# hupe1980/vecgo

Hardware: AMD Instinct MI355X
Metric: QPS at recall@10≥0.95, 1M×768 HNSW+PQ; PQ-ADC HBM GB/s vs peak (higher is better)
Workload: dtype f32; 1 GPU; flat_exact_l2_1Mx768_top10 (BASELINE configs[1]): MFMA GEMM nomination + exact re-score + proof; operating_point=flat_exact, rows=1000000, dim=768, k=10, parallelism=1 GPU

## Files before the change

### go/segment/resident.go

```go

package segment

import "C"

import (
	"fmt"
	"unsafe"

	"github.com/hupe1980/vecgo/distance"
	"github.com/hupe1980/vecgo/internal/hipctx"
)

type Stats struct {
	NodesVisited, DistanceComputations, DistanceShortCircuits, Pops int64
	DescentDistanceComputations                                    int64
}

const (
	ScanF32 = int32(C.VG_SCAN_F32)
	ScanPQ  = int32(C.VG_SCAN_PQ)
	ScanSQ8 = int32(C.VG_SCAN_SQ8)
)

const (
// ... 346 lines not shown
		return nil, nil, counts, false, nil
	}
	if mask != nil {
		need := (r.rows + 7) / 8
		if maskStride != 0 {
			if maskStride < need {
				return nil, nil, nil, false, fmt.Errorf("%s: maskStride %d is shorter than a mask (%d bytes)", name, maskStride, need)
			}
			need += (nq - 1) * maskStride
		}
		if len(mask) < need {
			return nil, nil, nil, false, fmt.Errorf("%s: mask holds %d bytes, %d needed", name, len(mask), need)
		}
	}
	ids, sc = r.out(nq, maxResults)
	return ids, sc, counts, true, nil
}

func (r *Resident) SearchProbedThreshold(queries []float32, nq int, thresholds []float32, maxResults, nprobes int, scan int32, rerank bool, mask []byte, maskStride int) ([]uint32, []float32, []int32, error) {
	ids, sc, counts, ok, err := r.thresholdOperands("SearchProbedThreshold", nq, thresholds, maxResults, mask, maskStride)
	if !ok {
		return nil, nil, counts, err
	}
	var mp *C.uint8_t
	if mask != nil {
		mp = bp(mask)
	}
	rr := 0
	if rerank {
		rr = 1
	}
	st := C.vg_search_flat_probed_threshold(r.h, fp(queries), C.int64_t(nq), fp(thresholds), C.int32_t(maxResults), C.int32_t(nprobes), C.int32_t(scan), C.int32_t(rr), mp, C.int64_t(maskStride), up(ids), fp(sc), ip(counts), nil)
	return ids, sc, counts, hipctx.Err(int32(st))
}

func (r *Resident) SearchSegmentThreshold(queries []float32, nq int, thresholds []float32, maxResults, nprobes int, rerank bool, mask []byte, maskStride int) ([]uint32, []float32, []int32, error) {
	ids, sc, counts, ok, err := r.thresholdOperands("SearchSegmentThreshold", nq, thresholds, maxResults, mask, maskStride)
	if !ok {
		return nil, nil, counts, err
	}
	var mp *C.uint8_t
	if mask != nil {
		mp = bp(mask)
	}
	rr := 0
	if rerank {
		rr = 1
	}
	st := C.vg_segment_search_threshold(r.seg, fp(queries), C.int64_t(nq), fp(thresholds), C.int32_t(maxResults), C.int32_t(nprobes), C.int32_t(rr), mp, C.int64_t(maskStride), up(ids), fp(sc), ip(counts), nil)
	return ids, sc, counts, hipctx.Err(int32(st))
}

func (r *Resident) SearchPQ(queries []float32, nq, k int) ([]uint32, []float32, error) {
	ids, sc := r.out(nq, k)
	st := C.vg_search_pq_adc(r.h, fp(queries), C.int64_t(nq), C.int32_t(k), up(ids), fp(sc), nil)
	return ids, sc, hipctx.Err(int32(st))
}

func (r *Resident) SearchSQ8(queries []float32, nq, k int) ([]uint32, []float32, error) {
	ids, sc := r.out(nq, k)
	st := C.vg_search_sq8(r.h, fp(queries), C.int64_t(nq), C.int32_t(k), up(ids), fp(sc), nil)
	return ids, sc, hipctx.Err(int32(st))
}

func (r *Resident) EnableSQ8Nomination(on bool) error {
	v := C.int32_t(0)
	if on {
		v = 1
	}
	return hipctx.Err(int32(C.vg_index_enable_sq8_nomination(r.h, v, nil)))
}

func (r *Resident) EnablePQNomination(on bool) error {
	v := C.int32_t(0)
	if on {
		v = 1
	}
	return hipctx.Err(int32(C.vg_index_enable_pq_nomination(r.h, v, nil)))
}

func (r *Resident) FlatRetried() (int64, error) {
	var n C.int64_t
	st := C.vg_index_flat_retried(r.h, &n, nil)
	return int64(n), hipctx.Err(int32(st))
}

func (r *Resident) SearchRaBitQ(queries []float32, nq, k int) ([]uint32, []float32, error) {
	ids, sc := r.out(nq, k)
	st := C.vg_search_rabitq(r.h, fp(queries), C.int64_t(nq), C.int32_t(k), up(ids), fp(sc), nil)
	return ids, sc, hipctx.Err(int32(st))
}

func (r *Resident) SearchProbed(queries []float32, nq, k, nprobes int, scan int32) ([]uint32, []float32, error) {
	ids, sc := r.out(nq, k)
	st := C.vg_search_flat_probed(r.h, fp(queries), C.int64_t(nq), C.int32_t(k), C.int32_t(nprobes), C.int32_t(scan), up(ids), fp(sc), nil)
	return ids, sc, hipctx.Err(int32(st))
}

func (r *Resident) SearchSegmentFiltered(queries []float32, nq, k, nprobes int, mask []byte, maskStride int) ([]uint32, []float32, error) {
	ids, sc := r.out(nq, k)
	need := (r.rows + 7) / 8
	if maskStride != 0 {
		if maskStride < need {
			return nil, nil, fmt.Errorf("SearchSegmentFiltered: maskStride %d is shorter than a mask (%d bytes)", maskStride, need)
		}
		need += (nq - 1) * maskStride
	}
	if len(mask) < need {
		return nil, nil, fmt.Errorf("SearchSegmentFiltered: mask holds %d bytes, %d needed", len(mask), need)
	}
	st := C.vg_segment_search_filtered(r.seg, fp(queries), C.int64_t(nq), C.int32_t(k), C.int32_t(nprobes), bp(mask), C.int64_t(maskStride), up(ids), fp(sc), nil)
	return ids, sc, hipctx.Err(int32(st))
}

func (r *Resident) SearchFiltered(queries []float32, nq, k, nprobes int, scan int32, mask []byte, maskStride int) ([]uint32, []float32, error) {
	ids, sc := r.out(nq, k)
	need := (r.rows + 7) / 8
	if maskStride != 0 {
		if maskStride < need {
			return nil, nil, fmt.Errorf("SearchFiltered: maskStride %d is shorter than a mask (%d bytes)", maskStride, need)
		}
		need += (nq - 1) * maskStride
	}
	if len(mask) < need {
		return nil, nil, fmt.Errorf("SearchFiltered: mask holds %d bytes, %d needed", len(mask), need)
	}
	st := C.vg_search_flat_filtered(r.h, fp(queries), C.int64_t(nq), C.int32_t(k), C.int32_t(nprobes), C.int32_t(scan), bp(mask), C.int64_t(maskStride), up(ids), fp(sc), nil)
	return ids, sc, hipctx.Err(int32(st))
}

func (r *Resident) Search(queries []float32, nq, k, nprobes int) ([]uint32, []float32, error) {
	ids, sc := r.out(nq, k)
	st := C.vg_segment_search(r.seg, fp(queries), C.int64_t(nq), C.int32_t(k), C.int32_t(nprobes), up(ids), fp(sc), nil)
	return ids, sc, hipctx.Err(int32(st))
}

func (r *Resident) SearchHNSW(queries []float32, nq, k, ef int, stats []Stats) ([]uint32, []float32, error) {
	ids, sc := r.out(nq, k)
	var sp *C.vg_search_stats
	if len(stats) >= nq && nq > 0 {
		sp = (*C.vg_search_stats)(unsafe.Pointer(&stats[0]))
	}
	st := C.vg_search_hnsw(r.h, fp(queries), C.int64_t(nq), C.int32_t(k), C.int32_t(ef), up(ids), fp(sc), sp, nil)
	return ids, sc, hipctx.Err(int32(st))
}

func (r *Resident) SearchHNSWPQ(queries []float32, nq, k, ef int, stats []Stats) ([]uint32, []float32, error) {
	ids, sc := r.out(nq, k)
	var sp *C.vg_search_stats
	if len(stats) >= nq && nq > 0 {
		sp = (*C.vg_search_stats)(unsafe.Pointer(&stats[0]))
	}
	st := C.vg_search_hnsw_pq(r.h, fp(queries), C.int64_t(nq), C.int32_t(k), C.int32_t(ef), up(ids), fp(sc), sp, nil)
	return ids, sc, hipctx.Err(int32(st))
}

func (r *Resident) SearchHNSWFiltered(queries []float32, nq, k, ef int, mask []byte, maskStride int, selectivity float64, stats []Stats) ([]uint32, []float32, error) {
	ids, sc := r.out(nq, k)
	need := (r.rows + 7) / 8
	if maskStride != 0 {
		if maskStride < need {
			return nil, nil, fmt.Errorf("SearchHNSWFiltered: maskStride %d is shorter than a mask (%d bytes)", maskStride, need)
		}
		need += (nq - 1) * maskStride
	}
	if len(mask) < need {
// ... 196 lines not shown
```

### include/vecgo_hip.h

```cpp
#ifndef VECGO_HIP_H
#define VECGO_HIP_H

#include <stddef.h>
#include <stdint.h>

#ifdef __cplusplus
extern "C" {
#endif

#define VG_ABI_VERSION 2
#define VG_ABI_MINOR 13
#define VG_INVALID_ID 0xFFFFFFFFu
#define VG_STREAM_LEGACY ((void *)1)

typedef enum vg_status {
    VG_OK = 0,
    VG_ERR_INVALID_ARG = -1,
    VG_ERR_DIM_MISMATCH = -2,
    VG_ERR_NOT_TRAINED = -3,
    VG_ERR_CODE_LENGTH = -4,
    VG_ERR_UNSUPPORTED = -5,
    VG_ERR_OUT_OF_MEMORY = -6,
    VG_ERR_HIP = -7,
    VG_ERR_NO_DEVICE = -8,
// ... 89 lines not shown
                                const int64_t *level_rows, uint32_t entry_point, void *stream);
int32_t vg_hnsw_build(vg_index *idx, int32_t m, int32_t ef_construction, int32_t max_batch,
                      int32_t growth_div, void *stream);
int32_t vg_hnsw_insert(vg_index *idx, const float *rows, int64_t count, int32_t m, int32_t ef_construction,
                       int32_t max_batch, int32_t growth_div, void *stream);
int32_t vg_hnsw_level_for_id(uint64_t id, int32_t m);
typedef struct vg_hnsw_compact_stats {
    int64_t repaired_nodes;
    int64_t repaired_lists;
    int64_t pruned_links;
    int64_t cleared_nodes;
} vg_hnsw_compact_stats;
int32_t vg_hnsw_compact(vg_index *idx, int32_t ef_construction, int32_t max_batch, vg_hnsw_compact_stats *stats,
                        void *stream);
int32_t vg_index_get_hnsw_graph(const vg_index *idx, int32_t *m0, int32_t *m, int32_t *max_level,
                                uint32_t *entry_point, int64_t *level_rows, uint32_t *l0,
                                uint32_t *upper_slot, uint32_t *upper_adj, void *stream);
int32_t vg_index_set_vamana_graph(vg_index *idx, int32_t r, const uint32_t *graph, uint32_t entry_point,
                                  void *stream);
int32_t vg_vamana_build(vg_index *idx, int32_t r, int32_t l, float alpha, const uint32_t *init_graph, uint64_t seed,
                        int32_t max_batch, int32_t growth_div, void *stream);
int32_t vg_vamana_insert(vg_index *idx, const float *rows, int64_t count, int32_t r, int32_t l, float alpha,
                         const uint8_t *deleted, uint64_t seed, int32_t max_batch, int32_t growth_div, void *stream);
typedef struct vg_vamana_consolidate_stats {
    int64_t repaired_nodes;
    int64_t dropped_links;
    int64_t links_before;
    int64_t links_after;
} vg_vamana_consolidate_stats;
int32_t vg_vamana_consolidate(vg_index *idx, int32_t l, float alpha, const uint8_t *deleted, int32_t max_batch,
                              vg_vamana_consolidate_stats *stats, void *stream);
int32_t vg_index_get_vamana_graph(const vg_index *idx, int32_t *r, uint32_t *entry_point, uint32_t *graph,
                                  void *stream);
int32_t vg_vamana_reorder_bfs(vg_index *idx, uint32_t *perm, uint32_t *inv_perm, void *stream);

int32_t vg_index_set_vectors(vg_index *idx, const float *base, void *stream);

int32_t vg_squared_l2_batch(vg_ctx *ctx, const float *query, const float *targets, int64_t dim,
                            int64_t n, float *out, void *stream);
int32_t vg_dot_batch(vg_ctx *ctx, const float *query, const float *targets, int64_t dim,
                     int64_t n, float *out, void *stream);

int32_t vg_squared_l2_bounded_batch(vg_ctx *ctx, const float *query, const float *targets, int64_t dim,
                                    int64_t n, const float *bounds, int64_t n_bounds, float *dist,
                                    int32_t *exceeded, void *stream);
int32_t vg_pq_adc_lookup_batch(vg_ctx *ctx, const float *table, const uint8_t *codes, int64_t m, int64_t n,
                               float *out, void *stream);

int32_t vg_kmeans_train(vg_ctx *ctx, const float *vectors, int64_t n, int32_t dim, int32_t k, int32_t metric,
                        int32_t max_iter, uint64_t seed, float *centroids, int32_t *produced, void *stream);
int32_t vg_kmeans_assign(vg_ctx *ctx, const float *vectors, int64_t n, int32_t dim, const float *centroids,
                         int32_t k, int32_t metric, int32_t *out, void *stream);
int32_t vg_find_closest_centroids(vg_ctx *ctx, const float *query, const float *centroids, int32_t dim,
                                  int32_t k, int32_t nprobe, int32_t metric, int32_t *out, int32_t *n_out,
                                  void *stream);

int64_t vg_binary_code_bytes(int32_t dim);
int32_t vg_binary_train(vg_ctx *ctx, int32_t dim, const float *vectors, int64_t n, float *threshold, void *stream);
int32_t vg_binary_encode(vg_ctx *ctx, int32_t dim, float threshold, const float *vectors, int64_t n,
                         uint8_t *codes, void *stream);
int32_t vg_binary_decode(vg_ctx *ctx, int32_t dim, float threshold, const uint8_t *codes, int64_t n,
                         int32_t code_bytes, float *out, void *stream);
int32_t vg_binary_hamming_batch(vg_ctx *ctx, int32_t dim, float threshold, const float *query,
                                const uint8_t *codes, int64_t n, int32_t *out, void *stream);
int32_t vg_normalize_l2(vg_ctx *ctx, float *vectors, int64_t n, int32_t dim, uint8_t *ok, void *stream);

int32_t vg_rerank(vg_index *idx, const float *queries, int64_t nq, const uint32_t *cand_ids,
                  int32_t nc, int32_t k, uint32_t *ids, float *scores, void *stream);
int32_t vg_score_candidates(vg_index *idx, const float *queries, int64_t nq,
                            const uint32_t *cand_ids, int32_t nc, float *scores, void *stream);

int32_t vg_search_flat(vg_index *idx, const float *queries, int64_t nq, int32_t k, uint32_t *ids,
                       float *scores, void *stream);
int32_t vg_index_enable_bf16_filter(vg_index *idx, int32_t on, void *stream);

int32_t vg_search_flat_threshold(vg_index *idx, const float *queries, int64_t nq, const float *thresholds,
                                 int32_t max_results, const uint8_t *mask, int64_t mask_stride,
                                 uint32_t *ids, float *scores, int32_t *counts, void *stream);

int32_t vg_index_flat_stats(vg_index *idx, int64_t *queries, int64_t *exhaustive, void *stream);

int32_t vg_index_flat_retried(vg_index *idx, int64_t *retried, void *stream);

int32_t vg_search_rabitq(vg_index *idx, const float *queries, int64_t nq, int32_t k, uint32_t *ids,
                         float *scores, void *stream);

int32_t vg_sq8_create(vg_ctx *ctx, int32_t dim, vg_sq8 **out);
int32_t vg_sq8_destroy(vg_sq8 *sq);
int32_t vg_sq8_is_trained(vg_sq8 *sq);
int32_t vg_sq8_train(vg_sq8 *sq, const float *vectors, int64_t n, void *stream);
int32_t vg_sq8_set_bounds(vg_sq8 *sq, const float *mins, const float *maxs);
int32_t vg_sq8_get_params(vg_sq8 *sq, float *mins, float *maxs, float *scales, float *inv_scales);
int32_t vg_sq8_encode(vg_sq8 *sq, const float *vectors, int64_t n, uint8_t *codes, void *stream);
int32_t vg_sq8_decode(vg_sq8 *sq, const uint8_t *codes, int64_t n, float *out, void *stream);
int32_t vg_sq8_l2_distance_batch(vg_sq8 *sq, const float *query, const uint8_t *codes, int64_t n,
                                 float *out, void *stream);
int32_t vg_index_set_sq8_codes(vg_index *idx, vg_sq8 *sq, const uint8_t *codes, void *stream);
int32_t vg_index_enable_sq8_nomination(vg_index *idx, int32_t on, void *stream);
int32_t vg_search_sq8(vg_index *idx, const float *queries, int64_t nq, int32_t k, uint32_t *ids,
                      float *scores, void *stream);

int32_t vg_int4_create(vg_ctx *ctx, int32_t dim, vg_int4 **out);
int32_t vg_int4_destroy(vg_int4 *iq);
int32_t vg_int4_is_trained(vg_int4 *iq);
int32_t vg_int4_train(vg_int4 *iq, const float *vectors, int64_t n, void *stream);
int32_t vg_int4_set_params(vg_int4 *iq, const float *min_val, const float *diff);
int32_t vg_int4_get_params(vg_int4 *iq, float *min_val, float *diff, float *table);
int64_t vg_int4_code_bytes(int32_t dim);
int32_t vg_int4_encode(vg_int4 *iq, const float *vectors, int64_t n, uint8_t *codes, void *stream);
int32_t vg_int4_decode(vg_int4 *iq, const uint8_t *codes, int64_t n, float *out, void *stream);
int32_t vg_int4_l2_distance_batch(vg_int4 *iq, const float *query, const uint8_t *codes, int64_t n,
                                  int32_t precomputed, float *out, void *stream);
int32_t vg_index_set_int4_codes(vg_index *idx, vg_int4 *iq, const uint8_t *codes, void *stream);

int32_t vg_robust_prune(vg_index *idx, const uint32_t *nodes, int64_t n_nodes, const uint32_t *cands,
                        int32_t nc, int32_t r, float alpha, uint32_t *out, int32_t *counts, void *stream);
int32_t vg_hnsw_select_neighbors(vg_index *idx, int64_t n_nodes, const uint32_t *cand_ids,
                                 const float *cand_dists, int32_t nc, int32_t m, uint32_t *out,
                                 int32_t *counts, void *stream);

int32_t vg_index_set_partitions(vg_index *idx, const float *centroids, const uint32_t *part_offsets,
                                int32_t num_partitions, void *stream);
enum { VG_SCAN_F32 = 0, VG_SCAN_PQ = 1, VG_SCAN_SQ8 = 2 };
int32_t vg_search_flat_probed(vg_index *idx, const float *queries, int64_t nq, int32_t k, int32_t nprobes,
                              int32_t scan, uint32_t *ids, float *scores, void *stream);
int32_t vg_search_flat_filtered(vg_index *idx, const float *queries, int64_t nq, int32_t k, int32_t nprobes,
                                int32_t scan, const uint8_t *mask, int64_t mask_stride, uint32_t *ids, float *scores,
                                void *stream);

int32_t vg_search_flat_probed_threshold(vg_index *idx, const float *queries, int64_t nq, const float *thresholds,
                                        int32_t max_results, int32_t nprobes, int32_t scan , int32_t rerank,
                                        const uint8_t *mask, int64_t mask_stride,
                                        uint32_t *ids, float *scores, int32_t *counts, void *stream);

int32_t vg_flat_build(vg_index *idx, int32_t num_partitions, int32_t quantization, int32_t pq_m, int32_t kmeans_iters,
                      int32_t pq_iters, uint64_t seed, vg_sq8 *sq, vg_pq *pq, uint32_t *perm, uint32_t *inv_perm, void *stream);

enum { VG_QUANT_NONE = 0, VG_QUANT_PQ = 1, VG_QUANT_SQ8 = 3, VG_QUANT_RABITQ = 5, VG_QUANT_INT4 = 6 };
typedef struct vg_segment_info {
    uint64_t segment_id;
    int64_t rows;
    int32_t dim, metric;
    int32_t kind;
    int32_t quantization;
    int32_t pq_m, pq_k;
    int32_t max_degree, search_list_size;
    uint32_t entrypoint;
    int32_t num_partitions;
} vg_segment_info;
int32_t vg_segment_open_flat(vg_ctx *ctx, const void *image, int64_t size, int32_t verify_checksum,
                             vg_segment **out, void *stream);
int32_t vg_segment_search(vg_segment *seg, const float *queries, int64_t nq, int32_t k, int32_t nprobes,
                          uint32_t *ids, float *scores, void *stream);
int32_t vg_segment_search_filtered(vg_segment *seg, const float *queries, int64_t nq, int32_t k, int32_t nprobes,
                                   const uint8_t *mask, int64_t mask_stride, uint32_t *ids, float *scores, void *stream);
int32_t vg_segment_search_threshold(vg_segment *seg, const float *queries, int64_t nq, const float *thresholds,
                                    int32_t max_results, int32_t nprobes, int32_t rerank, const uint8_t *mask,
                                    int64_t mask_stride, uint32_t *ids, float *scores, int32_t *counts, void *stream);
int32_t vg_segment_open_diskann(vg_ctx *ctx, const void *image, int64_t size, int32_t verify_checksum,
                                vg_segment **out, void *stream);
int32_t vg_segment_get_info(vg_segment *seg, vg_segment_info *info);
vg_index *vg_segment_index(vg_segment *seg);
vg_pq *vg_segment_pq(vg_segment *seg);
vg_sq8 *vg_segment_sq8(vg_segment *seg);
vg_int4 *vg_segment_int4(vg_segment *seg);
int32_t vg_segment_close(vg_segment *seg);
// ... 81 lines not shown
```

### include/vecgo_hip.hpp

```cpp
#pragma once

#include <algorithm>
#include <cstdint>
#include <cstring>
#include <memory>
#include <stdexcept>
#include <string>
#include <utility>
#include <vector>

#include "vecgo_hip.h"

namespace vecgo {

class Error : public std::runtime_error {
public:
    Error(int32_t status, const std::string &msg) : std::runtime_error(msg), status_(status) {}
    int32_t status() const { return status_; }

private:
    int32_t status_;
};

inline void check(int32_t status)
// ... 483 lines not shown
{
    int32_t out = -1;
    check(vg_kmeans_assign(c.handle(), vec.data(), 1, dim, centroids.data(), static_cast<int32_t>(centroids.size() / dim),
                           static_cast<int32_t>(metric), &out, nullptr));
    return out;
}

inline std::vector<int> FindClosestCentroids(const Context &c, const std::vector<float> &query,
                                             const std::vector<float> &centroids, int dim, int n, distance::Metric metric)
{
    const int k = static_cast<int>(centroids.size() / dim);
    std::vector<int32_t> out(static_cast<size_t>(std::max(1, std::min(n, k))));
    int32_t cnt = 0;
    check(vg_find_closest_centroids(c.handle(), query.data(), centroids.data(), dim, k, n, static_cast<int32_t>(metric),
                                    out.data(), &cnt, nullptr));
    return std::vector<int>(out.begin(), out.begin() + cnt);
}

}

inline uint32_t CRC32CDevice(const Context &c, const void *devicePtr, int64_t size)
{
    uint32_t out = 0;
    check(vg_crc32c_device(c.handle(), devicePtr, size, &out, nullptr));
    return out;
}

struct Result {
    std::vector<uint32_t> ids;
    std::vector<float> scores;
};
struct ThresholdResult {
    std::vector<uint32_t> ids;
    std::vector<float> scores;
    std::vector<int32_t> counts;
};

class Segment {
public:
    Segment(std::shared_ptr<Context> ctx, int64_t rows, int dim, distance::Metric metric)
        : ctx_(std::move(ctx)), n_(rows), dim_(dim)
    {
        check(vg_index_create(ctx_->handle(), rows, dim, static_cast<int32_t>(metric), &h_));
    }
    ~Segment() { vg_index_destroy(h_); }
    Segment(const Segment &) = delete;
    Segment &operator=(const Segment &) = delete;

    void SetVectors(const float *base) { check(vg_index_set_vectors(h_, base, nullptr)); }
    void SetPQCodes(std::shared_ptr<quantization::ProductQuantizer> pq, const uint8_t *codes)
    {
        pq_ = std::move(pq);
        check(vg_index_set_pq_codes(h_, pq_->handle(), codes, nullptr));
    }
    void SetRaBitQCodes(const uint8_t *codes) { check(vg_index_set_rabitq_codes(h_, codes, nullptr)); }
    void SetVamanaGraph(int r, const uint32_t *graph, uint32_t entry) { check(vg_index_set_vamana_graph(h_, r, graph, entry, nullptr)); }
    void SetHNSWLayer0(int m0, const uint32_t *l0, uint32_t entry)
    {
        check(vg_index_set_hnsw_graph(h_, m0, l0, 0, m0 / 2 > 0 ? m0 / 2 : 1, nullptr, nullptr, nullptr, entry, nullptr));
    }

    Result SearchFlat(const float *queries, int64_t nq, int k) { return run(nq, k, [&](Result &r) { return vg_search_flat(h_, queries, nq, k, r.ids.data(), r.scores.data(), nullptr); }); }
    ThresholdResult SearchThreshold(const float *queries, int64_t nq, const float *thresholds, int max_results,
                                    const uint8_t *mask = nullptr, int64_t mask_stride = 0)
    {
        ThresholdResult r;
        r.ids.resize(static_cast<size_t>(nq) * max_results);
        r.scores.resize(static_cast<size_t>(nq) * max_results);
        r.counts.resize(static_cast<size_t>(nq));
        check(vg_search_flat_threshold(h_, queries, nq, thresholds, max_results, mask, mask_stride, r.ids.data(), r.scores.data(),
                                       r.counts.data(), nullptr));
        return r;
    }
    ThresholdResult SearchProbedThreshold(const float *queries, int64_t nq, const float *thresholds, int max_results, int nprobes,
                                          int scan, bool rerank, const uint8_t *mask = nullptr, int64_t mask_stride = 0)
    {
        ThresholdResult r;
        r.ids.resize(static_cast<size_t>(nq) * max_results);
        r.scores.resize(static_cast<size_t>(nq) * max_results);
        r.counts.resize(static_cast<size_t>(nq));
        check(vg_search_flat_probed_threshold(h_, queries, nq, thresholds, max_results, nprobes, scan, rerank ? 1 : 0, mask, mask_stride,
                                              r.ids.data(), r.scores.data(), r.counts.data(), nullptr));
        return r;
    }
    void EnableBF16Filter(bool on = true) { check(vg_index_enable_bf16_filter(h_, on ? 1 : 0, nullptr)); }
    Result SearchPQ(const float *queries, int64_t nq, int k) { return run(nq, k, [&](Result &r) { return vg_search_pq_adc(h_, queries, nq, k, r.ids.data(), r.scores.data(), nullptr); }); }
    void EnablePQNomination(bool on = true) { check(vg_index_enable_pq_nomination(h_, on ? 1 : 0, nullptr)); }
    Result SearchRaBitQ(const float *queries, int64_t nq, int k) { return run(nq, k, [&](Result &r) { return vg_search_rabitq(h_, queries, nq, k, r.ids.data(), r.scores.data(), nullptr); }); }
    void SetPartitions(const float *centroids, const uint32_t *part_offsets, int num_partitions)
    {
        check(vg_index_set_partitions(h_, centroids, part_offsets, num_partitions, nullptr));
    }
    Result SearchFiltered(const float *queries, int64_t nq, int k, int nprobes, int scan, const uint8_t *mask, int64_t mask_stride) { return run(nq, k, [&](Result &r) { return vg_search_flat_filtered(h_, queries, nq, k, nprobes, scan, mask, mask_stride, r.ids.data(), r.scores.data(), nullptr); }); }
    Result SearchProbed(const float *queries, int64_t nq, int k, int nprobes, int scan) { return run(nq, k, [&](Result &r) { return vg_search_flat_probed(h_, queries, nq, k, nprobes, scan, r.ids.data(), r.scores.data(), nullptr); }); }
    void BuildHNSW(int m = 32, int efConstruction = 300, int maxBatch = 8192, int growthDiv = 32)
    {
        check(vg_hnsw_build(h_, m, efConstruction, maxBatch, growthDiv, nullptr));
    }
    void InsertHNSW(const float *rows, int64_t count, int m = 32, int ef = 300, int maxBatch = 8192, int growthDiv = 32)
    {
        check(vg_hnsw_insert(h_, rows, count, m, ef, maxBatch, growthDiv, nullptr));
    }
    vg_hnsw_compact_stats CompactHNSW(int ef = 300, int maxBatch = 8192)
    {
        vg_hnsw_compact_stats stats{};
        check(vg_hnsw_compact(h_, ef, maxBatch, &stats, nullptr));
        return stats;
    }
    void BuildVamana(int r = 64, int l = 100, float alpha = 1.2f, const uint32_t *initGraph = nullptr, uint64_t seed = 0,
                     int maxBatch = 8192, int growthDiv = 32)
    {
        check(vg_vamana_build(h_, r, l, alpha, initGraph, seed, maxBatch, growthDiv, nullptr));
    }
    void InsertVamana(const float *rows, int64_t count, int r = 64, int l = 100, float alpha = 1.2f, const uint8_t *deleted = nullptr,
                      uint64_t seed = 0, int maxBatch = 8192, int growthDiv = 32)
    {
        check(vg_vamana_insert(h_, rows, count, r, l, alpha, deleted, seed, maxBatch, growthDiv, nullptr));
    }
    vg_vamana_consolidate_stats ConsolidateVamana(const uint8_t *deleted, int l = 100, float alpha = 1.2f, int maxBatch = 8192)
    {
        vg_vamana_consolidate_stats stats{};
        check(vg_vamana_consolidate(h_, l, alpha, deleted, maxBatch, &stats, nullptr));
        return stats;
    }
    void ReorderVamanaBFS(uint32_t *perm, uint32_t *invPerm) { check(vg_vamana_reorder_bfs(h_, perm, invPerm, nullptr)); }
    void FlatBuild(int numPartitions, int quantization, std::shared_ptr<quantization::ScalarQuantizer> sq,
                   std::shared_ptr<quantization::ProductQuantizer> pq, uint32_t *perm, uint32_t *invPerm, uint64_t seed = 0,
                   int pqM = 0, int kmeansIters = 0, int pqIters = 0)
    {
        check(vg_flat_build(h_, numPartitions, quantization, pqM, kmeansIters, pqIters, seed, sq ? sq->handle() : nullptr,
                            pq ? pq->handle() : nullptr, perm, invPerm, nullptr));
        if (quantization == VG_QUANT_SQ8) sq_ = std::move(sq);
        if (quantization == VG_QUANT_PQ) pq_ = std::move(pq);
    }
    std::vector<uint8_t> WriteFlat(uint64_t segmentID, const uint64_t *ids = nullptr, const std::vector<uint8_t> *metadata = nullptr,
                                   const std::vector<uint8_t> *blockStats = nullptr)
    {
        const int64_t size = vg_segment_flat_image_size(h_, metadata ? static_cast<int64_t>(metadata->size()) : -1,
                                                        blockStats ? static_cast<int64_t>(blockStats->size()) : -1);
        if (size < 0) check(VG_ERR_UNSUPPORTED);
        std::vector<uint8_t> image(static_cast<size_t>(size));
        static const uint8_t none = 0;
        int64_t written = 0;
        check(vg_segment_write_flat(h_, segmentID, ids, metadata ? (metadata->empty() ? &none : metadata->data()) : nullptr,
                                    metadata ? static_cast<int64_t>(metadata->size()) : 0,
                                    blockStats ? (blockStats->empty() ? &none : blockStats->data()) : nullptr,
                                    blockStats ? static_cast<int64_t>(blockStats->size()) : 0, image.data(), size, &written, nullptr));
        return image;
    }
    int DiskANNBuild(int r, int l, float alpha, int quantization, std::shared_ptr<quantization::ProductQuantizer> pq,
                     std::shared_ptr<quantization::Int4Quantizer> iq, uint32_t *perm, uint32_t *invPerm, uint64_t seed = 0,
                     int pqM = 0, int pqIters = 0, int maxBatch = 8192, int growthDiv = 32)
    {
        int32_t used = VG_QUANT_NONE;
        check(vg_diskann_build(h_, r, l, alpha, quantization, pqM, pqIters, seed, maxBatch, growthDiv, pq ? pq->handle() : nullptr,
                               iq ? iq->handle() : nullptr, perm, invPerm, &used, nullptr));
        if (used == VG_QUANT_PQ) pq_ = std::move(pq);
        if (used == VG_QUANT_INT4) iq_ = std::move(iq);
        return used;
    }
    std::vector<uint8_t> WriteDiskANN(uint64_t segmentID, int searchListSize = 0, int compressionType = 1, const uint64_t *ids = nullptr,
                                      const std::vector<uint8_t> *metadata = nullptr, const std::vector<uint8_t> *metadataIndex = nullptr)
    {
        const int64_t size = vg_segment_diskann_image_size(h_, metadata ? static_cast<int64_t>(metadata->size()) : -1,
                                                           metadataIndex ? static_cast<int64_t>(metadataIndex->size()) : -1);
        std::vector<uint8_t> image(static_cast<size_t>(size < 0 ? 1 : size));
// ... 67 lines not shown
```

### vecgo_amd/api.py

```python
from __future__ import annotations

import ctypes as C
import enum

import numpy as np

from . import _lib
from ._lib import VecgoHipError, check

try:
    import torch
except Exception:
    torch = None


class Metric(enum.IntEnum):
    L2 = 0
    COSINE = 1
    DOT = 2
    HAMMING = 3


def _is_torch(x) -> bool:
    return torch is not None and isinstance(x, torch.Tensor)
# ... 1302 lines not shown
    def score_candidates(self, queries, cand_ids, out=None, stream=None):
        nq = _rows(queries, self.dim)
        nc = (cand_ids.numel() if _is_torch(cand_ids) else np.asarray(cand_ids).size) // max(nq, 1)
        q, pq_ = _ptr(queries, np.float32)
        c, pc = _ptr(cand_ids, np.uint32, nq * nc)
        if out is None:
            out = _empty_like(queries, (nq, nc), np.float32)
        s, ps = _ptr(out, np.float32, nq * nc)
        check(self._lib.vg_score_candidates(self._h, pq_, C.c_int64(nq), pc, C.c_int32(nc), ps,
                                            _stream_ptr(stream)))
        return out

    def _search(self, fn, queries, k, extra=(), out=None, stream=None):
        nq = _rows(queries, self.dim)
        q, pq_ = _ptr(queries, np.float32)
        if out is None:
            ids = _empty_like(queries, (nq, k), np.uint32)
            scores = _empty_like(queries, (nq, k), np.float32)
        else:
            ids, scores = out
        i, pi = _ptr(ids, np.uint32, nq * k)
        s, ps = _ptr(scores, np.float32, nq * k)
        check(fn(self._h, pq_, C.c_int64(nq), C.c_int32(k), *extra, pi, ps, _stream_ptr(stream)))
        return ids, scores

    def search_flat(self, queries, k, out=None, stream=None):
        return self._search(self._lib.vg_search_flat, queries, k, out=out, stream=stream)

    def _threshold_search(self, name, call, queries, thresholds, max_results, mask, out):
        nq = _rows(queries, self.dim)
        q, pq_ = _ptr(queries, np.float32)
        if _is_torch(thresholds):
            t = thresholds.to(torch.float32).reshape(-1)
            if t.numel() == 1 and nq != 1:
                t = t.expand(nq)
            t = t.contiguous()
        else:
            t = np.asarray(thresholds, np.float32).reshape(-1)
            if t.size == 1:
                t = np.full(nq, t[0], np.float32)
        if (t.numel() if _is_torch(t) else t.size) != nq:
            raise ValueError(f"{name}: one threshold for the batch or one per query ({nq})")
        t, pt = _ptr(t, np.float32, nq)
        m, pm, stride = (None, None, 0) if mask is None else self._packed_mask(mask, nq, name)
        if out is None:
            ids = _empty_like(queries, (nq, max_results), np.uint32)
            scores = _empty_like(queries, (nq, max_results), np.float32)
            counts = _empty_like(queries, (nq,), np.int32)
        else:
            ids, scores, counts = out
        i, pi = _ptr(ids, np.uint32, nq * max_results)
        s, ps = _ptr(scores, np.float32, nq * max_results)
        c, pc = _ptr(counts, np.int32, nq)
        check(call(pq_, C.c_int64(nq), pt, pm, C.c_int64(stride), pi, ps, pc))
        return ids, scores, counts

    def search_flat_threshold(self, queries, thresholds, max_results, mask=None, out=None, stream=None):
        def call(pq_, nq, pt, pm, stride, pi, ps, pc):
            return self._lib.vg_search_flat_threshold(self._h, pq_, nq, pt, C.c_int32(max_results), pm, stride, pi, ps, pc,
                                                      _stream_ptr(stream))
        return self._threshold_search("search_flat_threshold", call, queries, thresholds, max_results, mask, out)

    def search_flat_probed_threshold(self, queries, thresholds, max_results, nprobes=0, scan=0, rerank=False, mask=None, out=None,
                                     stream=None):
        def call(pq_, nq, pt, pm, stride, pi, ps, pc):
            return self._lib.vg_search_flat_probed_threshold(self._h, pq_, nq, pt, C.c_int32(max_results), C.c_int32(nprobes),
                                                             C.c_int32(scan), C.c_int32(1 if rerank else 0), pm, stride, pi, ps, pc,
                                                             _stream_ptr(stream))
        return self._threshold_search("search_flat_probed_threshold", call, queries, thresholds, max_results, mask, out)

    def enable_bf16_filter(self, on: bool = True, stream=None):
        check(self._lib.vg_index_enable_bf16_filter(self._h, C.c_int32(1 if on else 0), _stream_ptr(stream)))

    def flat_stats(self, stream=None):
        q, e = C.c_int64(0), C.c_int64(0)
        check(self._lib.vg_index_flat_stats(self._h, C.byref(q), C.byref(e), _stream_ptr(stream)))
        return q.value, e.value

    def flat_retried(self, stream=None):
        r = C.c_int64(0)
        check(self._lib.vg_index_flat_retried(self._h, C.byref(r), _stream_ptr(stream)))
        return r.value

    def search_pq_adc(self, queries, k, out=None, stream=None):
        return self._search(self._lib.vg_search_pq_adc, queries, k, out=out, stream=stream)


class SegmentInfo(C.Structure):
    _fields_ = [("segment_id", C.c_uint64), ("rows", C.c_int64), ("dim", C.c_int32), ("metric", C.c_int32),
                ("kind", C.c_int32), ("quantization", C.c_int32), ("pq_m", C.c_int32), ("pq_k", C.c_int32),
                ("max_degree", C.c_int32), ("search_list_size", C.c_int32), ("entrypoint", C.c_uint32),
                ("num_partitions", C.c_int32)]


class Segment:

    def __init__(self, ctx: Context, image, kind: str = "flat", verify_checksum: bool = True, stream=None):
        self._lib, self.ctx = ctx._lib, ctx
        buf = np.frombuffer(image, np.uint8) if isinstance(image, (bytes, bytearray, memoryview)) else \
            np.ascontiguousarray(image, np.uint8)
        fn = {"flat": self._lib.vg_segment_open_flat, "diskann": self._lib.vg_segment_open_diskann}[kind]
        h = C.c_void_p()
        check(fn(ctx._h, C.c_void_p(buf.ctypes.data), C.c_int64(buf.size), C.c_int32(int(verify_checksum)),
                 C.byref(h), _stream_ptr(stream)))
        self._h = h
        info = SegmentInfo()
        check(self._lib.vg_segment_get_info(self._h, C.byref(info)))
        self.info = info
        self._lib.vg_segment_index.restype = C.c_void_p
        ih = C.c_void_p(self._lib.vg_segment_index(self._h))
        self.index = Index._borrowed(ctx, ih, int(info.rows), int(info.dim), int(info.metric), self)

    def search(self, queries, k, nprobes=0, out=None, stream=None):
        seg = self._h

        def fn(_index_handle, *args):
            return self._lib.vg_segment_search(seg, *args)
        return self.index._search(fn, queries, k, extra=(C.c_int32(nprobes),), out=out, stream=stream)

    def search_filtered(self, queries, k, mask, nprobes=0, out=None, stream=None):
        if mask is None:
            return self.search(queries, k, nprobes, out=out, stream=stream)
        seg = self._h
        m, pm, stride = self.index._packed_mask(mask, _rows(queries, self.index.dim), "Segment.search_filtered")

        def fn(_index_handle, *args):
            return self._lib.vg_segment_search_filtered(seg, *args)
        return self.index._search(fn, queries, k, extra=(C.c_int32(nprobes), pm, C.c_int64(stride)), out=out, stream=stream)

    def search_threshold(self, queries, thresholds, max_results, nprobes=0, rerank=False, mask=None, out=None, stream=None):
        seg = self._h

        def call(pq_, nq, pt, pm, stride, pi, ps, pc):
            return self._lib.vg_segment_search_threshold(seg, pq_, nq, pt, C.c_int32(max_results), C.c_int32(nprobes),
                                                         C.c_int32(1 if rerank else 0), pm, stride, pi, ps, pc, _stream_ptr(stream))
        return self.index._threshold_search("Segment.search_threshold", call, queries, thresholds, max_results, mask, out)

    def close(self):
        if getattr(self, "_h", None):
            self.index._h = None
            self._lib.vg_segment_close(self._h)
            self._h = None

    def __del__(self):
        try:
            self.close()
        except Exception:
            pass


def crc32c(data) -> int:
    from . import _lib
    lib = _lib.load()
    lib.vg_crc32c.restype = C.c_uint32
    buf = np.frombuffer(data, np.uint8) if isinstance(data, (bytes, bytearray, memoryview)) else \
        np.ascontiguousarray(data, np.uint8)
    return int(lib.vg_crc32c(C.c_void_p(buf.ctypes.data), C.c_int64(buf.size)))


def crc32c_device(ctx: Context, data, stream=None) -> int:
    if not _is_torch(data) or not data.is_cuda:
        raise TypeError("crc32c_device takes a torch tensor in device memory (crc32c is the host's)")
    if not data.is_contiguous():
        raise ValueError("crc32c_device: the tensor must be contiguous")
    out = C.c_uint32(0)
    check(ctx._lib.vg_crc32c_device(ctx._h, C.c_void_p(data.data_ptr()), C.c_int64(data.numel() * data.element_size()), C.byref(out),
# ... 3 lines not shown
```

### vecgo_amd/csrc/k_exact.hip

```cpp
#include "vg_device.hpp"
#include "vg_exact.hpp"
#include "vg_internal.hpp"

namespace vg {

constexpr int kExactThreads = 256;

template <bool DOT>
__global__ __launch_bounds__(kExactThreads) void batch_kernel(const float *__restrict__ query,
                                                              const float *__restrict__ targets,
                                                              int dim, int64_t n,
                                                              float *__restrict__ out)
{
    const Sub16 sub = Sub16::make(threadIdx.x);
    const int64_t groups = static_cast<int64_t>(gridDim.x) * (kExactThreads / 16);
    for (int64_t i = static_cast<int64_t>(blockIdx.x) * (kExactThreads / 16) + (threadIdx.x >> 4);
         i < n; i += groups) {
        const float v = exact_pair16<DOT, kBatch, true>(targets + i * dim, query, dim, sub);
        if ((threadIdx.x & 15) == 0) out[i] = v;
    }
}

__global__ __launch_bounds__(256) void bounded_batch_kernel(const float *__restrict__ query,
                                                            const float *__restrict__ targets, int dim, int64_t n,
// ... 86 lines not shown
{
    __shared__ float sm[1024];
    float m = 0.0f;
    for (int64_t i = threadIdx.x; i < n; i += 1024) m = fmaxf(m, v[i]);
    sm[threadIdx.x] = m;
    __syncthreads();
    for (int s = 512; s > 0; s >>= 1) {
        if (threadIdx.x < s) sm[threadIdx.x] = fmaxf(sm[threadIdx.x], sm[threadIdx.x + s]);
        __syncthreads();
    }
    if (threadIdx.x == 0) out[0] = sm[0];
}

__global__ void row_norms_kernel(const float *__restrict__ base, int64_t n, int dim,
                                 float *__restrict__ norms, int *__restrict__ maxabs_bits)
{
    const int64_t row = static_cast<int64_t>(blockIdx.x) * (blockDim.x / 64) + (threadIdx.x >> 6);
    if (row >= n) return;
    const int lane = threadIdx.x & 63;
    float s = 0.0f, mx = 0.0f;
    for (int j = lane; j < dim; j += 64) {
        const float v = base[row * dim + j];
        s = __builtin_fmaf(v, v, s);
        const float a = fabsf(v);
        mx = fmaxf(mx, a == a ? a : INFINITY);
    }
    for (int off = 32; off > 0; off >>= 1) {
        s += __shfl_xor(s, off);
        mx = fmaxf(mx, __shfl_xor(mx, off));
    }
    if (lane == 0) {
        norms[row] = s;
        if (__float_as_int(mx) > *reinterpret_cast<volatile int *>(maxabs_bits)) atomicMax(maxabs_bits, __float_as_int(mx));
    }
}

}

static bool metric_is_dot(int32_t metric) { return metric != VG_METRIC_L2; }

namespace vg {
__global__ void fold_max_kernel(float *__restrict__ dst, const float *__restrict__ src) { dst[0] = fmaxf(dst[0], src[0]); }

int32_t append_row_norms(vg_index *idx, int64_t from, int64_t to, hipStream_t st)
{
    if (to <= from) return VG_OK;
    DevTmp<float> mx;
    VG_TRY(mx.init(1, st));
    VG_LAUNCH(row_norms_kernel, dim3(static_cast<unsigned>((to - from + 3) / 4)), dim3(256), 0, st,
              idx->d_vectors + from * idx->dim, to - from, idx->dim, idx->d_norms + from, reinterpret_cast<int *>(idx->d_norm_max + 1));
    VG_LAUNCH(norm_max_kernel, dim3(1), dim3(1024), 0, st, idx->d_norms + from, to - from, mx.ptr);
    VG_LAUNCH(fold_max_kernel, dim3(1), dim3(1), 0, st, idx->d_norm_max, mx.ptr);
    return VG_OK;
}
}

VG_API int32_t vg_index_set_vectors(vg_index *idx, const float *base, void *stream)
{
    VG_CHECK(idx, VG_ERR_INVALID_ARG, "vg_index_set_vectors: NULL index");
    VG_CHECK(idx->n == 0 || base, VG_ERR_INVALID_ARG, "vg_index_set_vectors: base is NULL");
    VG_CHECK(idx->metric != VG_METRIC_HAMMING, VG_ERR_UNSUPPORTED,
             "unsupported metric for float32: Hamming");
    VG_HIP(hipSetDevice(idx->ctx->device));
    hipStream_t st = vg::pick_stream(idx->ctx, stream);
    if (idx->d_vectors) {
        VG_HIP(hipStreamSynchronize(st));
        VG_HIP(hipFree(idx->d_vectors));
        VG_HIP(hipFree(idx->d_norms));
        VG_HIP(hipFree(idx->d_norm_max));
        VG_HIP(hipFree(idx->d_flat_stats));
        if (idx->d_vectors_bf16) VG_HIP(hipFree(idx->d_vectors_bf16));
        idx->d_vectors = idx->d_norms = idx->d_norm_max = nullptr;
        idx->d_flat_stats = nullptr;
        idx->d_vectors_bf16 = nullptr;
    }
    idx->rows_cap = idx->bf16_cap = 0;
    if (idx->n == 0) return VG_OK;
    const int32_t status = [&]() -> int32_t {
        size_t count = static_cast<size_t>(idx->n) * idx->dim;
        VG_HIP(hipMalloc(reinterpret_cast<void **>(&idx->d_vectors), count * sizeof(float)));
        VG_HIP(hipMalloc(reinterpret_cast<void **>(&idx->d_norms), static_cast<size_t>(idx->n) * sizeof(float)));
        VG_HIP(hipMalloc(reinterpret_cast<void **>(&idx->d_norm_max), 2 * sizeof(float)));
        VG_HIP(hipMemsetAsync(idx->d_norm_max, 0, 2 * sizeof(float), st));
        VG_HIP(hipMalloc(reinterpret_cast<void **>(&idx->d_flat_stats), 3 * sizeof(unsigned long long)));
        VG_HIP(hipMemcpyAsync(idx->d_vectors, base, count * sizeof(float), hipMemcpyDefault, st));
        VG_LAUNCH(vg::row_norms_kernel, dim3(static_cast<unsigned>((idx->n + 3) / 4)), dim3(256),
                           0, st, idx->d_vectors, idx->n, idx->dim, idx->d_norms, reinterpret_cast<int *>(idx->d_norm_max + 1));
        VG_LAUNCH(vg::norm_max_kernel, dim3(1), dim3(1024), 0, st, idx->d_norms, idx->n, idx->d_norm_max);
        VG_HIP(hipMemsetAsync(idx->d_flat_stats, 0, 3 * sizeof(unsigned long long), st));
        VG_HIP(hipStreamSynchronize(st));
        return VG_OK;
    }();
    if (status != VG_OK) {
        (void)hipStreamSynchronize(st);
        if (idx->d_vectors) (void)hipFree(idx->d_vectors);
        if (idx->d_norms) (void)hipFree(idx->d_norms);
        if (idx->d_norm_max) (void)hipFree(idx->d_norm_max);
        if (idx->d_flat_stats) (void)hipFree(idx->d_flat_stats);
        idx->d_vectors = idx->d_norms = idx->d_norm_max = nullptr;
        idx->d_flat_stats = nullptr;
    }
    return status;
}

static int32_t batch_impl(vg_ctx *ctx, bool dot, const float *query, const float *targets,
                          int64_t dim, int64_t n, float *out, void *stream)
{
    VG_CHECK(ctx, VG_ERR_INVALID_ARG, "batch kernel: ctx is NULL");
    if (dim <= 0 || n <= 0) return VG_OK;
    VG_CHECK(query && targets && out, VG_ERR_INVALID_ARG, "batch kernel: NULL buffer");
    VG_CHECK(dim < (1 << 30), VG_ERR_INVALID_ARG, "batch kernel: dim too large");
    VG_HIP(hipSetDevice(ctx->device));
    hipStream_t st = vg::pick_stream(ctx, stream);
    vg::DevIn<float> q, t;
    vg::DevOut<float> o;
    VG_TRY(q.init(query, static_cast<size_t>(dim), st));
    VG_TRY(t.init(targets, static_cast<size_t>(n) * dim, st));
    VG_TRY(o.init(out, static_cast<size_t>(n), st));
    int64_t blocks = (n + 15) / 16;
    if (blocks > 4096) blocks = 4096;
    {
        auto kern = dot ? vg::batch_kernel<true> : vg::batch_kernel<false>;
        VG_LAUNCH(kern, dim3(static_cast<unsigned>(blocks)),
                           dim3(vg::kExactThreads), 0, st, q.ptr, t.ptr, static_cast<int>(dim), n, o.ptr);
    }
    VG_TRY(o.finish());
    return VG_OK;
}

VG_API int32_t vg_squared_l2_batch(vg_ctx *ctx, const float *query, const float *targets,
                                   int64_t dim, int64_t n, float *out, void *stream)
{
    return batch_impl(ctx, false, query, targets, dim, n, out, stream);
}

VG_API int32_t vg_dot_batch(vg_ctx *ctx, const float *query, const float *targets, int64_t dim,
                            int64_t n, float *out, void *stream)
{
    return batch_impl(ctx, true, query, targets, dim, n, out, stream);
}

VG_API int32_t vg_squared_l2_bounded_batch(vg_ctx *ctx, const float *query, const float *targets, int64_t dim,
                                           int64_t n, const float *bounds, int64_t n_bounds, float *dist,
                                           int32_t *exceeded, void *stream)
{
    VG_CHECK(ctx, VG_ERR_INVALID_ARG, "vg_squared_l2_bounded_batch: ctx is NULL");
    if (n <= 0) return VG_OK;
    VG_CHECK(dim >= 0 && dim < (1 << 30), VG_ERR_INVALID_ARG, "vg_squared_l2_bounded_batch: bad dim");
    VG_CHECK(bounds && dist && exceeded && (n_bounds == 1 || n_bounds == n), VG_ERR_INVALID_ARG,
             "vg_squared_l2_bounded_batch: bounds must have 1 or n entries");
    VG_CHECK(dim == 0 || (query && targets), VG_ERR_INVALID_ARG, "vg_squared_l2_bounded_batch: NULL buffer");
    VG_HIP(hipSetDevice(ctx->device));
    hipStream_t st = vg::pick_stream(ctx, stream);
    vg::DevIn<float> q, t, b;
    vg::DevOut<float> od;
    vg::DevOut<int32_t> oe;
    VG_TRY(q.init(query, static_cast<size_t>(dim), st));
    VG_TRY(t.init(targets, static_cast<size_t>(n) * dim, st));
    VG_TRY(b.init(bounds, static_cast<size_t>(n_bounds), st));
    VG_TRY(od.init(dist, static_cast<size_t>(n), st));
    VG_TRY(oe.init(exceeded, static_cast<size_t>(n), st));
    int64_t blocks = std::min<int64_t>((n + 15) / 16, 4096);
    VG_LAUNCH(vg::bounded_batch_kernel, dim3(static_cast<unsigned>(blocks)), dim3(256), 0, st, q.ptr, t.ptr,
                       static_cast<int>(dim), n, b.ptr, n_bounds, od.ptr, oe.ptr);
    VG_TRY(od.finish());
    VG_TRY(oe.finish());
    return VG_OK;
}

VG_API int32_t vg_score_candidates(vg_index *idx, const float *queries, int64_t nq,
                                   const uint32_t *cand_ids, int32_t nc, float *scores,
                                   void *stream)
// ... 74 lines not shown
```

### vecgo_amd/csrc/k_flat.hip

```cpp
#include <algorithm>

#include "vg_device.hpp"
#include "vg_exact.hpp"
#include "vg_cand_replay.hpp"
#include "vg_flat_gemm.hpp"
#include "vg_internal.hpp"
#include "vg_nominate.hpp"
#include "vg_search.hpp"

namespace vg {

struct GemmOperands {
    const float *a, *b;
    int64_t n;
    int dim_words;
    const float *norms;
    bool bf16, dma;
};
struct NomCall {
    hipStream_t st;
    bool dot;
    GemmOperands ops;
    int64_t cnt;
    const uint8_t *mask;
// ... 13 lines not shown
    int cap = 0;
    int cus = 256;
    int *counts_wide = nullptr;
    int skip_stride = 0;
    bool split = false;
    bool screen = false;
    const uint32_t *tile_active = nullptr;

    explicit GemmArgs(const NomCall &call) : c(call), queries(call.ops.a) {}
    static GemmArgs sample(const NomCall &c, float *sc, int stride, int64_t cols)
    {
        GemmArgs a(c);
        a.scores = sc, a.tile_stride = stride, a.out_cols = cols;
        return a;
    }
    static GemmArgs append(const NomCall &c, const float *thr, int sel_k, int *counts, uint64_t *cand, int cap)
    {
        GemmArgs a(c);
        a.thr = thr, a.thr_stride = sel_k, a.thr_off = sel_k - 1, a.counts = counts, a.cand = cand, a.cap = cap;
        return a;
    }
    GemmArgs &wide(int *lines, int compute_units) { return counts_wide = lines, cus = compute_units, *this; }
    GemmArgs &skipping(int stride) { return skip_stride = stride, *this; }
    GemmArgs &split_tile(const uint32_t *image) { return queries = reinterpret_cast<const float *>(image), split = true, *this; }
    GemmArgs &screen_tile() { return screen = true, *this; }
    GemmArgs &retry(const uint32_t *active) { return tile_active = active, *this; }
};
constexpr int kCountLine = 32;
static bool gemm_runs_split(bool fused, bool bf16, bool dma, int64_t nq, int dim, int cap, int thr_stride)
{
    return fused && !bf16 && dma && nq > kGemmBM && dim % kGemmBK == 0 && nq * static_cast<int64_t>(cap) < (int64_t(1) << 31) &&
           thr_stride < 65536 && !hook(kHookFlatNoSplit);
}
static float split_gemm_eps(bool dot, int dim)
{
    const float m = static_cast<float>(3 * dim + 16) * 5.9604645e-8f;
    return dot ? 1.5001f * 1.52587890625e-5f + 2.52f * m : 3.0002f * 1.52587890625e-5f + 4.03f * m;
}
static float screen_gemm_eps(bool dot, int dim)
{
    const float m = static_cast<float>(dim + 16) * 5.9604645e-8f;
    return dot ? 0.00390625f + 7.62939453125e-6f + 2.52f * m : 0.0078125f + 1.52587890625e-5f + 4.03f * m;
}
float bf16_filter_eps(bool dot) { return (dot ? 0.00390625f : 0.0078125f) * 1.02f; }
static bool gemm_skips_sample(bool dma, int64_t nq, bool bf16, bool split = false)
{
    if (bf16 || split || hook(kHookFlatRescoreSample)) return false;
    return !(dma && nq <= 3 * kG32BM && !hook(kHookFlatNoSmallTile));
}
__global__ void counts_narrow_kernel(const int *__restrict__ wide, int64_t nq, int *__restrict__ counts)
{
    const int64_t q = static_cast<int64_t>(blockIdx.x) * blockDim.x + threadIdx.x;
    if (q < nq) counts[q] = wide[q * kCountLine];
}

template <class Kern, class... Args>
static int32_t launch_lds(Kern kern, dim3 grid, dim3 threads, size_t lds, hipStream_t st, Args... args)
{
    VG_HIP(hipFuncSetAttribute(reinterpret_cast<const void *>(kern), hipFuncAttributeMaxDynamicSharedMemorySize, static_cast<int>(lds)));
    if (grid.x != 0) VG_LAUNCH(kern, grid, threads, lds, st, args...);
    return VG_OK;
}
template <bool DOT, int M, bool BF16, class F>
static int32_t with_g32_tile(int rb, F f)
{
    constexpr int kMost = BF16 ? 4 : 3;
    if (rb <= 1) return f(flat_gemm_dma32_kernel<DOT, M, 1, BF16>, g32_lds_bytes<1>());
    if (rb == 2) return f(flat_gemm_dma32_kernel<DOT, M, 2, BF16>, g32_lds_bytes<2>());
    if (rb == 3) return f(flat_gemm_dma32_kernel<DOT, M, 3, BF16>, g32_lds_bytes<3>());
    return f(flat_gemm_dma32_kernel<DOT, M, kMost, BF16>, g32_lds_bytes<kMost>());
}

template <bool DOT, int MODE>
static int32_t launch_gemm_t(const GemmArgs &a)
{
    const NomCall &c = a.c;
    const bool dma = c.ops.dma, bf16 = c.ops.bf16;
    const hipStream_t st = c.st;
    const int skip = MODE == 2 ? a.skip_stride : 0;
    VG_CHECK(skip == 0 || (skip > 1 && gemm_skips_sample(dma, c.cnt, bf16, a.split)), VG_ERR_INVALID_ARG, "launch_gemm: skip_stride on a kernel without it");
    const int64_t mt = (c.cnt + kGemmBM - 1) / kGemmBM, nt = (c.ops.n + kGemmBN - 1) / kGemmBN;
    const int64_t tiles = skip ? nt - gemm_skip_sampled_tiles(nt, skip) : (nt + a.tile_stride - 1) / a.tile_stride;
    const dim3 grid(static_cast<unsigned>(mt * ((tiles + 7) / 8) * 8)), threads(kGemmThreads);
    auto launch_big = [&](auto kern, size_t lds, auto... extra) -> int32_t {
        const int64_t bmt = (c.cnt + kBigBM - 1) / kBigBM, bnt = (c.ops.n + kBigBN - 1) / kBigBN;
        const int64_t slots = bmt * ((bnt + 7) / 8) * 8, per_cu = std::max(a.cus / 8, 1) * 8;
        if (a.counts_wide && !a.tile_active) VG_HIP(hipMemsetAsync(a.counts_wide, 0, sizeof(int) * static_cast<size_t>(c.cnt) * kCountLine, st));
        VG_TRY(launch_lds(kern, dim3(static_cast<unsigned>(std::min(slots, per_cu))), dim3(kBigThreads), lds, st, a.queries, c.cnt, c.ops.b, c.ops.n,
                          c.ops.dim_words, c.ops.norms, a.thr, a.thr_stride, a.thr_off, a.counts_wide ? a.counts_wide : a.counts, a.cand, a.cap, c.mask,
                          c.mask_stride, a.counts_wide ? kCountLine : 1, extra...));
        if (a.counts_wide)
            VG_LAUNCH(counts_narrow_kernel, dim3(static_cast<unsigned>((c.cnt + 255) / 256)), dim3(256), 0, st, a.counts_wide, c.cnt, a.counts);
        return VG_OK;
    };
    auto launch_tile = [&](auto kern, dim3 blocks, size_t lds, auto... last) -> int32_t {
        return launch_lds(kern, blocks, threads, lds, st, a.queries, c.cnt, c.ops.b, c.ops.n, c.ops.dim_words, c.ops.norms, a.scores, a.tile_stride, a.out_cols, a.thr,
                          a.thr_stride, a.thr_off, a.counts, a.cand, a.cap, c.mask, c.mask_stride, last...);
    };
    auto launch_128 = [&](auto kern, size_t lds, int last) { return launch_tile(kern, grid, lds, last); };
    auto launch_g32 = [&](auto kern, size_t lds) { return launch_tile(kern, dim3(static_cast<unsigned>(tiles)), lds); };
    constexpr int M = MODE == 0 ? 1 : MODE;
    const int rb = static_cast<int>((c.cnt + kG32BM - 1) / kG32BM);
    if (MODE == 2 && a.split) {
        VG_CHECK(!bf16 && gemm_runs_split(true, false, dma, c.cnt, c.ops.dim_words, a.cap, a.thr_stride), VG_ERR_INVALID_ARG, "launch_gemm: split tile on a call without it");
        if (a.screen) return launch_big(flat_gemm_screen_big_kernel<DOT, 3>, big_lds_bytes<3>());
        VG_CHECK(!a.tile_active || (c.cnt <= 32 * kBigBM && a.counts_wide), VG_ERR_INVALID_ARG, "launch_gemm: tile_active is one word, with wide counters");
        note_flat_split_launch();
        return launch_big(flat_gemm_split_big_kernel<DOT, 3>, big_lds_bytes<3>(), a.tile_active);
    }
    if (skip && tiles == 0) return VG_OK;
    if (bf16) {
        if (c.cnt <= 4 * kG32BM && !hook(kHookFlatNoSmallTile)) return with_g32_tile<DOT, M, true>(rb, launch_g32);
        if (MODE == 2 && c.cnt > kGemmBM && c.cnt * static_cast<int64_t>(a.cap) < (int64_t(1) << 31) && a.thr_stride < 65536 &&
            !hook(kHookFlatNoBigTile)) {
            const bool two = hook(kHookFlatBigTile2);
            auto kern = two ? flat_gemm_bf16_big_kernel<DOT, 2> : hook(kHookFlatBigEarlyB) ? flat_gemm_bf16_big_kernel<DOT, 3, 512> : flat_gemm_bf16_big_kernel<DOT, 3>;
            return launch_big(kern, two ? big_lds_bytes<2>() : big_lds_bytes<3>());
        }
        return launch_128(flat_gemm_dma_kernel<DOT, M, 0, true>, kDmaLdsBytes, 0);
    }
    if (dma && MODE != 0 && c.cnt <= 3 * kG32BM && !hook(kHookFlatNoSmallTile)) return with_g32_tile<DOT, M, false>(rb, launch_g32);
    if (dma) return launch_128(flat_gemm_dma_kernel<DOT, MODE>, kDmaLdsBytes, skip);
    return launch_128(flat_gemm_kernel<DOT, MODE>, kGemmLdsBytes, skip);
}

template <int MODE>
static int32_t launch_gemm(const GemmArgs &a)
{
    return a.c.dot ? launch_gemm_t<true, MODE>(a) : launch_gemm_t<false, MODE>(a);
}

__global__ void f32_to_bf16_pad_kernel(const float *__restrict__ src, int64_t rows, int dim, int dim_pad, uint16_t *__restrict__ dst)
{
    const int64_t i = static_cast<int64_t>(blockIdx.x) * blockDim.x + threadIdx.x;
    if (i >= rows * dim_pad) return;
    const int64_t r = i / dim_pad;
    const int j = static_cast<int>(i - r * dim_pad);
    const uint32_t u = j < dim ? __float_as_uint(src[r * dim + j]) : 0u;
    uint16_t v;
    if ((u & 0x7F800000u) == 0x7F800000u && (u & 0x007FFFFFu) != 0)
        v = static_cast<uint16_t>((u >> 16) | 0x0040u);
    else
        v = static_cast<uint16_t>((u + 0x7FFFu + ((u >> 16) & 1u)) >> 16);
    dst[i] = v;
}

__global__ void flat_split_queries_kernel(const float *__restrict__ src, int64_t rows, int dim, uint32_t *__restrict__ dst)
{
    const int64_t i = static_cast<int64_t>(blockIdx.x) * blockDim.x + threadIdx.x;
    const int half = dim / 2;
    if (i >= rows * half) return;
    const int64_t r = i / half;
    const int p = static_cast<int>(i - r * half), s = p >> 4, w = p & 15;
    const float2 v = *reinterpret_cast<const float2 *>(src + r * dim + 32 * s + 2 * w);
    uint32_t hi, lo;
    split2_bf16(v.x, v.y, hi, lo);
    dst[r * dim + 32 * s + w] = hi;
    dst[r * dim + 32 * s + 16 + w] = lo;
}

__global__ __launch_bounds__(256) void flat_todo_kernel(const int *__restrict__ flags, const int *__restrict__ always,
                                                        int cnt, int *__restrict__ todo,
                                                        unsigned long long *__restrict__ stats)
{
    __shared__ int part[256];
    const int tid = threadIdx.x;
    const int per = (cnt + 255) / 256;
    const int lo = tid * per < cnt ? tid * per : cnt, hi = lo + per < cnt ? lo + per : cnt;
    if (!flags) {
        if (tid == 0) atomicAdd(&stats[0], static_cast<unsigned long long>(cnt));
        return;
    }
    const bool all = *always != 0;
    int mine = 0;
    for (int i = lo; i < hi; i++) mine += (all || flags[i] != 0);
    part[tid] = mine;
    __syncthreads();
    if (tid == 0) {
        int run = 0;
        for (int t = 0; t < 256; t++) {
            const int c = part[t];
            part[t] = run;
            run += c;
        }
        todo[0] = run;
        atomicAdd(&stats[0], static_cast<unsigned long long>(cnt));
        atomicAdd(&stats[1], static_cast<unsigned long long>(run));
    }
    __syncthreads();
    int at = part[tid];
    for (int i = lo; i < hi; i++)
        if (all || flags[i] != 0) todo[1 + at++] = i;
}

__global__ __launch_bounds__(kBigBM) void flat_retry_prepare_kernel(int *__restrict__ flags, bool all, int cnt, float *__restrict__ thr,
                                                                    int thr_stride, int thr_off, int *__restrict__ counts,
                                                                    int *__restrict__ counts_wide, uint32_t *__restrict__ tile_active,
                                                                    unsigned long long *__restrict__ stats)
{
    uint32_t word = 0;
    int total = 0;
    for (int t = 0; t * kBigBM < cnt; t++) {
        const int q = t * kBigBM + static_cast<int>(threadIdx.x);
        bool retry = false;
        if (q < cnt) {
            retry = all || flags[q] != 0;
            if (retry) {
                flags[q] = 1;
                counts[q] = 0;
                counts_wide[static_cast<int64_t>(q) * kCountLine] = 0;
            } else {
                thr[static_cast<int64_t>(q) * thr_stride + thr_off] = -INFINITY;
            }
        }
        const int here = __syncthreads_count(retry);
        word |= here ? 1u << t : 0u;
        total += here;
    }
    if (threadIdx.x == 0) {
        *tile_active = word;
        if (total) atomicAdd(&stats[2], static_cast<unsigned long long>(total));
    }
}

constexpr int kSampleAppendThreads = 256, kSampleAppendVec = 4;
__global__ __launch_bounds__(kSampleAppendThreads) void flat_sample_append_kernel(
    const float *__restrict__ sc , int64_t ns, int sample_stride, const float *__restrict__ thr,
    int thr_stride, int thr_off, int *__restrict__ counts, uint64_t *__restrict__ cand, int cap)
{
    constexpr int kWaves = kSampleAppendThreads / 64, kPiece = kSampleAppendThreads * 4, kRound = kPiece * kSampleAppendVec;
    __shared__ int wave_n[2][kWaves];
    const int64_t q = blockIdx.x;
    const int tid = threadIdx.x, lane = tid & 63, wave = tid >> 6;
    const float t = thr[q * thr_stride + thr_off];
    const float *row = sc + q * ns;
    uint64_t *dst = cand + q * cap;
    const uint64_t below = (uint64_t(1) << lane) - 1;
    int run = 0;
    for (int64_t c0 = 0, round = 0; c0 < ns; c0 += kRound, round++) {
        float v[kSampleAppendVec][4];
#pragma unroll
        for (int u = 0; u < kSampleAppendVec; u++) {
            const int64_t c = c0 + u * kPiece + tid * 4;
            const float4 x = c < ns ? *reinterpret_cast<const float4 *>(row + c) : make_float4(INFINITY, INFINITY, INFINITY, INFINITY);
            v[u][0] = x.x; v[u][1] = x.y; v[u][2] = x.z; v[u][3] = x.w;
        }
        int mine = 0;
#pragma unroll
        for (int u = 0; u < kSampleAppendVec; u++)
#pragma unroll
            for (int e = 0; e < 4; e++) mine += __popcll(__ballot(v[u][e] < t));
        const int b = static_cast<int>(round & 1);
        if (lane == 0) wave_n[b][wave] = mine;
        __syncthreads();
        int at = run, all = 0;
#pragma unroll
        for (int w = 0; w < kWaves; w++) {
            const int cnt = wave_n[b][w];
            at += w < wave ? cnt : 0;
            all += cnt;
        }
        if (mine != 0) {
#pragma unroll
            for (int u = 0; u < kSampleAppendVec; u++)
#pragma unroll
                for (int e = 0; e < 4; e++) {
                    const bool pass = v[u][e] < t;
                    const uint64_t bal = __ballot(pass);
// ... 255 lines not shown
        const int c = c0 + (tid >> 4);
        if (c < cnt) {
            const uint32_t id = key_row(cand[q * cap + c]);
            const float v = exact_pair16<DOT, kPair>(base + static_cast<int64_t>(id) * dim, qv, dim, sub);
            if ((tid & 15) == 0) sortbuf[c] = make_key(v, id, DOT);
        }
    }
    for (int i = cnt + tid; i < n2; i += 256) sortbuf[i] = kKeyMax;
    __syncthreads();
    bitonic_sort_lds(sortbuf, n2, tid, 256);
    for (int i = tid; i < k; i += 256) {
        const uint64_t e = i < n2 ? sortbuf[i] : kKeyMax;
        ids[q * k + i] = e == kKeyMax ? VG_INVALID_ID : key_row(e);
        scores[q * k + i] = e == kKeyMax ? (DOT ? -INFINITY : INFINITY) : key_score(e, DOT);
    }
    if (tid >= 64) return;
    float qn = 0.0f;
    for (int j = lane; j < dim; j += 64) qn = __builtin_fmaf(qv[j], qv[j], qn);
    for (int off = 32; off > 0; off >>= 1) qn += __shfl_xor(qn, off);
    const uint64_t kth = k - 1 < n2 ? sortbuf[k - 1] : kKeyMax;
    const float tau = thr[q * thr_stride + thr_off];
    bool ok = total <= cap;
    if (ok && tau != INFINITY) {
        const float xmax = norms_max[0];
        const float eps = (4.0f * (static_cast<float>(dim) * 5.9604645e-8f) + eps_extra) * (qn + xmax) + 1e-30f;
        if (kth == kKeyMax)
            ok = false;
        else if (DOT)
            ok = key_score(kth, true) > (-tau) + eps;
        else
            ok = key_score(kth, false) < (tau + qn) - eps;
    }
    if (lane == 0) fallback[q] = ok ? 0 : 1;
}

constexpr int kExactSlots = 32;
template <bool DOT>
__global__ __launch_bounds__(256) void flat_exact_kernel(const float *__restrict__ base, int64_t n,
                                                         int dim, const float *__restrict__ queries,
                                                         const int *__restrict__ todo, int slices, int k,
                                                         uint64_t *__restrict__ partial,
                                                         const uint64_t *__restrict__ min_keys = nullptr,
                                                         const uint8_t *__restrict__ mask = nullptr, int64_t mask_stride = 0)
{
    __shared__ uint64_t lists[4 * 64];
    __shared__ int valid[4];
    const int s = blockIdx.x;
    const int tid = threadIdx.x, lane = tid & 63, wave = tid >> 6;
    const int ntodo = todo[0];
    const Sub16 sub = Sub16::make(tid);
    const int64_t r0 = n * s / slices, r1 = n * (s + 1) / slices;
    for (int j = blockIdx.y; j < ntodo; j += gridDim.y) {
        const int64_t q = todo[1 + j];
        uint64_t *out = partial + (q * slices + s) * k;
        const float *qv = queries + q * dim;
        const uint64_t floor_key = min_keys ? min_keys[q] : 0;
        const uint8_t *mq = mask ? mask + q * mask_stride : nullptr;
        WaveTopK tk;
        tk.init(k);
        for (int64_t i0 = r0 + wave * 4; i0 < r1; i0 += 16) {
            const int64_t i = i0 + (lane >> 4);
            uint64_t key = kKeyMax;
            if (i < r1 && mask_bit(mq, i)) {
                const float v = exact_pair16<DOT, kPair>(base + i * dim, qv, dim, sub);
                if ((lane & 15) == 0) {
                    key = make_key(v, static_cast<uint32_t>(i), DOT);
                    if (min_keys && key <= floor_key) key = kKeyMax;
                }
            }
            tk.offer(key, lane);
        }
        wg_rank_merge<4>(tk, lists, valid, wave, lane, tid, k, out);
        __syncthreads();
    }
}

constexpr int kScanQB = 8;
constexpr int kGemmMaxK = 48;
constexpr int kFlatMaxK = 512;
constexpr int kScreenMaxK = 16;
static bool gemm_runs_screen(bool split, int k)
{
    return split && !hook(kHookFlatNoScreen) && k <= (hook(kHookFlatScreenFail) ? kGemmMaxK : kScreenMaxK);
}
constexpr int kScanMaxBatch = 4;
template <bool DOT>
__global__ __launch_bounds__(256) void flat_scan_mq_kernel(const float *__restrict__ base, int64_t n, int dim,
                                                           const float *__restrict__ queries, int nq, int slices,
                                                           int k, uint64_t *__restrict__ partial)
{
    extern __shared__ float qlds[];
    uint64_t *lists = reinterpret_cast<uint64_t *>(qlds + static_cast<size_t>(kScanQB) * dim);
    int *valid = reinterpret_cast<int *>(lists + 4 * 64);
    const int s = blockIdx.x;
    const int tid = threadIdx.x, lane = tid & 63, wave = tid >> 6;
    for (int t = tid; t < nq * dim; t += 256) qlds[t] = queries[t];
    __syncthreads();
    const Sub16 sub = Sub16::make(tid);
    const int nblk = dim >> 6;
    const int64_t r0 = n * s / slices, r1 = n * (s + 1) / slices;
    WaveTopK tk[kScanQB];
#pragma unroll
    for (int qi = 0; qi < kScanQB; qi++) tk[qi].init(k);
    for (int64_t i0 = r0 + wave * 4; i0 < r1; i0 += 16) {
        const int64_t i = i0 + (lane >> 4);
        const bool live = i < r1;
        const float *row = base + (live ? i : r1 - 1) * dim;
        float4 rr[16];
        const float4 *r4 = reinterpret_cast<const float4 *>(row) + sub.f4;
#pragma unroll
        for (int e = 0; e < 16; e++)
            if (e < nblk) rr[e] = load_stream(r4 + e * 16);
#pragma unroll
        for (int qi = 0; qi < kScanQB; qi++) {
            if (qi < nq) {
                const float v = exact_rowregs16<DOT>(rr, nblk, row, qlds + static_cast<size_t>(qi) * dim, dim, sub);
                uint64_t key = kKeyMax;
                if (live && (lane & 15) == 0) key = make_key(v, static_cast<uint32_t>(i), DOT);
                tk[qi].offer(key, lane);
            }
        }
    }
#pragma unroll
    for (int qi = 0; qi < kScanQB; qi++) {
        if (qi < nq) {
            wg_rank_merge<4>(tk[qi], lists, valid, wave, lane, tid, k,
                             partial + (static_cast<int64_t>(qi) * slices + s) * k);
            __syncthreads();
        }
    }
}

__global__ void flat_patch_kernel(const int *__restrict__ fallback, const int *__restrict__ always, int k,
                                  const uint32_t *__restrict__ fids, const float *__restrict__ fscores,
                                  uint32_t *__restrict__ ids, float *__restrict__ scores)
{
    const int64_t q = blockIdx.x;
    if (!(always && always[0]) && !fallback[q]) return;
    for (int i = threadIdx.x; i < k; i += blockDim.x) {
        ids[q * k + i] = fids[q * k + i];
        scores[q * k + i] = fscores[q * k + i];
    }
}

__global__ void flat_page_patch_kernel(const int *__restrict__ fallback, const int *__restrict__ always, int k, int off,
                                       int kk, bool descending, const uint32_t *__restrict__ fids,
                                       const float *__restrict__ fscores, uint32_t *__restrict__ ids,
                                       float *__restrict__ scores, uint64_t *__restrict__ min_keys)
{
    const int64_t q = blockIdx.x;
    if (!(always && always[0]) && !(fallback && fallback[q])) return;
    for (int i = threadIdx.x; i < kk; i += blockDim.x) {
        ids[q * k + off + i] = fids[q * kk + i];
        scores[q * k + off + i] = fscores[q * kk + i];
    }
    if (threadIdx.x == 0) {
        const uint32_t last = fids[q * kk + kk - 1];
        min_keys[q] = last == VG_INVALID_ID ? kKeyMax : make_key(fscores[q * kk + kk - 1], last, descending);
    }
}

int32_t launch_page_patch(int64_t nq, int k, int off, int kk, bool descending, const int *always_one,
                          const uint32_t *fids, const float *fscores, uint32_t *ids, float *scores, uint64_t *min_keys,
                          hipStream_t st)
{
    VG_LAUNCH(flat_page_patch_kernel, dim3(static_cast<unsigned>(nq)), dim3(64), 0, st, nullptr, always_one, k, off, kk,
              descending, fids, fscores, ids, scores, min_keys);
    return VG_OK;
}

static GemmOperands fp32_operands(const vg_index *idx, const float *queries, bool dma = true)
{
    return {queries, idx->d_vectors, idx->n, idx->dim, idx->d_norms, false, dma && idx->dim % 4 == 0 && aligned16(queries) && aligned16(idx->d_vectors)};
}
static int32_t gemm_operands(const float *queries, int64_t cnt, int dim, int64_t n, const float *norms, const uint16_t *rows_bf16, int dim_pad,
                             uint16_t *qbf, hipStream_t st, GemmOperands *ops)
{
    VG_LAUNCH(f32_to_bf16_pad_kernel, dim3(static_cast<unsigned>((cnt * dim_pad + 255) / 256)), dim3(256), 0, st, queries, cnt, dim, dim_pad, qbf);
    *ops = {reinterpret_cast<const float *>(qbf), reinterpret_cast<const float *>(rows_bf16), n, dim_pad / 2, norms, true, true};
    return VG_OK;
}
static int64_t sample_cols(int64_t n, int stride)
{
    const int64_t nt = (n + kGemmBN - 1) / kGemmBN;
    return (nt + stride - 1) / stride * kGemmBN;
}
static int select_slices(int64_t cols, int per_slice, int most)
{
    return static_cast<int>(std::min<int64_t>(most, std::max<int64_t>(1, cols / per_slice)));
}
constexpr int kFlatKc = 64;
struct NomScratch {
    float *sc;
    uint64_t *partial;
    uint32_t *sid;
    int64_t cols;
    int slices;
    ProbeNominated nom;
    size_t bytes;
    void carve(Carve &c, int64_t cnt, int64_t cols_, int sel_k, int cap, bool sampled = true, int slices_ = 0)
    {
        cols = cols_;
        slices = slices_ ? slices_ : select_slices(cols, 4096, 64);
        nom.sel_k = sel_k;
        nom.cap = cap;
        c.take(sc, sampled ? cnt * cols : 1);
        c.take(partial, cnt * slices * sel_k);
        c.take(sid, cnt * sel_k);
        c.take(nom.thr, cnt * sel_k);
        c.take(nom.counts, cnt);
        c.take(nom.cand, cnt * cap);
        c.take(nom.cand_id, cnt * kFlatKc);
        c.take(nom.cand_sc, cnt * kFlatKc);
    }
};
static int32_t launch_flat_select(const NomScratch &s, int64_t cnt, int sel_k, hipStream_t st)
{
    VG_LAUNCH(flat_select_kernel, dim3(s.slices, static_cast<unsigned>(cnt)), dim3(kSelThreads), 0, st, s.sc, s.cols, s.slices, sel_k, s.partial);
    return VG_OK;
}
static int32_t select_thresholds(const NomScratch &s, int64_t cnt, int sel_k, uint32_t *ids, float *thr, hipStream_t st)
{
    VG_TRY(launch_flat_select(s, cnt, sel_k, st));
    return launch_topk_merge(s.partial, cnt, s.slices, sel_k, false, ids, thr, st);
}
static int32_t sample_thresholds(const NomCall &c, const NomScratch &s, int stride, int sel_k, float *thr, bool sampled)
{
    if (!sampled) {
        VG_LAUNCH(fill_f32_kernel, dim3(static_cast<unsigned>((c.cnt * sel_k + 255) / 256)), dim3(256), 0, c.st, thr, c.cnt * sel_k, INFINITY);
        return VG_OK;
    }
    VG_TRY(launch_gemm<1>(GemmArgs::sample(c, s.sc, stride, s.cols)));
    return select_thresholds(s, c.cnt, sel_k, s.sid, thr, c.st);
}
static int32_t launch_flat_pick(const ProbeNominated &nom, int64_t cnt, const int *only, hipStream_t st)
{
    VG_LAUNCH(flat_pick_kernel, dim3(static_cast<unsigned>(cnt)), dim3(256), 0, st, nom.cand, nom.counts, nom.cap, kFlatKc, nom.cand_id, nom.cand_sc, only);
    return VG_OK;
}
static int32_t launch_flat_verify(bool dot, int k, const vg_index *idx, const float *queries, int64_t cnt, const ProbeNominated &nom,
                                  float eps_extra, uint32_t *ids, float *scores, int *fail, const int *only, hipStream_t st)
{
    return with_metric(dot, [&](auto dot_c) -> int32_t {
        constexpr bool DOT = decltype(dot_c)::value;
        const dim3 grid(static_cast<unsigned>(cnt)), threads(256);
        if (nom.thr && k > 64)
            VG_LAUNCH(flat_verify_sort_kernel<DOT>, grid, threads, sizeof(uint64_t) * static_cast<size_t>(nom.cap), st, idx->d_vectors, idx->dim, queries,
                      idx->d_norm_max, nom.cand, nom.counts, nom.cap, k, ids, scores, fail, nom.thr, nom.sel_k, nom.sel_k - 1, eps_extra);
        else if (nom.thr && k > kGemmMaxK)
            VG_LAUNCH(flat_verify_all_kernel<DOT>, grid, threads, 0, st, idx->d_vectors, idx->dim, queries, idx->d_norm_max, nom.cand, nom.counts,
                      nom.cap, k, ids, scores, fail, nom.thr, nom.sel_k, nom.sel_k - 1, eps_extra);
        else
            VG_LAUNCH(flat_verify_kernel<DOT>, grid, threads, 0, st, idx->d_vectors, idx->n, idx->dim, queries, idx->d_norm_max, nom.cand_id,
                      nom.cand_sc, kFlatKc, k, ids, scores, fail, nom.thr, nom.sel_k, nom.sel_k - 1, nom.counts, nom.cap, eps_extra, only);
        return VG_OK;
    });
}

struct FlatCall {
    vg_index *idx;
    int k;
    hipStream_t st;
    bool dot;
    const float *q;
    int64_t nq;
    const uint8_t *mask;
    int64_t mask_stride;
    uint32_t *oid;
    float *osc;
    int64_t n = idx->n;
    int dim = idx->dim;
    FlatCall range(int64_t q0, int64_t cnt) const
    {
        FlatCall r = *this;
        r.q += q0 * dim, r.nq = cnt, r.oid += q0 * k, r.osc += q0 * k;
        if (mask) r.mask += q0 * mask_stride;
        return r;
    }
    NomCall nom() const { return {st, dot, fp32_operands(idx, q, !hook(kHookFlatNoDma)), nq, mask, mask_stride}; }
};
constexpr int kFlatCap = 4096;
constexpr int kFlatSampleStride = 64;
static int exact_slices(int64_t n) { return static_cast<int>(std::min<int64_t>(256, std::max<int64_t>(1, n / 64))); }
struct FlatScratch : NomScratch {
    bool fused;
    bool use_sample;
    bool bf16;
    bool may_split;
    int ex_slices, pk;
    int64_t qc;
    int *flags, *todo;
    uint64_t *fpartial, *min_keys;
    uint32_t *fid;
    float *fsc;
    uint16_t *qbf;
    int *counts_wide;
    uint32_t *tile_active;
    FlatScratch(const FlatCall &c, bool unfused, char *base) : fused(!unfused), use_sample(fused && c.n > kFlatCap)
    {
        bf16 = c.idx->d_vectors_bf16 != nullptr && fused && !hook(kHookFlatNoDma);
        const int sel_k = !fused ? kFlatKc : c.k <= 64 ? 8 : std::min(64, std::max(8, (3 * c.k + 63) / 64));
        ex_slices = exact_slices(c.n);
        pk = std::min(c.k, 64);
        qc = fused ? 4096 : (int64_t(2) << 30) / (c.n * 4);
        if (qc > 4096) qc = 4096;
        if (qc >= kGemmBM) qc = (qc / kGemmBM) * kGemmBM;
        if (qc < 1) qc = 1;
        if (qc > c.nq) qc = c.nq;
        may_split = gemm_runs_split(fused, bf16, true, qc, c.dim, kFlatCap, sel_k);
        Carve cv{base};
        carve(cv, qc, fused ? sample_cols(c.n, kFlatSampleStride) : c.n, sel_k, fused ? kFlatCap : 0, !fused || use_sample);
        cv.take(flags, qc + 1);
        cv.take(todo, qc + 1);
        cv.take(fpartial, qc * ex_slices * pk);
        cv.take(fid, qc * pk);
// ... 16 lines not shown
    const size_t lds = sizeof(float) * static_cast<size_t>(kScanQB) * c.dim + 4 * 64 * sizeof(uint64_t) + 64;
    for (int64_t q0 = 0; q0 < c.nq; q0 += kScanQB) {
        const int cnt = static_cast<int>(std::min<int64_t>(kScanQB, c.nq - q0));
        ProfScope prof(c.idx->ctx, "flat_scan", c.st);
        auto kern = c.dot ? flat_scan_mq_kernel<true> : flat_scan_mq_kernel<false>;
        VG_LAUNCH(kern, dim3(slices), dim3(256), lds, c.st, c.idx->d_vectors, c.n, c.dim, c.q + q0 * c.dim, cnt, slices, c.k, partial + q0 * slices * c.k);
    }
    VG_TRY(launch_topk_merge(partial, c.nq, slices, c.k, c.dot, c.oid, c.osc, c.st));
    return launch_flat_todo(nullptr, nullptr, static_cast<int>(c.nq), nullptr, c.idx->d_flat_stats, c.st);
}

static int32_t launch_flat_exact(const FlatCall &c, const int *todo, int ex_slices, int kk, uint64_t *fpartial, const uint64_t *floor_keys)
{
    const unsigned slots = static_cast<unsigned>(std::min<int64_t>(c.nq, kExactSlots));
    auto kern = c.dot ? flat_exact_kernel<true> : flat_exact_kernel<false>;
    VG_LAUNCH(kern, dim3(ex_slices, slots), dim3(256), 0, c.st, c.idx->d_vectors, c.n, c.dim, c.q, todo, ex_slices, kk, fpartial, floor_keys, c.mask,
              c.mask_stride);
    return VG_OK;
}
static int32_t flat_exact_every_query(const FlatCall &call)
{
    const int ex_slices = exact_slices(call.n);
    const int64_t qc = std::min<int64_t>(call.nq, 4096);
    ArenaCall ar(call.idx->ctx, call.st);
    const int i_flags = ar.add(sizeof(int) * (static_cast<size_t>(qc) + 1));
    const int i_todo = ar.add(sizeof(int) * (static_cast<size_t>(qc) + 1));
    const int i_fpartial = ar.add(sizeof(uint64_t) * static_cast<size_t>(qc) * ex_slices * call.k);
    VG_TRY(ar.commit());
    int *flags = ar.get<int>(i_flags), *todo = ar.get<int>(i_todo);
    uint64_t *fpartial = ar.get<uint64_t>(i_fpartial);
    VG_HIP(hipMemsetAsync(flags, 0, sizeof(int) * static_cast<size_t>(qc), call.st));
    VG_HIP(hipMemsetAsync(flags + qc, 1, sizeof(int), call.st));
    for (int64_t q0 = 0; q0 < call.nq; q0 += qc) {
        const FlatCall c = call.range(q0, std::min(qc, call.nq - q0));
        VG_TRY(launch_flat_todo(flags, flags + qc, static_cast<int>(c.nq), todo, c.idx->d_flat_stats, c.st));
        VG_TRY(launch_flat_exact(c, todo, ex_slices, c.k, fpartial, nullptr));
        VG_TRY(launch_topk_merge(fpartial, c.nq, ex_slices, c.k, c.dot, c.oid, c.osc, c.st));
    }
    return VG_OK;
}

static int32_t flat_unfused_chunk(const FlatCall &c, const FlatScratch &s)
{
    const NomCall nc = c.nom();
    {
        ProfScope prof(c.idx->ctx, "flat_gemm", c.st);
        VG_TRY(launch_gemm<0>(GemmArgs::sample(nc, s.sc, 1, c.n)));
    }
    {
        ProfScope prof(c.idx->ctx, "flat_select", c.st);
        VG_TRY(launch_flat_select(s, c.nq, kFlatKc, c.st));
    }
    VG_TRY(launch_topk_merge(s.partial, c.nq, s.slices, kFlatKc, false, s.nom.cand_id, s.nom.cand_sc, c.st));
    ProbeNominated nom = s.nom;
    nom.thr = nullptr;
    return launch_flat_verify(c.dot, c.k, c.idx, c.q, c.nq, nom, 0.0f, c.oid, c.osc, s.flags, nullptr, c.st);
}

static int32_t flat_screen_retry(const FlatCall &c, const NomCall &nc, const FlatScratch &s)
{
    const ProbeNominated &nom = s.nom;
    VG_LAUNCH(flat_retry_prepare_kernel, dim3(1), dim3(kBigBM), 0, c.st, s.flags, hook(kHookFlatScreenFail), static_cast<int>(c.nq), nom.thr,
              nom.sel_k, nom.sel_k - 1, nom.counts, s.counts_wide, s.tile_active, c.idx->d_flat_stats);
    {
        ProfScope prof(c.idx->ctx, "flat_retry", c.st);
        VG_TRY(launch_gemm<2>(GemmArgs::append(nc, nom.thr, nom.sel_k, nom.counts, nom.cand, nom.cap)
                                  .wide(s.counts_wide, c.idx->ctx->compute_units)
                                  .split_tile(reinterpret_cast<const uint32_t *>(s.qbf))
                                  .retry(s.tile_active)));
    }
    VG_TRY(launch_flat_pick(nom, c.nq, s.flags, c.st));
    return launch_flat_verify(c.dot, c.k, c.idx, c.q, c.nq, nom, split_gemm_eps(c.dot, c.dim), c.oid, c.osc, s.flags, s.flags, c.st);
}

static int32_t flat_fused_chunk(const FlatCall &c, const FlatScratch &s)
{
    const vg_index *idx = c.idx;
    const ProbeNominated &nom = s.nom;
    NomCall nc = c.nom();
    const bool split = gemm_runs_split(true, s.bf16, nc.ops.dma, c.nq, c.dim, nom.cap, nom.sel_k);
    const bool screen = gemm_runs_screen(split, c.k);
    const float eps_extra = screen ? screen_gemm_eps(c.dot, c.dim) : split ? split_gemm_eps(c.dot, c.dim) : s.bf16 ? bf16_filter_eps(c.dot) : 0.0f;
    if (s.bf16) VG_TRY(gemm_operands(c.q, c.nq, c.dim, c.n, idx->d_norms, idx->d_vectors_bf16, idx->vectors_bf16_dim, s.qbf, c.st, &nc.ops));
    VG_TRY(sample_thresholds(nc, s, kFlatSampleStride, nom.sel_k, nom.thr, s.use_sample));
    if (s.bf16 || split) VG_LAUNCH(flat_thr_cap_kernel, dim3(nc.ucnt()), dim3(64), 0, c.st, nom.thr, nom.sel_k, c.q, c.dim, idx->d_norm_max);
    if (split)
        VG_LAUNCH(flat_split_queries_kernel, dim3(static_cast<unsigned>((c.nq * (c.dim / 2) + 255) / 256)), dim3(256), 0, c.st, c.q, c.nq, c.dim,
                  reinterpret_cast<uint32_t *>(s.qbf));
    const bool once = s.use_sample && gemm_skips_sample(nc.ops.dma, c.nq, s.bf16, split);
    if (!once) VG_HIP(hipMemsetAsync(nom.counts, 0, sizeof(int) * static_cast<size_t>(c.nq), c.st));
    {
        ProfScope prof(idx->ctx, "flat_gemm", c.st);
        if (once)
            VG_LAUNCH(flat_sample_append_kernel, dim3(nc.ucnt()), dim3(kSampleAppendThreads), 0, c.st, s.sc, s.cols, kFlatSampleStride, nom.thr,
                      nom.sel_k, nom.sel_k - 1, nom.counts, nom.cand, nom.cap);
        GemmArgs a = GemmArgs::append(nc, nom.thr, nom.sel_k, nom.counts, nom.cand, nom.cap);
        a.wide(s.bf16 || split ? s.counts_wide : nullptr, idx->ctx->compute_units).skipping(once ? kFlatSampleStride : 0);
        if (split) a.split_tile(reinterpret_cast<const uint32_t *>(s.qbf));
        if (screen) a.screen_tile();
        VG_TRY(launch_gemm<2>(a));
    }
    if (c.k <= kGemmMaxK) VG_TRY(launch_flat_pick(nom, c.nq, nullptr, c.st));
    VG_TRY(launch_flat_verify(c.dot, c.k, idx, c.q, c.nq, nom, eps_extra, c.oid, c.osc, s.flags, nullptr, c.st));
    return screen ? flat_screen_retry(c, nc, s) : VG_OK;
}

static void flat_debug_counts(const FlatCall &c, int64_t q0, const FlatScratch &s)
{
    std::vector<int> hf(c.nq), hc(c.nq);
    (void)hipMemcpyAsync(hf.data(), s.flags, sizeof(int) * c.nq, hipMemcpyDeviceToHost, c.st);
    (void)hipMemcpyAsync(hc.data(), s.nom.counts, sizeof(int) * c.nq, hipMemcpyDeviceToHost, c.st);
    (void)hipStreamSynchronize(c.st);
    int64_t nf = 0, csum = 0, cmax = 0;
    for (int f : hf) nf += f != 0;
    for (int n : hc) { csum += n; cmax = std::max<int64_t>(cmax, n); }
    fprintf(stderr, "[vg_search_flat] chunk q0=%lld cnt=%lld: %lld queries failed the proof; "
            "appended candidates avg %.1f max %lld\n", (long long)q0, (long long)c.nq, (long long)nf,
            s.fused ? double(csum) / c.nq : 0.0, (long long)(s.fused ? cmax : 0));
}

static int32_t flat_fallback_pages(const FlatCall &c, const FlatScratch &s)
{
    const int *always = s.flags + s.qc;
    const dim3 grid(static_cast<unsigned>(c.nq));
    for (int off = 0; off < c.k; off += 64) {
        const int kk = std::min(64, c.k - off);
        VG_TRY(launch_flat_exact(c, s.todo, s.ex_slices, kk, s.fpartial, off ? s.min_keys : nullptr));
        VG_TRY(launch_topk_merge(s.fpartial, c.nq, s.ex_slices, kk, c.dot, s.fid, s.fsc, c.st, s.flags, always));
        if (c.k <= 64)
            VG_LAUNCH(flat_patch_kernel, grid, dim3(64), 0, c.st, s.flags, always, c.k, s.fid, s.fsc, c.oid, c.osc);
        else
            VG_LAUNCH(flat_page_patch_kernel, grid, dim3(64), 0, c.st, s.flags, always, c.k, off, kk, c.dot, s.fid, s.fsc, c.oid, c.osc, s.min_keys);
    }
    return VG_OK;
}

static int32_t flat_gemm_search(const FlatCall &call, bool unfused)
{
    ArenaCall ar(call.idx->ctx, call.st);
    const int i_all = ar.add(FlatScratch(call, unfused, nullptr).bytes);
    VG_TRY(ar.commit());
    const FlatScratch s(call, unfused, ar.get<char>(i_all));
    int *always = s.flags + s.qc;
    VG_HIP(hipMemsetAsync(always, hook(kHookFlatForceExact) ? 1 : 0, sizeof(int), call.st));
    for (int64_t q0 = 0; q0 < call.nq; q0 += s.qc) {
        const FlatCall c = call.range(q0, std::min(s.qc, call.nq - q0));
        VG_TRY(s.fused ? flat_fused_chunk(c, s) : flat_unfused_chunk(c, s));
        VG_TRY(launch_flat_todo(s.flags, always, static_cast<int>(c.nq), s.todo, c.idx->d_flat_stats, c.st));
        if (hook(kHookFlatDebug)) flat_debug_counts(c, q0, s);
        VG_TRY(flat_fallback_pages(c, s));
    }
    return VG_OK;
}

int32_t flat_search_masked(vg_index *idx, const float *queries, int64_t nq, int32_t k, const uint8_t *mask, int64_t mask_stride, uint32_t *ids,
                           float *scores, void *stream, bool l2_scores, bool cand_replay)
{
    VG_CHECK(idx, VG_ERR_INVALID_ARG, "vg_search_flat: NULL index");
    VG_CHECK(nq >= 0 && k >= 0, VG_ERR_INVALID_ARG, "vg_search_flat: negative nq or k");
    if (nq == 0 || k == 0) return VG_OK;
    VG_CHECK(idx->metric != VG_METRIC_HAMMING, VG_ERR_UNSUPPORTED, "unsupported metric for float32: Hamming");
    VG_CHECK(idx->n == 0 || idx->d_vectors, VG_ERR_NOT_READY, "vg_search_flat: index has no fp32 vectors");
    VG_CHECK(queries && ids && scores, VG_ERR_INVALID_ARG, "vg_search_flat: NULL buffer");
    VG_CHECK(k <= kFlatMaxK, VG_ERR_UNSUPPORTED, "vg_search_flat: k=%d exceeds %d", k, kFlatMaxK);
    const bool unfused = hook(kHookFlatUnfused) && mask == nullptr;
    VG_CHECK(k <= 64 || !unfused, VG_ERR_UNSUPPORTED, "vg_search_flat: k=%d needs the fused GEMM path", k);

    SearchIO io;
    VG_TRY(io.init(idx->ctx, stream, queries, static_cast<size_t>(nq) * idx->dim, ids, scores, static_cast<size_t>(nq) * k));
    const bool dot = idx->metric != VG_METRIC_L2 && !l2_scores;
    const FlatCall c{idx, k, io.st, dot, io.q.ptr, nq, mask, mask_stride, io.oid.ptr, io.osc.ptr};
    const bool scan_small = mask == nullptr && nq <= kScanMaxBatch && k <= 64 && c.dim % 4 == 0 && c.dim <= 1024 && c.dim >= 64 &&
                            !hook(kHookFlatNoScan) && !hook(kHookFlatForceExact) && !unfused && aligned16(idx->d_vectors);
    if (c.n == 0)
        VG_TRY(empty_results(nq, k, dot, c.oid, c.osc, c.st));
    else if (scan_small)
        VG_TRY(flat_scan_small(c));
    else if (unfused && k > kGemmMaxK)
        VG_TRY(flat_exact_every_query(c));
    else
        VG_TRY(flat_gemm_search(c, unfused));
    if (c.n > 0 && cand_replay)
        VG_TRY(launch_cand_replay(FlatF32Scorer{idx->d_vectors, idx->d_norm_max + 1, c.dim, dot, 0}, c.q, c.dim, c.n, nq, k, dot, mask, mask_stride,
                                  c.oid, c.osc, c.st));
    return io.finish();
}

int probe_gemm_sel_k(int k, bool bf16) { return k <= kGemmMaxK ? 8 : std::min(64, std::max(8, ((bf16 ? 5 : 3) * k + 7) / 8)); }
constexpr int kProbeGemmCap = 2048;
struct ProbeGemmScratch : NomScratch {
    uint16_t *qbf;
    ProbeGemmScratch(char *base, int64_t pairs, int64_t ns_max, int k, int bf16_dim)
    {
        Carve c{base};
        carve(c, pairs, ns_max, probe_gemm_sel_k(k, bf16_dim > 0), kProbeGemmCap, true, select_slices(ns_max, 1024, 8));
        c.take(qbf, pairs * bf16_dim);
        bytes = c.off;
    }
};
size_t flat_probe_gemm_scratch_bytes(int64_t pairs, int64_t ns_max, int k, int bf16_dim)
{
    return ProbeGemmScratch(nullptr, pairs, ns_max, k, bf16_dim).bytes;
}
template <int MODE>
static int32_t launch_gemm_grouped(const GemmArgs &a, const GemmGroup *groups, int ngroups, const int64_t grid[4],
                                   const int64_t *const first_block[4], const int64_t *mask_off)
{
    const NomCall &c = a.c;
    return with_metric(c.dot, [&](auto dot_c) -> int32_t {
        constexpr bool DOT = decltype(dot_c)::value;
        const bool bf16 = c.ops.bf16;
        auto launch = [&](auto kern, size_t lds, int at) -> int32_t {
            return launch_lds(kern, dim3(static_cast<unsigned>(grid[at])), dim3(kGemmThreads), lds, c.st, groups, first_block[at], ngroups, a.queries,
                              c.ops.b, c.ops.dim_words, c.ops.norms, a.scores, a.tile_stride, a.out_cols, a.thr, a.thr_stride, a.thr_off, a.counts, a.cand, a.cap,
                              c.mask, mask_off);
        };
        VG_TRY(launch(bf16 ? flat_gemm_dma_grouped_kernel<DOT, MODE, true> : flat_gemm_dma_grouped_kernel<DOT, MODE>, kDmaLdsBytes, MODE - 1));
        return launch(bf16 ? flat_gemm_dma32_grouped_kernel<DOT, MODE, kProbeRB, true> : flat_gemm_dma32_grouped_kernel<DOT, MODE, kProbeRB>,
                      g32_lds_bytes<kProbeRB>(), MODE + 1);
    });
}

int32_t flat_probe_gemm(vg_index *idx, const float *pair_queries, int64_t pairs, const GemmGroup *groups, const int64_t *const first_block[4],
                        int ngroups, const int64_t grid[4], int sample_stride, int64_t ns_max, int k, uint32_t *pair_ids,
                        float *pair_scores, int *fail, char *scratch, const uint8_t *mask ,
                        const int64_t *mask_off , hipStream_t st,
                        const NomImage &img, ProbeNominated *nominated)
{
    const bool dot = idx->metric != VG_METRIC_L2;
    const bool bf16 = img.rows != nullptr, own_filter = bf16 && img.rows == idx->d_vectors_bf16;
    const ProbeGemmScratch s(scratch, pairs, ns_max, k, img.dim_pad);
// ... 33 lines not shown

int32_t flat_nominate_bf16(vg_index *idx, const NomImage &img, bool dot, const float *queries, int64_t cnt, const uint8_t *mask,
                           int64_t mask_stride, int k, char *scratch, hipStream_t st, ProbeNominated *nom)
{
    const NominateScratch s(scratch, cnt, idx->n, img.dim_pad, k);
    NomCall nc{st, dot, {}, cnt, mask, mask_stride};
    VG_TRY(gemm_operands(queries, cnt, idx->dim, idx->n, img.norms, img.rows, img.dim_pad, s.qbf, st, &nc.ops));
    *nom = s.nom;
    VG_TRY(sample_thresholds(nc, s, kFlatSampleStride, nom->sel_k, nom->thr, idx->n > kFlatCap));
    VG_LAUNCH(flat_thr_cap_kernel, dim3(nc.ucnt()), dim3(64), 0, st, nom->thr, nom->sel_k, queries, idx->dim, img.norm_max);
    VG_HIP(hipMemsetAsync(nom->counts, 0, sizeof(int) * static_cast<size_t>(cnt), st));
    {
        ProfScope prof(idx->ctx, "sq8_nominate_gemm", st);
        VG_TRY(launch_gemm<2>(GemmArgs::append(nc, nom->thr, nom->sel_k, nom->counts, nom->cand, nom->cap).wide(s.counts_wide, idx->ctx->compute_units)));
    }
    return k <= kNomPickMaxK ? launch_flat_pick(*nom, cnt, nullptr, st) : VG_OK;
}

__global__ __launch_bounds__(64) void flat_thr_combine_kernel(const float *__restrict__ uthr, const float *__restrict__ sthr, int sel_k,
                                                              const float *__restrict__ queries, int dim, const float *__restrict__ norm_max,
                                                              float eps_extra, bool dot, float *__restrict__ gthr, float *__restrict__ qnorm,
                                                              int *__restrict__ untight)
{
    const int64_t q = blockIdx.x;
    const int lane = threadIdx.x;
    float qn = 0.0f;
    for (int j = lane; j < dim; j += 64) qn = __builtin_fmaf(queries[q * dim + j], queries[q * dim + j], qn);
    for (int off = 32; off > 0; off >>= 1) qn += __shfl_xor(qn, off);
    if (lane != 0) return;
    qnorm[q] = qn;
    const float xmax = norm_max[0];
    const float bound = 2.002f * (qn + xmax);
    if (!(bound < 1e30f)) {
        gthr[q] = -3.0e38f;
        untight[q] = -1;
        return;
    }
    const float t = uthr[q];
    const float eps = (4.0f * (static_cast<float>(dim) * 5.9604645e-8f) + eps_extra) * (qn + xmax) + 1e-30f;
    float ut = (dot ? -t : t - qn) + eps;
    if (!(ut > -bound)) ut = -bound;
    if (ut > bound) ut = bound;
    const float st = sthr ? sthr[q * sel_k + sel_k - 1] : INFINITY;
    const bool user = ut <= st;
    gthr[q] = user ? ut : st;
    untight[q] = user ? 1 : 0;
}
struct ThrNomScratch : NomScratch {
    ThrNominated out;
    uint16_t *qbf;
    int *counts_wide;
    ThrNomScratch(char *base, const vg_index *idx, const ThrNomPlan &p, int64_t cnt)
    {
        Carve c{base};
        carve(c, cnt, sample_cols(idx->n, p.sample_stride), p.sel_k, p.cap);
        out.counts = nom.counts, out.cand = nom.cand;
        c.take(out.gthr, cnt);
        c.take(out.qnorm, cnt);
        c.take(out.untight, cnt);
        c.take(qbf, p.bf16 ? cnt * idx->vectors_bf16_dim : 0);
        c.take(counts_wide, p.bf16 ? cnt * kCountLine : 0);
        bytes = c.off;
    }
};
size_t flat_thr_nominate_scratch(const vg_index *idx, const ThrNomPlan &p, int64_t qc) { return ThrNomScratch(nullptr, idx, p, qc).bytes; }

int32_t flat_thr_nominate(vg_index *idx, const ThrNomPlan &p, const float *qp, const float *uthr, int64_t cnt, const uint8_t *m0,
                          int64_t mask_stride, char *scratch, ThrNominated *nominated, hipStream_t st)
{
    const ThrNomScratch s(scratch, idx, p, cnt);
    const ThrNominated &out = *nominated = s.out;
    const bool dot = idx->metric != VG_METRIC_L2;
    NomCall nc{st, dot, fp32_operands(idx, qp), cnt, m0, mask_stride};
    if (p.bf16) VG_TRY(gemm_operands(qp, cnt, idx->dim, idx->n, idx->d_norms, idx->d_vectors_bf16, idx->vectors_bf16_dim, s.qbf, st, &nc.ops));
    const bool use_sample = idx->n > p.cap;
    if (use_sample) VG_TRY(sample_thresholds(nc, s, p.sample_stride, p.sel_k, s.nom.thr, true));
    VG_LAUNCH(flat_thr_combine_kernel, dim3(nc.ucnt()), dim3(64), 0, st, uthr, use_sample ? s.nom.thr : nullptr, p.sel_k, qp, idx->dim, idx->d_norm_max,
              p.eps_extra, dot, out.gthr, out.qnorm, out.untight);
    VG_HIP(hipMemsetAsync(out.counts, 0, sizeof(int) * static_cast<size_t>(cnt), st));
    ProfScope prof(idx->ctx, "flat_thr_gemm", st);
    return launch_gemm<2>(GemmArgs::append(nc, out.gthr, 1, out.counts, out.cand, p.cap).wide(p.bf16 ? s.counts_wide : nullptr, idx->ctx->compute_units));
}

int32_t launch_flat_todo(const int *flags, const int *always, int cnt, int *todo, unsigned long long *stats, hipStream_t st)
{
    VG_LAUNCH(flat_todo_kernel, dim3(1), dim3(256), 0, st, flags, always, cnt, todo, stats);
    return VG_OK;
}
}

VG_API int32_t vg_search_flat(vg_index *idx, const float *queries, int64_t nq, int32_t k, uint32_t *ids,
                              float *scores, void *stream)
{
    return vg::flat_search_masked(idx, queries, nq, k, nullptr, 0, ids, scores, stream);
}

namespace vg {
int32_t append_bf16_rows(vg_index *idx, int64_t from, int64_t to, hipStream_t st)
{
    const int64_t count = (to - from) * idx->vectors_bf16_dim;
    if (count <= 0) return VG_OK;
    VG_LAUNCH(f32_to_bf16_pad_kernel, dim3(static_cast<unsigned>((count + 255) / 256)), dim3(256), 0, st,
              idx->d_vectors + from * idx->dim, to - from, idx->dim, idx->vectors_bf16_dim,
              idx->d_vectors_bf16 + from * idx->vectors_bf16_dim);
    return VG_OK;
}
}

VG_API int32_t vg_index_enable_bf16_filter(vg_index *idx, int32_t on, void *stream)
{
    VG_CHECK(idx, VG_ERR_INVALID_ARG, "vg_index_enable_bf16_filter: NULL index");
    VG_HIP(hipSetDevice(idx->ctx->device));
    hipStream_t st = vg::pick_stream(idx->ctx, stream);
    if (idx->d_vectors_bf16) {
        VG_HIP(hipStreamSynchronize(st));
        VG_HIP(hipFree(idx->d_vectors_bf16));
        idx->d_vectors_bf16 = nullptr;
    }
    idx->bf16_cap = 0;
    if (!on) return VG_OK;
    VG_CHECK(idx->d_vectors, VG_ERR_NOT_READY, "vg_index_enable_bf16_filter: index has no fp32 vectors");
    idx->vectors_bf16_dim = (idx->dim + 2 * vg::kGemmBK - 1) / (2 * vg::kGemmBK) * (2 * vg::kGemmBK);
    const int64_t count = idx->n * idx->vectors_bf16_dim;
    VG_HIP(hipMalloc(reinterpret_cast<void **>(&idx->d_vectors_bf16), static_cast<size_t>(count) * sizeof(uint16_t)));
    VG_LAUNCH(vg::f32_to_bf16_pad_kernel, dim3(static_cast<unsigned>((count + 255) / 256)), dim3(256), 0, st, idx->d_vectors,
              idx->n, idx->dim, idx->vectors_bf16_dim, idx->d_vectors_bf16);
    VG_HIP(hipStreamSynchronize(st));
    return VG_OK;
}

VG_API int32_t vg_index_flat_stats(vg_index *idx, int64_t *queries, int64_t *exhaustive, void *stream)
{
    VG_CHECK(idx, VG_ERR_INVALID_ARG, "vg_index_flat_stats: NULL index");
    VG_CHECK(idx->d_flat_stats, VG_ERR_INVALID_ARG, "vg_index_flat_stats: no fp32 vectors attached");
    VG_HIP(hipSetDevice(idx->ctx->device));
    hipStream_t st = vg::pick_stream(idx->ctx, stream);
    unsigned long long h[2] = {0, 0};
    VG_HIP(hipMemcpyAsync(h, idx->d_flat_stats, sizeof h, hipMemcpyDeviceToHost, st));
    VG_HIP(hipStreamSynchronize(st));
    if (queries) *queries = static_cast<int64_t>(h[0]);
    if (exhaustive) *exhaustive = static_cast<int64_t>(h[1]);
    return VG_OK;
}

VG_API int32_t vg_index_flat_retried(vg_index *idx, int64_t *retried, void *stream)
{
    VG_CHECK(idx && retried, VG_ERR_INVALID_ARG, "vg_index_flat_retried: NULL index or pointer");
    VG_CHECK(idx->d_flat_stats, VG_ERR_INVALID_ARG, "vg_index_flat_retried: no fp32 vectors attached");
    VG_HIP(hipSetDevice(idx->ctx->device));
    hipStream_t st = vg::pick_stream(idx->ctx, stream);
    unsigned long long h = 0;
    VG_HIP(hipMemcpyAsync(&h, idx->d_flat_stats + 2, sizeof h, hipMemcpyDeviceToHost, st));
    VG_HIP(hipStreamSynchronize(st));
    *retried = static_cast<int64_t>(h);
    return VG_OK;
}
```

### vecgo_amd/csrc/vg_api.hip

```cpp
#include "vg_internal.hpp"

namespace vg {

static thread_local std::string g_last_error;

void set_error(const char *fmt, ...)
{
    char buf[512];
    va_list ap;
    va_start(ap, fmt);
    vsnprintf(buf, sizeof buf, fmt, ap);
    va_end(ap);
    g_last_error = buf;
}

bool is_device_ptr(const void *p)
{
    if (!p) return false;
    hipPointerAttribute_t a;
    hipError_t e = hipPointerGetAttributes(&a, p);
    (void)hipGetLastError();
    if (e != hipSuccess) return false;
    return a.type == hipMemoryTypeDevice || a.type == hipMemoryTypeManaged;
}
// ... 215 lines not shown
    VG_HIP(hipSetDevice(ctx->device));
    std::lock_guard<std::mutex> g(ctx->prof_mu);
    int64_t n = 0;
    double ms = 0.0;
    std::vector<vg_prof_record> keep;
    for (auto &r : ctx->prof) {
        if (strcmp(r.name, kernel) != 0) {
            keep.push_back(r);
            continue;
        }
        float t = 0.0f;
        if (hipEventSynchronize(r.stop) == hipSuccess && hipEventElapsedTime(&t, r.start, r.stop) == hipSuccess) {
            n++;
            ms += t;
        }
        (void)hipEventDestroy(r.start);
        (void)hipEventDestroy(r.stop);
    }
    ctx->prof.swap(keep);
    *launches = n;
    *total_ms = ms;
    return VG_OK;
}

VG_API int32_t vg_index_create(vg_ctx *ctx, int64_t n, int32_t dim, int32_t metric,
                               vg_index **out)
{
    VG_CHECK(ctx && out, VG_ERR_INVALID_ARG, "vg_index_create: NULL argument");
    *out = nullptr;
    VG_CHECK(n >= 0 && n < 0xFFFFFFFFll, VG_ERR_INVALID_ARG,
             "vg_index_create: n=%lld out of range (row ids are uint32)", (long long)n);
    VG_CHECK(dim > 0, VG_ERR_INVALID_ARG, "vg_index_create: dim must be positive");
    VG_CHECK(metric >= VG_METRIC_L2 && metric <= VG_METRIC_HAMMING, VG_ERR_UNSUPPORTED,
             "vg_index_create: unknown metric %d", metric);
    vg_index *idx = new vg_index();
    idx->ctx = ctx;
    idx->n = n;
    idx->dim = dim;
    idx->metric = metric;
    *out = idx;
    return VG_OK;
}

VG_API int32_t vg_index_destroy(vg_index *idx)
{
    if (!idx) return VG_OK;
    (void)hipSetDevice(idx->ctx->device);
    if (idx->d_pq_tiles) (void)hipFree(idx->d_pq_tiles);
    if (idx->d_vectors) (void)hipFree(idx->d_vectors);
    if (idx->d_norms) (void)hipFree(idx->d_norms);
    if (idx->d_norm_max) (void)hipFree(idx->d_norm_max);
    if (idx->d_flat_stats) (void)hipFree(idx->d_flat_stats);
    if (idx->d_vectors_bf16) (void)hipFree(idx->d_vectors_bf16);
    if (idx->d_rq_tiles) (void)hipFree(idx->d_rq_tiles);
    if (idx->d_rq_norms) (void)hipFree(idx->d_rq_norms);
    for (uint32_t **a : {&idx->d_hnsw_l0, &idx->d_hnsw_slot, &idx->d_hnsw_adj}) vg::drop_device(a);
    for (float **a : {&idx->d_hnsw_l0_dist, &idx->d_hnsw_l0_cdist, &idx->d_hnsw_adj_cdist}) vg::drop_device(a);
    vg::drop_device(&idx->d_hnsw_tomb);
    vg::drop_device(&idx->d_hnsw_level_off);
    if (idx->d_vamana) (void)hipFree(idx->d_vamana);
    if (idx->d_pq_rows) (void)hipFree(idx->d_pq_rows);
    if (idx->d_rq_rows) (void)hipFree(idx->d_rq_rows);
    if (idx->d_sq_tiles) (void)hipFree(idx->d_sq_tiles);
    (void)vg::nom_free(idx->sq_nom, idx->ctx->stream);
    (void)vg::nom_free(idx->pq_nom, idx->ctx->stream);
    if (idx->d_int4_rows) (void)hipFree(idx->d_int4_rows);
    if (idx->d_centroids) (void)hipFree(idx->d_centroids);
    if (idx->d_part_off) (void)hipFree(idx->d_part_off);
    delete idx;
    return VG_OK;
}

#include <atomic>
namespace vg {
static std::atomic<int> g_hooks[kHookCount];
static std::once_flag g_hooks_once;
static const char *const kHookNames[kHookCount] = {"VG_FLAT_NO_SMALL_TILE", "VG_FLAT_UNFUSED", "VG_FLAT_NO_SCAN",
                                                   "VG_FLAT_FORCE_EXACT", "VG_FLAT_NO_DMA", "VG_FLAT_DEBUG",
                                                   "VG_PROBE_NO_GROUP", "VG_ADC_BIGK_EXHAUSTIVE", "VG_BUILD_DEBUG",
                                                   "VG_KM_NO_MFMA", "VG_KM_LIST_ALL", "VG_KM_BF16", "VG_KM_NO_BF16", "VG_BRUTE_NO_FLAT", "VG_PQ_NO_MFMA",
                                                   "VG_PQ_LIST_ALL", "VG_PQ_FP32_MFMA", "VG_PROBE_NO_GEMM", "VG_FLAT_NO_BIG_TILE",
                                                   "VG_FLAT_BIG_TILE_2", "VG_FLAT_BIG_EARLY_B", "VG_PQ_NOM_ALWAYS", "VG_KM_NO_RANGES", "VG_NO_CAND_REPLAY",
                                                   "VG_VAMANA_SMALL_SCRATCH", "VG_FLAT_RESCORE_SAMPLE", "VG_PTHR_FORCE_HIST",
                                                   "VG_WALK_SMALL_SCRATCH", "VG_FLAT_NO_SPLIT", "VG_FLAT_NO_SCREEN", "VG_FLAT_SCREEN_FAIL"};
static void hooks_from_env()
{
    for (int h = 0; h < kHookCount; h++) {
        const char *e = getenv(kHookNames[h]);
        g_hooks[h].store(e && e[0] == '1' ? 1 : 0, std::memory_order_relaxed);
    }
}
bool hook(Hook h)
{
    std::call_once(g_hooks_once, hooks_from_env);
    return g_hooks[h].load(std::memory_order_relaxed) != 0;
}
}

VG_API int32_t vg_debug_set_hook(const char *name, int32_t on)
{
    VG_CHECK(name, VG_ERR_INVALID_ARG, "vg_debug_set_hook: NULL name");
    std::call_once(vg::g_hooks_once, vg::hooks_from_env);
    for (int h = 0; h < vg::kHookCount; h++)
        if (std::strcmp(name, vg::kHookNames[h]) == 0) {
            vg::g_hooks[h].store(on ? 1 : 0, std::memory_order_relaxed);
            return VG_OK;
        }
    vg::set_error("vg_debug_set_hook: unknown hook %s", name);
    return VG_ERR_INVALID_ARG;
}
```

### vecgo_amd/csrc/vg_flat_gemm.hpp

```cpp
#pragma once

#include <hip/hip_runtime.h>

#include <cmath>
#include <cstdint>
#include <type_traits>

#include "vg_device.hpp"

namespace vg {

constexpr int kGemmBM = 128, kGemmBN = 128, kGemmBK = 32, kGemmLd = kGemmBK + 1;
constexpr int kGemmPasses = kGemmBM * kGemmBK / 4 / 256;
constexpr int kGemmThreads = 256;
constexpr int kGemmTile = kGemmBM * kGemmLd;
constexpr size_t kGemmLdsBytes = 4 * kGemmTile * sizeof(float);
using f32x16 = __attribute__((ext_vector_type(16))) float;

template <bool DOT, int MODE>
__device__ __forceinline__ void gemm_epilogue(const f32x16 (&acc)[2][2], float *lds_thr, float thr_reg,
                                              const float (&xn)[2], int tid, int lane, int wr, int wc, int64_t q0,
                                              int64_t nq, int64_t n0, int64_t n, int64_t tn,
                                              float *__restrict__ scores, int64_t out_cols,
                                              int *__restrict__ counts, uint64_t *__restrict__ cand, int cap,
// ... 420 lines not shown
        if (t == 123.456f) scores[0] = t;
        return;
    }
    gemm_epilogue<DOT, MODE>(acc, gemm_lds, thr_reg, xn, tid, lane, wr, wc, q0, nq, n0, n, tn, scores, out_cols,
                             counts, cand, cap, mask, mask_stride, GROUPED ? row_base : 0u, GROUPED ? mask_off : nullptr);
}

template <bool DOT, int MODE, int PROBE = 0, bool BF16 = false>
__global__ __launch_bounds__(kGemmThreads) void flat_gemm_dma_kernel(
    const float *__restrict__ queries, int64_t nq, const float *__restrict__ base, int64_t n,
    int dim, const float *__restrict__ norms, float *__restrict__ scores, int tile_stride,
    int64_t out_cols, const float *__restrict__ thr, int thr_stride, int thr_off,
    int *__restrict__ counts, uint64_t *__restrict__ cand, int cap, const uint8_t *__restrict__ mask = nullptr,
    int64_t mask_stride = 0, int skip_stride = 0)
{
    flat_gemm_dma_body<DOT, MODE, PROBE, BF16, false>(queries, nq, base, n, dim, norms, scores, tile_stride, out_cols, thr, thr_stride,
                                                       thr_off, counts, cand, cap, mask, mask_stride, blockIdx.x, 0u, nullptr, skip_stride);
}

struct GemmGroup {
    int64_t a_off, b_off;
    int32_t a_cnt, b_cnt;
};
template <bool DOT, int MODE, bool BF16 = false>
__global__ __launch_bounds__(kGemmThreads) void flat_gemm_dma_grouped_kernel(
    const GemmGroup *__restrict__ groups, const int64_t *__restrict__ first_block, int ngroups,
    const float *__restrict__ queries, const float *__restrict__ base, int dim, const float *__restrict__ norms,
    float *__restrict__ scores, int tile_stride, int64_t out_cols, const float *__restrict__ thr, int thr_stride, int thr_off,
    int *__restrict__ counts, uint64_t *__restrict__ cand, int cap, const uint8_t *__restrict__ mask , const int64_t *__restrict__ mask_off )
{
    const int64_t b = blockIdx.x;
    if (b >= first_block[ngroups]) return;
    int lo = 0, hi = ngroups - 1;
    while (lo < hi) {
        const int mid = (lo + hi + 1) >> 1;
        if (first_block[mid] <= b)
            lo = mid;
        else
            hi = mid - 1;
    }
    const GemmGroup g = groups[lo];
    if (g.a_cnt == 0 || g.b_cnt == 0) return;
    flat_gemm_dma_body<DOT, MODE, 0, BF16, true>(
        queries + g.a_off * dim, g.a_cnt, base + g.b_off * dim, g.b_cnt, dim, norms + g.b_off,
        scores ? scores + g.a_off * out_cols : nullptr, tile_stride, out_cols, thr ? thr + g.a_off * thr_stride : nullptr, thr_stride,
        thr_off, counts ? counts + g.a_off : nullptr, cand ? cand + g.a_off * cap : nullptr, cap, mask, 0, b - first_block[lo],
        static_cast<uint32_t>(g.b_off), mask ? mask_off + g.a_off : nullptr);
}

constexpr int kBigBM = 256, kBigBN = 256, kBigThreads = 512;
constexpr int kBigTile = kBigBM * kGemmBK;
template <int NB>
constexpr size_t big_lds_bytes() { return (2 + NB) * kBigTile * sizeof(float); }

__device__ __forceinline__ void big_split3(float x, uint32_t &p0, uint32_t &p1, uint32_t &p2)
{
    auto rne = [](float v) {
        const uint32_t u = __float_as_uint(v);
        return (u + 0x7FFFu + ((u >> 16) & 1u)) >> 16;
    };
    p0 = rne(x);
    const float r1 = x - __uint_as_float(p0 << 16);
    p1 = rne(r1);
    const float r2 = r1 - __uint_as_float(p1 << 16);
    p2 = rne(r2);
}
__device__ __forceinline__ int big_max3_i32(int a, int b, int c)
{
    int r;
    asm("v_max3_i32 %0, %1, %2, %3" : "=v"(r) : "v"(a), "v"(b), "v"(c));
    return r;
}

typedef __bf16 vg_bf16x2 __attribute__((ext_vector_type(2)));
typedef float vg_f32x2 __attribute__((ext_vector_type(2)));
__device__ __forceinline__ void split2_bf16(float a, float b, uint32_t &hi, uint32_t &lo)
{
    hi = __builtin_bit_cast(uint32_t, __builtin_convertvector(vg_f32x2{a, b}, vg_bf16x2));
    const float ra = a - __uint_as_float(hi << 16), rb = b - __uint_as_float(hi & 0xFFFF0000u);
    lo = __builtin_bit_cast(uint32_t, __builtin_convertvector(vg_f32x2{ra, rb}, vg_bf16x2));
}

enum { kBigImages = 0, kBigSplit = 1, kBigScreen = 2 };
template <bool DOT, int NB, int PROBE, int OPS>
__device__ __forceinline__ void flat_gemm_big_body(
    const float *__restrict__ queries, int64_t nq, const float *__restrict__ base, int64_t n, int dim ,
    const float *__restrict__ norms, const float *__restrict__ thr, int thr_stride, int thr_off, int *__restrict__ counts,
    uint64_t *__restrict__ cand, int cap, const uint8_t *__restrict__ mask, int64_t mask_stride,
    int count_stride ,
    const uint32_t *__restrict__ tile_active = nullptr)
{
    static_assert(NB == 2 || NB == 3, "two or three row-tile buffers");
    constexpr bool SPLIT = OPS != kBigImages;
    constexpr bool SCREEN = OPS == kBigScreen;
    extern __shared__ float gemm_lds[];
    const int mtiles = static_cast<int>((nq + kBigBM - 1) / kBigBM);
    const int ntiles = static_cast<int>((n + kBigBN - 1) / kBigBN);
    const int total = mtiles * ((ntiles + 7) / 8) * 8, G = static_cast<int>(gridDim.x), xcd = static_cast<int>(blockIdx.x & 7);
    const int dq = (G >> 3) / mtiles, dr = (G >> 3) % mtiles;
    struct Pos {
        int bt, quo, rem;
    };
    auto tm_of = [&](const Pos &p) { return p.rem; };
    auto tn_of = [&](const Pos &p) { return p.quo * 8 + xcd; };
    const uint32_t active = tile_active ? *tile_active : 0xFFFFFFFFu;
    auto hole = [&](const Pos &p) { return tn_of(p) >= ntiles || ((active >> (p.rem & 31)) & 1u) == 0; };
    auto step = [&](Pos &p) {
        do {
            p.bt += G;
            p.quo += dq;
            p.rem += dr;
            if (p.rem >= mtiles) {
                p.rem -= mtiles;
                p.quo++;
            }
        } while (p.bt < total && hole(p));
    };
    Pos pos0;
    pos0.bt = static_cast<int>(blockIdx.x);
    pos0.quo = (pos0.bt >> 3) / mtiles;
    pos0.rem = (pos0.bt >> 3) % mtiles;
    if (pos0.bt < total && hole(pos0)) step(pos0);
    if (pos0.bt >= total) return;
    int my_tiles = 0;
    for (Pos p = pos0; p.bt < total; step(p)) my_tiles++;

    const int tid = threadIdx.x;
    const int lane = tid & 63;
    const int wave = __builtin_amdgcn_readfirstlane(tid >> 6);
    const int wr = wave >> 2, wc = wave & 3;
    const int ksteps = dim / kGemmBK;
    const int S = my_tiles * ksteps;

    const int drow = wave * 8 + (lane >> 3);
    const int dgl = (lane & 7) ^ ((wave * 4 + (lane >> 4)) & 7);
    const uint32_t lds0 = static_cast<uint32_t>(reinterpret_cast<uintptr_t>(
        (__attribute__((address_space(3))) void *)gemm_lds));
    auto piece = [&](int buf, int p) {
        return static_cast<uint32_t>(__builtin_amdgcn_readfirstlane(
            static_cast<int>(lds0 + (buf * kBigTile + (p * 64 + wave * 8) * kGemmBK) * 4)));
    };
    Pos a_pos = pos0, b_pos = pos0;
    int a_k = 0, b_k = 0, ia = 0, ib = 0;
    const float *abase, *bbase;
    int a_last, b_last;
    const uint32_t off0 = static_cast<uint32_t>((drow * dim + dgl * 4) * 4);
    auto set_a = [&](const Pos &ps) {
        const int64_t q0 = static_cast<int64_t>(tm_of(ps)) * kBigBM;
        abase = queries + q0 * dim;
        a_last = static_cast<int>(nq - q0 < kBigBM ? nq - q0 : kBigBM) - 1;
    };
    auto set_b = [&](const Pos &ps) {
        const int64_t n0 = static_cast<int64_t>(tn_of(ps)) * kBigBN;
        bbase = base + n0 * dim;
        b_last = static_cast<int>(n - n0 < kBigBN ? n - n0 : kBigBN) - 1;
    };
    auto fill = [&](const float *src , int last, int buf) {
        if (last == kBigBM - 1) {
#pragma unroll
            for (int p = 0; p < 4; p++) glds16(src + static_cast<int64_t>(p) * 64 * dim, off0, piece(buf, p));
        } else {
#pragma unroll
            for (int p = 0; p < 4; p++) {
                const int row = p * 64 + drow < last ? p * 64 + drow : last;
                glds16(src, static_cast<uint32_t>((row * dim + dgl * 4) * 4), piece(buf, p));
            }
        }
    };
    auto stage_a = [&]() {
        fill(abase + a_k * kGemmBK, a_last, ia);
        ia ^= 1;
        if (++a_k == ksteps) {
            a_k = 0;
            step(a_pos);
            if (a_pos.bt < total) set_a(a_pos);
        }
    };
    auto stage_b = [&]() {
        if (!(PROBE & 64)) fill(bbase + b_k * kGemmBK, b_last, 2 + ib);
        ib = ib + 1 == NB ? 0 : ib + 1;
        if (++b_k == ksteps) {
            b_k = 0;
            step(b_pos);
            if (b_pos.bt < total) set_b(b_pos);
        }
    };
    set_a(pos0);
    set_b(pos0);

    f32x16 acc[4][2];
    const int h = lane >> 5, f = (lane >> 1) & 7;
    int lpart[4];
#pragma unroll
    for (int j = 0; j < 4; j++) {
        const int gran = !SPLIT ? 2 * j + h : j < 2 ? 2 * j + h : 4 * (j - 2) + 2 * h;
        lpart[j] = (lane & 31) * kGemmBK + (gran ^ f) * 4;
    }
    const int a_wave = wr * 128 * kGemmBK, b_wave = wc * 64 * kGemmBK;

    constexpr float kThrClamp = 1e30f;
    Pos c_pos = pos0;
    float tq2[2], xq1;
    auto tile_loads = [&](const Pos &ps) {
        const int64_t q0 = static_cast<int64_t>(tm_of(ps)) * kBigBM, n0 = static_cast<int64_t>(tn_of(ps)) * kBigBN;
#pragma unroll
        for (int i = 0; i < 2; i++) {
            const int64_t qq = q0 + wr * 128 + i * 64 + lane;
            tq2[i] = thr[(qq < nq ? qq : nq - 1) * thr_stride + thr_off];
        }
        const int64_t nn = n0 + wc * 64 + lane;
        xq1 = norms[nn < n ? nn : n - 1];
    };
    auto tile_init = [&]() {
        const uint32_t one = 0x3F80u;
        uint4 ta[4], xb[2];
        const int64_t iq0 = static_cast<int64_t>(tm_of(c_pos)) * kBigBM;
#pragma unroll
        for (int i = 0; i < 4; i++) {
            float t = __shfl(tq2[i >> 1], (i & 1) * 32 + (lane & 31));
            t = iq0 + wr * 128 + i * 32 + (lane & 31) < nq ? t : -INFINITY;
            t = t < kThrClamp ? t : kThrClamp;
            t = t > -kThrClamp ? t : -kThrClamp;
            uint32_t p0, p1, p2;
            big_split3(DOT ? t : 0.5f * t, p0, p1, p2);
            ta[i] = h == 0 ? make_uint4(p0 | (p1 << 16), p2 | (one << 16), one | (one << 16), 0u) : make_uint4(0u, 0u, 0u, 0u);
        }
#pragma unroll
        for (int j = 0; j < 2; j++) {
            uint32_t p0 = 0, p1 = 0, p2 = 0;
            if (!DOT) big_split3(-0.5f * __shfl(xq1, j * 32 + (lane & 31)), p0, p1, p2);
            xb[j] = h == 0 ? make_uint4(one | (one << 16), one | (p0 << 16), p1 | (p2 << 16), 0u) : make_uint4(0u, 0u, 0u, 0u);
        }
        const f32x16 zero = {0.0f, 0.0f, 0.0f, 0.0f, 0.0f, 0.0f, 0.0f, 0.0f, 0.0f, 0.0f, 0.0f, 0.0f, 0.0f, 0.0f, 0.0f, 0.0f};
#pragma unroll
        for (int i = 0; i < 4; i++)
#pragma unroll
            for (int j = 0; j < 2; j++)
                acc[i][j] = __builtin_amdgcn_mfma_f32_32x32x16_bf16(__builtin_bit_cast(vg_bf16x8, ta[i]),
                                                                   __builtin_bit_cast(vg_bf16x8, xb[j]), zero, 0, 0, 0);
    };
#ifndef VG_BIG_PARK
#define VG_BIG_PARK 4
#endif
#ifndef VG_BIG_FLUSH_EVERY
#define VG_BIG_FLUSH_EVERY 6
#endif
    constexpr int kPark = VG_BIG_PARK;
    int pend = 0;
    uint32_t p_q[kPark], p_row[kPark];
    float p_a[kPark];
#pragma unroll
    for (int e = 0; e < kPark; e++) {
        p_q[e] = 0u;
        p_row[e] = 0u;
        p_a[e] = 0.0f;
    }
    constexpr int kFlushEvery = VG_BIG_FLUSH_EVERY;
    int flushes = 0, tiles_done = static_cast<int>(blockIdx.x >> 3) % kFlushEvery;
    auto finish = [&](uint32_t qq, uint32_t row, float a, float t, int pos) {
        t = t < kThrClamp ? t : kThrClamp;
        const float sc = DOT ? t - a : __builtin_fmaf(-2.0f, a, t);
        if (pos < cap) cand[qq * static_cast<uint32_t>(cap) + static_cast<uint32_t>(pos)] = make_key(sc, row, false);
    };
    auto flush_parked = [&]() {
        int pos[kPark];
        float tt[kPark];
#pragma unroll
        for (int e = 0; e < kPark; e++) {
            pos[e] = 0;
            tt[e] = 0.0f;
            if (pend > e) {
                pos[e] = (PROBE & 4096) ? e : atomicAdd(&counts[p_q[e] * static_cast<uint32_t>(count_stride)], 1);
                tt[e] = thr[p_q[e] * static_cast<uint32_t>(thr_stride) + static_cast<uint32_t>(thr_off)];
            }
        }
        __builtin_amdgcn_s_waitcnt(0x0F70);
#pragma unroll
        for (int e = 0; e < kPark; e++)
            if (pend > e) finish(p_q[e], p_row[e], p_a[e], tt[e], pos[e]);
        pend = 0;
        flushes++;
    };
    auto tile_append = [&](const Pos &ps) {
        const int64_t q0 = static_cast<int64_t>(tm_of(ps)) * kBigBM, n0 = static_cast<int64_t>(tn_of(ps)) * kBigBN;
        const int n_in = static_cast<int>(n - n0 < kBigBN ? n - n0 : kBigBN);
        int hv = 4 * h, lv = lane & 31;
        asm volatile("" : "+v"(hv), "+v"(lv));
#pragma unroll
        for (int i = 0; i < 4; i++) {
#pragma unroll
            for (int j = 0; j < 2; j++) {
                int gm[4];
#pragma unroll
                for (int g = 0; g < 4; g++) {
                    const int m3 = big_max3_i32(__float_as_int(acc[i][j][4 * g]), __float_as_int(acc[i][j][4 * g + 1]),
                                                __float_as_int(acc[i][j][4 * g + 2]));
                    gm[g] = m3 > __float_as_int(acc[i][j][4 * g + 3]) ? m3 : __float_as_int(acc[i][j][4 * g + 3]);
                }
                int mx = big_max3_i32(gm[0], gm[1], gm[2]);
                mx = mx > gm[3] ? mx : gm[3];
                if (__builtin_amdgcn_ballot_w64(mx > 0) == 0) continue;
                if (PROBE & 256) {
                    if (mx == 0x12345678) counts[0] = 1;
                    continue;
                }
                const int nl = wc * 64 + j * 32 + lv;
                if (nl >= n_in) continue;
#pragma unroll
                for (int g = 0; g < 4; g++) {
                    if (gm[g] <= 0) continue;
#pragma unroll
                    for (int e = 0; e < 4; e++) {
                        const int r = 4 * g + e;
                        const float a = acc[i][j][r];
                        if (a > 0.0f) {
                            const uint32_t qq = static_cast<uint32_t>(q0) + static_cast<uint32_t>(wr * 128 + i * 32 + (r & 3) + 8 * (r >> 2) + hv);
                            const int64_t nn = n0 + nl;
                            if (static_cast<int64_t>(qq) < nq && (mask == nullptr || mask_bit(mask + static_cast<int64_t>(qq) * mask_stride, nn))) {
                                if (pend < kPark) {
#pragma unroll
                                    for (int s2 = 0; s2 < kPark; s2++) {
                                        const bool here = pend == s2;
                                        p_q[s2] = here ? qq : p_q[s2];
                                        p_row[s2] = here ? static_cast<uint32_t>(nn) : p_row[s2];
                                        p_a[s2] = here ? a : p_a[s2];
                                    }
                                    pend++;
                                } else {
                                    finish(qq, static_cast<uint32_t>(nn), a, thr[qq * static_cast<uint32_t>(thr_stride) + static_cast<uint32_t>(thr_off)],
                                           atomicAdd(&counts[qq * static_cast<uint32_t>(count_stride)], 1));
                                }
                            }
                        }
                    }
                }
            }
        }
        if (PROBE & 2048) pend = 0;
        if (++tiles_done % kFlushEvery == 0) flush_parked();
    };

    float4 fa[2][4], fb[2][2];
    uint4 bc[2][2];
    auto read_part = [&](const float *As, const float *Bs, auto P) {
        constexpr int p = decltype(P)::value, set = p & 1;
        if constexpr (!SPLIT) {
            const float *pa = As + a_wave + lpart[p], *pb = Bs + b_wave + lpart[p];
#pragma unroll
            for (int i = 0; i < 4; i++) fa[set][i] = *reinterpret_cast<const float4 *>(pa + i * 32 * kGemmBK);
#pragma unroll
            for (int i = 0; i < 2; i++) fb[set][i] = *reinterpret_cast<const float4 *>(pb + i * 32 * kGemmBK);
        } else {
            const int oa = a_wave + lpart[p >> 1] + 2 * (p & 1) * 32 * kGemmBK;
#pragma unroll
            for (int b = 0; b < 2; b++) {
                fa[set][2 * b] = *reinterpret_cast<const float4 *>(As + oa + b * 32 * kGemmBK);
                if constexpr (!SCREEN) fa[set][2 * b + 1] = *reinterpret_cast<const float4 *>(As + ((oa + b * 32 * kGemmBK) ^ 16));
            }
            if constexpr ((p & 1) == 0) {
                const int ob = b_wave + lpart[2 + (p >> 1)];
#pragma unroll
                for (int b = 0; b < 2; b++) {
                    fb[b][0] = *reinterpret_cast<const float4 *>(Bs + ob + b * 32 * kGemmBK);
                    fb[b][1] = *reinterpret_cast<const float4 *>(Bs + ((ob + b * 32 * kGemmBK) ^ 4));
                }
            }
        }
    };
    auto mfma_part = [&](auto P) {
        constexpr int p = decltype(P)::value, set = p & 1;
        if constexpr (!SPLIT) {
#pragma unroll
            for (int i = 0; i < 4; i++)
#pragma unroll
                for (int j = 0; j < 2; j++)
                    acc[i][j] = __builtin_amdgcn_mfma_f32_32x32x16_bf16(__builtin_bit_cast(vg_bf16x8, fa[set][i]),
                                                                       __builtin_bit_cast(vg_bf16x8, fb[set][j]), acc[i][j], 0, 0, 0);
        } else {
            constexpr int i0 = 2 * (p & 1), even = (p & 1) == 0;
            auto raw = [&](int b, int w) { return w == 0 ? make_float2(fb[b][0].x, fb[b][0].y) : w == 1 ? make_float2(fb[b][0].z, fb[b][0].w) :
                                                  w == 2 ? make_float2(fb[b][1].x, fb[b][1].y) : make_float2(fb[b][1].z, fb[b][1].w); };
            auto put = [](uint4 &v, int w, uint32_t x) { (w == 0 ? v.x : w == 1 ? v.y : w == 2 ? v.z : v.w) = x; };
            auto get = [](const uint4 &v, int w) { return w == 0 ? v.x : w == 1 ? v.y : w == 2 ? v.z : v.w; };
            if constexpr (even) {
#pragma unroll
                for (int b = 0; b < 2; b++)
#pragma unroll
                    for (int w = 0; w < 4; w++)
                        put(bc[b][0], w, __builtin_bit_cast(uint32_t, __builtin_convertvector(vg_f32x2{raw(b, w).x, raw(b, w).y}, vg_bf16x2)));
                __builtin_amdgcn_sched_barrier(0);
            }
#pragma unroll
            for (int pr = 0; pr < (SCREEN ? 1 : 3); pr++)
#pragma unroll
                for (int b = 0; b < 2; b++)
#pragma unroll
                    for (int j = 0; j < 2; j++) {
                        acc[i0 + b][j] = __builtin_amdgcn_mfma_f32_32x32x16_bf16(
                            __builtin_bit_cast(vg_bf16x8, fa[set][2 * b + (pr == 1 ? 1 : 0)]),
                            __builtin_bit_cast(vg_bf16x8, bc[j][pr == 2 ? 1 : 0]), acc[i0 + b][j], 0, 0, 0);
                        if constexpr (even && !SCREEN) {
                            if (pr < 2) {
                                const int u = pr * 4 + b * 2 + j, rb = u >> 2, w = u & 3;
                                const uint32_t hi = get(bc[rb][0], w);
                                const float ra = raw(rb, w).x - __uint_as_float(hi << 16), rc = raw(rb, w).y - __uint_as_float(hi & 0xFFFF0000u);
                                put(bc[rb][1], w, __builtin_bit_cast(uint32_t, __builtin_convertvector(vg_f32x2{ra, rc}, vg_bf16x2)));
                                __builtin_amdgcn_sched_barrier(0);
                            }
                        }
                    }
        }
    };
    using P0 = std::integral_constant<int, 0>;
    using P1 = std::integral_constant<int, 1>;
    using P2 = std::integral_constant<int, 2>;
    using P3 = std::integral_constant<int, 3>;

    tile_loads(pos0);
    stage_a();
    stage_b();
    if (NB == 3 && S > 1) stage_b();
    tile_init();
    if (NB == 3 && S > 1)
        asm volatile("s_waitcnt vmcnt(4)" ::: "memory");
    else
        asm volatile("s_waitcnt vmcnt(0)" ::: "memory");
    __builtin_amdgcn_s_barrier();
    asm volatile("" ::: "memory");
    int ra = 0, rb = 0;
    __builtin_amdgcn_s_waitcnt(0xC07F);
    read_part(gemm_lds, gemm_lds + 2 * kBigTile, P0{});
    int t = 0;
    for (int g = 0; g < S; g++) {
        const float *As = gemm_lds + ra * kBigTile, *Bs = gemm_lds + (2 + rb) * kBigTile;
        const bool last = t == ksteps - 1;
        Pos n_pos = c_pos;
        if (last) {
            step(n_pos);
            if (n_pos.bt >= total) n_pos = c_pos;
            tile_loads(n_pos);
        }
        if (!(PROBE & 16)) read_part(As, Bs, P1{});
        __builtin_amdgcn_sched_barrier(0);
        mfma_part(P0{});
        __builtin_amdgcn_sched_barrier(0);
        if (g + 1 < S && !(PROBE & 2)) stage_a();
        if (g + NB - 1 < S && !(PROBE & 2) && (PROBE & 512)) stage_b();
        if (!(PROBE & 16)) read_part(As, Bs, P2{});
        __builtin_amdgcn_sched_barrier(0);
        mfma_part(P1{});
        __builtin_amdgcn_sched_barrier(0);
        if (g + NB - 1 < S && !(PROBE & 2) && !(PROBE & 512)) stage_b();
        if (!(PROBE & 16)) read_part(As, Bs, P3{});
        __builtin_amdgcn_sched_barrier(0);
        mfma_part(P2{});
        __builtin_amdgcn_sched_barrier(0);
        ra ^= 1;
        rb = rb + 1 == NB ? 0 : rb + 1;
        __builtin_amdgcn_s_waitcnt(0xC07F);
        if (NB == 3 && g + 2 < S)
            asm volatile("s_waitcnt vmcnt(4)" ::: "memory");
        else
            asm volatile("s_waitcnt vmcnt(0)" ::: "memory");
        if (!(PROBE & 8)) __builtin_amdgcn_s_barrier();
        asm volatile("" ::: "memory");
        if (!(PROBE & 16)) read_part(gemm_lds + ra * kBigTile, gemm_lds + (2 + rb) * kBigTile, P0{});
        __builtin_amdgcn_sched_barrier(0);
        mfma_part(P3{});
        __builtin_amdgcn_sched_barrier(0);
        if (last) {
            if (!(PROBE & 1)) {
                tile_append(c_pos);
            } else {
                float sum = 0.0f;
                for (int i = 0; i < 4; i++)
                    for (int j = 0; j < 2; j++)
                        for (int r = 0; r < 16; r++) sum += acc[i][j][r];
                if (sum == 123.456f) counts[0] = 1;
            }
            c_pos = n_pos;
            t = 0;
            if (PROBE & 1024) {
#pragma unroll
                for (int i = 0; i < 4; i++)
#pragma unroll
                    for (int j = 0; j < 2; j++)
#pragma unroll
                        for (int r = 0; r < 16; r++) acc[i][j][r] = 0.0f;
            } else {
                tile_init();
            }
        } else {
            t++;
        }
    }
    flush_parked();
    if ((PROBE & 32768) && lane == 0) atomicAdd(&counts[nq * count_stride], flushes);
}

template <bool DOT, int NB, int PROBE = 0>
__global__ __launch_bounds__(kBigThreads) void flat_gemm_bf16_big_kernel(
    const float *__restrict__ queries, int64_t nq, const float *__restrict__ base, int64_t n, int dim, const float *__restrict__ norms,
    const float *__restrict__ thr, int thr_stride, int thr_off, int *__restrict__ counts, uint64_t *__restrict__ cand, int cap,
    const uint8_t *__restrict__ mask, int64_t mask_stride, int count_stride)
{
    flat_gemm_big_body<DOT, NB, PROBE, kBigImages>(queries, nq, base, n, dim, norms, thr, thr_stride, thr_off, counts, cand, cap, mask,
                                                   mask_stride, count_stride);
}
template <bool DOT, int NB, int PROBE = 0>
__global__ __launch_bounds__(kBigThreads) void flat_gemm_split_big_kernel(
    const float *__restrict__ queries, int64_t nq, const float *__restrict__ base, int64_t n, int dim, const float *__restrict__ norms,
    const float *__restrict__ thr, int thr_stride, int thr_off, int *__restrict__ counts, uint64_t *__restrict__ cand, int cap,
    const uint8_t *__restrict__ mask, int64_t mask_stride, int count_stride, const uint32_t *__restrict__ tile_active)
{
    flat_gemm_big_body<DOT, NB, PROBE, kBigSplit>(queries, nq, base, n, dim, norms, thr, thr_stride, thr_off, counts, cand, cap, mask,
                                                  mask_stride, count_stride, tile_active);
}
template <bool DOT, int NB, int PROBE = 0>
__global__ __launch_bounds__(kBigThreads) void flat_gemm_screen_big_kernel(
    const float *__restrict__ queries, int64_t nq, const float *__restrict__ base, int64_t n, int dim, const float *__restrict__ norms,
    const float *__restrict__ thr, int thr_stride, int thr_off, int *__restrict__ counts, uint64_t *__restrict__ cand, int cap,
    const uint8_t *__restrict__ mask, int64_t mask_stride, int count_stride)
{
    flat_gemm_big_body<DOT, NB, PROBE, kBigScreen>(queries, nq, base, n, dim, norms, thr, thr_stride, thr_off, counts, cand, cap, mask,
                                                   mask_stride, count_stride);
}

constexpr int kG32BM = 32;
#ifndef VG_PROBE_RB
#define VG_PROBE_RB 4
#endif
constexpr int kProbeRB = VG_PROBE_RB;
template <int RB>
constexpr size_t g32_lds_bytes() { return 2 * (RB * kG32BM * kGemmBK + kDmaTile) * sizeof(float); }

template <bool DOT, int MODE, int RB, bool BF16, bool GROUPED>
__device__ __forceinline__ void flat_gemm_dma32_body(
    const float *__restrict__ queries, int64_t nq, const float *__restrict__ base, int64_t n,
    int dim, const float *__restrict__ norms, float *__restrict__ scores, int tile_stride,
    int64_t out_cols, const float *__restrict__ thr, int thr_stride, int thr_off,
    int *__restrict__ counts, uint64_t *__restrict__ cand, int cap, const uint8_t *__restrict__ mask,
    int64_t mask_stride, int64_t tn, uint32_t row_base, const int64_t *__restrict__ mask_off = nullptr)
{
    auto filter_of = [&](int ql) { return GROUPED && mask_off ? mask + mask_off[ql] : mask + ql * mask_stride; };
    extern __shared__ float gemm_lds[];
    constexpr int kATile = RB * kG32BM * kGemmBK;
    const int64_t ntiles = MODE == 1 ? (((n + kGemmBN - 1) / kGemmBN) + tile_stride - 1) / tile_stride
                                     : (n + kGemmBN - 1) / kGemmBN;
    if (tn >= ntiles) return;
    const int64_t n0 = (MODE == 1 ? tn * tile_stride : tn) * kGemmBN;

    const int tid = threadIdx.x;
    const int lane = tid & 63;
    const int wave = __builtin_amdgcn_readfirstlane(tid >> 6);

    const int drow = wave * 8 + (lane >> 3);
    const int dgl = (lane & 7) ^ ((wave * 4 + (lane >> 4)) & 7);
    const float *const bbase = base + n0 * dim;
    uint32_t boff[kGemmPasses], aoff[RB];
#pragma unroll
    for (int p = 0; p < kGemmPasses; p++) {
        int64_t nb = n0 + p * 32 + drow;
        if (nb >= n) nb = n - 1;
        boff[p] = static_cast<uint32_t>(((nb - n0) * dim + dgl * 4) * 4);
    }
#pragma unroll
    for (int p = 0; p < RB; p++) {
        int64_t qa = p * 32 + drow;
        if (qa >= nq) qa = nq - 1;
        aoff[p] = static_cast<uint32_t>((qa * dim + dgl * 4) * 4);
    }
    const int ksteps = (dim + kGemmBK - 1) / kGemmBK;
    const int full_steps = dim / kGemmBK;
    const uint32_t lds0 = static_cast<uint32_t>(reinterpret_cast<uintptr_t>(
        (__attribute__((address_space(3))) void *)gemm_lds));
    constexpr int kBuf = kATile + kDmaTile;
    auto a_piece = [&](int b, int p) {
        return static_cast<uint32_t>(__builtin_amdgcn_readfirstlane(
            static_cast<int>(lds0 + (b * kBuf + (p * 32 + wave * 8) * kGemmBK) * 4)));
    };
    auto b_piece = [&](int b, int p) {
        return static_cast<uint32_t>(__builtin_amdgcn_readfirstlane(
            static_cast<int>(lds0 + (b * kBuf + kATile + (p * 32 + wave * 8) * kGemmBK) * 4)));
    };
    auto dma_tile = [&](int kt) {
        const int k0 = kt * kGemmBK, b = kt & 1;
        if (kt < full_steps) {
#pragma unroll
            for (int p = 0; p < RB; p++) glds16(queries + k0, aoff[p], a_piece(b, p));
#pragma unroll
            for (int p = 0; p < kGemmPasses; p++) glds16_stream(bbase + k0, boff[p], b_piece(b, p));
        } else {
            const float *zeros = reinterpret_cast<const float *>(&g_gemm_zero16);
            const bool in = k0 + dgl * 4 < dim;
#pragma unroll
            for (int p = 0; p < RB; p++) glds16(in ? queries + k0 + aoff[p] / 4 : zeros, a_piece(b, p));
#pragma unroll
            for (int p = 0; p < kGemmPasses; p++) glds16(in ? bbase + k0 + boff[p] / 4 : zeros, b_piece(b, p));
        }
    };
    f32x16 acc[RB];
#pragma unroll
    for (int i = 0; i < RB; i++)
#pragma unroll
        for (int r = 0; r < 16; r++) acc[i][r] = 0.0f;
    const int h = lane >> 5, f = (lane >> 1) & 7;
    int goff[4];
#pragma unroll
// ... 134 lines not shown
```

### vecgo_amd/csrc/vg_grow_rows.hpp

```cpp
#pragma once

#include "vg_internal.hpp"

namespace vg {

template <typename T, typename F>
static int32_t grow_rows(T **p, int64_t *cap, int64_t n_old, int64_t n_new, F bytes, hipStream_t st)
{
    const int64_t have = std::max(*cap, n_old);
    if (*p && n_new <= have) return VG_OK;
    const int64_t want = std::max(n_new, have + have / 2);
    DevBuf<char> q;
    VG_TRY(q.alloc(bytes(want)));
    if (*p && n_old) VG_HIP(hipMemcpyAsync(q.p, *p, bytes(n_old), hipMemcpyDeviceToDevice, st));
    VG_HIP(hipStreamSynchronize(st));
    drop_device(p);
    *p = reinterpret_cast<T *>(q.release());
    *cap = want;
    return VG_OK;
}

static int32_t append_index_rows(vg_index *idx, const float *rows, int64_t count, hipStream_t st)
{
    const int64_t n_old = idx->n, n_new = n_old + count;
    const int dim = idx->dim;
    if (!idx->d_norm_max) {
        VG_HIP(hipMalloc(reinterpret_cast<void **>(&idx->d_norm_max), 2 * sizeof(float)));
        VG_HIP(hipMemsetAsync(idx->d_norm_max, 0, 2 * sizeof(float), st));
    }
    if (!idx->d_flat_stats) {
        VG_HIP(hipMalloc(reinterpret_cast<void **>(&idx->d_flat_stats), 3 * sizeof(unsigned long long)));
        VG_HIP(hipMemsetAsync(idx->d_flat_stats, 0, 3 * sizeof(unsigned long long), st));
    }
    {
        int64_t cap = idx->rows_cap;
        VG_TRY(grow_rows(&idx->d_norms, &cap, n_old, n_new, [](int64_t r) { return static_cast<size_t>(r) * 4; }, st));
        int64_t cap_v = idx->rows_cap;
        VG_TRY(grow_rows(&idx->d_vectors, &cap_v, n_old, n_new, [&](int64_t r) { return static_cast<size_t>(r) * dim * 4; }, st));
        idx->rows_cap = std::min(cap, cap_v);
    }
    VG_HIP(hipMemcpyAsync(idx->d_vectors + n_old * dim, rows, static_cast<size_t>(count) * dim * 4, hipMemcpyDeviceToDevice, st));
    VG_TRY(append_row_norms(idx, n_old, n_new, st));
    if (idx->d_vectors_bf16) {
        const int64_t bd = idx->vectors_bf16_dim;
        VG_TRY(grow_rows(&idx->d_vectors_bf16, &idx->bf16_cap, n_old, n_new, [&](int64_t r) { return static_cast<size_t>(r) * bd * 2; }, st));
        VG_TRY(append_bf16_rows(idx, n_old, n_new, st));
    }
    return VG_OK;
}

}
```

### vecgo_amd/csrc/vg_internal.hpp

```cpp
#pragma once

#include <hip/hip_runtime.h>

#include <algorithm>
#include <atomic>
#include <cstdarg>
#include <cstdint>
#include <cstdio>
#include <cstdlib>
#include <cstring>
#include <mutex>
#include <string>
#include <vector>

#include "../../include/vecgo_hip.h"

struct vg_index;

#define VG_API extern "C" __attribute__((visibility("default")))

namespace vg {

void set_error(const char *fmt, ...);

#define VG_HIP(expr)                                                                          \
    do {                                                                                      \
        hipError_t _e = (expr);                                                               \
        if (_e != hipSuccess) {                                                               \
            ::vg::set_error("%s failed: %s (%s:%d)", #expr, hipGetErrorString(_e), __FILE__,   \
                            __LINE__);                                                        \
            (void)hipGetLastError();                                                          \
            return _e == hipErrorOutOfMemory ? VG_ERR_OUT_OF_MEMORY : VG_ERR_HIP;             \
        }                                                                                     \
    } while (0)

#define VG_LAUNCH(...)                                                                              \
    do {                                                                                            \
        (void)hipGetLastError();                                                                    \
        hipLaunchKernelGGL(__VA_ARGS__);                                                            \
        hipError_t _le = hipGetLastError();                                                         \
        if (_le != hipSuccess) {                                                                    \
            ::vg::set_error("kernel launch failed: %s (%s:%d)", hipGetErrorString(_le), __FILE__,   \
                            __LINE__);                                                              \
            return VG_ERR_HIP;                                                                      \
        }                                                                                           \
    } while (0)

#define VG_CHECK(cond, status, ...)          \
    do {                                     \
        if (!(cond)) {                       \
            ::vg::set_error(__VA_ARGS__);    \
            return (status);                 \
        }                                    \
    } while (0)

#define VG_TRY(expr)                   \
    do {                               \
        int32_t _s = (expr);           \
        if (_s != VG_OK) return _s;    \
    } while (0)

bool is_device_ptr(const void *p);

enum Hook {
    kHookFlatNoSmallTile,
    kHookFlatUnfused,
    kHookFlatNoScan,
    kHookFlatForceExact,
    kHookFlatNoDma,
    kHookFlatDebug,
    kHookProbeNoGroup,
    kHookAdcBigkExhaustive,
    kHookBuildDebug,
    kHookKmNoMfma,
    kHookKmListAll,
    kHookKmBf16,
    kHookKmNoBf16,
    kHookBruteNoFlat,
    kHookPqNoMfma,
    kHookPqListAll,
    kHookPqFp32Mfma,
    kHookProbeNoGemm,
    kHookFlatNoBigTile,
    kHookFlatBigTile2,
    kHookFlatBigEarlyB,
    kHookPqNomAlways,
    kHookKmNoRanges,
    kHookNoCandReplay,
    kHookVamanaSmallScratch,
    kHookFlatRescoreSample,
    kHookPthrForceHist,
    kHookWalkSmallScratch,
    kHookFlatNoSplit,
    kHookFlatNoScreen,
    kHookFlatScreenFail,
    kHookCount
};
bool hook(Hook h);

int32_t scratch_alloc(void **out, size_t bytes, hipStream_t s);
int32_t append_row_norms(vg_index *idx, int64_t from, int64_t to, hipStream_t st);
int32_t append_bf16_rows(vg_index *idx, int64_t from, int64_t to, hipStream_t st);
void scratch_free(void *p);
void scratch_trim(int device);

}

struct vg_prof_record {
    const char *name;
    hipEvent_t start, stop;
};

struct vg_arena {
    char *base = nullptr;
    size_t cap = 0;
};

struct vg_ctx {
    int device = 0;
    std::mutex arena_mu;
    std::vector<std::pair<hipStream_t, vg_arena>> arenas;
    hipStream_t stream = nullptr;
    int compute_units = 0;
    int64_t hbm_bytes = 0;
    char arch[64] = {0};
    bool profiling = false;
    std::mutex prof_mu;
    std::vector<vg_prof_record> prof;
};

namespace vg {
struct ProfScope {
    vg_ctx *ctx;
    hipStream_t st;
    vg_prof_record rec{};
    bool active = false;
    ProfScope(vg_ctx *c, const char *name, hipStream_t s) : ctx(c), st(s)
    {
        if (!c->profiling) return;
        if (hipEventCreateWithFlags(&rec.start, hipEventReleaseToDevice) != hipSuccess) return;
        if (hipEventCreateWithFlags(&rec.stop, hipEventReleaseToDevice) != hipSuccess) {
            (void)hipEventDestroy(rec.start);
            return;
        }
        rec.name = name;
        (void)hipEventRecord(rec.start, st);
        active = true;
    }
    ~ProfScope()
    {
        if (!active) return;
        (void)hipEventRecord(rec.stop, st);
        std::lock_guard<std::mutex> g(ctx->prof_mu);
        ctx->prof.push_back(rec);
    }
};
}

namespace vg {

inline hipStream_t pick_stream(vg_ctx *ctx, void *stream)
{
    return stream ? reinterpret_cast<hipStream_t>(stream) : ctx->stream;
}

template <typename... T>
inline bool aligned16(const T *...p)
{
    return ((reinterpret_cast<uintptr_t>(p) | ...) & 15) == 0;
}

enum Align { kStage16, kAnyAlign };
void note_staged_device_buffer();
void note_flat_split_launch();

template <typename T>
struct DevIn {
    const T *ptr = nullptr;
// ... 323 lines not shown
```

### vecgo_amd/csrc/vg_search.hpp

```cpp
#pragma once

#include <algorithm>
#include <type_traits>

#include "vg_internal.hpp"
#include "vg_walk_chunk.hpp"

namespace vg {

int32_t launch_topk_merge(const uint64_t *partial, int64_t nq, int lists, int k, bool descending,
                          uint32_t *ids, float *scores, hipStream_t st, const int *only_if = nullptr,
                          const int *always = nullptr);
int32_t launch_pq_retile(const uint8_t *codes, int64_t n, int m, int groups, int64_t n_tiles, uint8_t *tiles, hipStream_t st);
int32_t launch_probe_scan_adc(const vg_index *idx, const float *tables, const uint32_t *probes, const uint32_t *part_off,
                              int64_t nq, int np, int split, int k, uint64_t *partial, const uint64_t *min_keys, bool desc,
                              const uint8_t *mask, int64_t mask_stride, hipStream_t st);
int32_t pq_nan_replay(vg_index *idx, const float *d_queries, int64_t nq, int k, bool desc, const uint8_t *d_mask, int64_t mask_stride,
                      const uint32_t *d_probes, int np, const uint32_t *d_part_off, uint32_t *d_ids, float *d_scores, hipStream_t st);
int32_t pq_adc_search_masked(vg_index *idx, const float *queries, int64_t nq, int32_t k, const uint8_t *mask, int64_t mask_stride,
                             bool desc, uint32_t *ids, float *scores, void *stream);

int32_t hnsw_edge_distances(vg_index *idx, const float *l0_dist, hipStream_t st);

int32_t launch_pq_build_table(const vg_pq *pq, const float *d_queries, int64_t nq, float *d_tables,
                              bool scan_layout, hipStream_t st);

int32_t launch_page_patch(int64_t nq, int k, int off, int kk, bool descending, const int *always_one,
                          const uint32_t *fids, const float *fscores, uint32_t *ids, float *scores, uint64_t *min_keys,
                          hipStream_t st);
int32_t flat_search_masked(vg_index *idx, const float *queries, int64_t nq, int32_t k, const uint8_t *mask, int64_t mask_stride,
                           uint32_t *ids, float *scores, void *stream, bool l2_scores = false, bool cand_replay = true);
float bf16_filter_eps(bool dot);
struct ThrNomPlan {
    int cap, sel_k, sample_stride;
    bool bf16;
    float eps_extra;
};
struct ThrNominated {
    float *gthr, *qnorm;
    int *untight, *counts;
    uint64_t *cand;
};
size_t flat_thr_nominate_scratch(const vg_index *idx, const ThrNomPlan &plan, int64_t qc);
int32_t flat_thr_nominate(vg_index *idx, const ThrNomPlan &plan, const float *qp, const float *uthr, int64_t cnt, const uint8_t *m0,
                          int64_t mask_stride, char *scratch, ThrNominated *out, hipStream_t st);
int32_t launch_flat_todo(const int *flags, const int *always, int cnt, int *todo, unsigned long long *stats, hipStream_t st);

constexpr int kThrMaxResults = 16384;
constexpr int kThrQB = 8;
inline bool thr_scan_regs(const vg_index *idx)
{
    return idx->dim % 4 == 0 && idx->dim >= 64 && idx->dim <= 1024 && aligned16(idx->d_vectors);
}
template <class F>
inline int32_t with_metric(bool dot, F f)
{
    return dot ? f(std::true_type{}) : f(std::false_type{});
}
int32_t launch_thr_select_lists(bool desc, const uint64_t *lists, int64_t list_cap, const int *counts, const int *qmap, int64_t nq,
                                int64_t longest, int max_results, uint32_t *ids, float *scores, int32_t *out_counts, hipStream_t st);
int32_t launch_thr_filter(bool desc, const float *thr, int64_t nq, int max_results, uint32_t *ids, float *scores, int32_t *counts,
                          hipStream_t st);
int32_t launch_thr_rescore(bool desc, const float *base, int dim, const float *queries, const float *thr, const uint64_t *cand,
                           const int *cand_counts, const uint32_t *cand_ids, int64_t nq, int cap, uint64_t *lists, int *list_counts,
                           hipStream_t st);
int32_t launch_thr_scan_f32(const vg_index *idx, const float *queries, const float *thr, const int *qmap, int64_t cnt,
                            const uint8_t *mask, int64_t mask_stride, int64_t list_cap, uint64_t *lists, int *counts, hipStream_t st);

int32_t launch_probe_select(const vg_index *idx, const float *d_queries, int64_t nq, int np, bool dot, uint32_t *d_probes, hipStream_t st);

int32_t launch_dim_minmax(const float *d_rows, int64_t n, int dim, DevTmp<float> &pmin, DevTmp<float> &pmax, int &chunks,
                          hipStream_t st);

int32_t launch_probe_scan_sq8(const vg_index *idx, const float *queries, const uint32_t *probes, const uint32_t *part_off,
                              int64_t nq, int np, int sub, int k, uint64_t *partial, const uint64_t *min_keys,
                              const uint8_t *mask, int64_t mask_stride, hipStream_t st);
int32_t launch_probe_scan_sq8_grouped(const vg_index *idx, const float *queries, const uint32_t *part_off,
                                      const uint32_t *pair_of, const ProbeGroup *groups, const uint32_t *ngroups, unsigned gmax,
                                      int np, int sub, int k, uint64_t *partial, const uint64_t *min_keys, const uint8_t *mask,
                                      int64_t mask_stride, hipStream_t st);
int32_t sq8_nan_replay(vg_index *idx, const float *d_queries, int64_t nq, int k, const uint8_t *d_mask, int64_t mask_stride,
                       const uint32_t *d_probes, int np, const uint32_t *d_part_off, uint32_t *d_ids, float *d_scores, hipStream_t st);

int32_t vamana_build_check(const vg_index *idx, int32_t &r, int32_t &l, float &alpha, int32_t max_batch, int32_t growth_div);

int32_t launch_rabitq_encode(const float *d_vectors, int64_t n, int dim, uint8_t *d_codes, hipStream_t st);
int32_t launch_rabitq_retile(const uint8_t *codes, int64_t n, int nb, int groups, int64_t n_tiles, uint8_t *tiles, float *norms,
                             hipStream_t st);

struct SearchIO {
    hipStream_t st = nullptr;
    DevIn<float> q;
    DevIn<uint8_t> mk;
    DevOut<uint32_t> oid;
    DevOut<float> osc;
    int32_t init(vg_ctx *ctx, void *stream, const float *queries, size_t query_floats, uint32_t *ids, float *scores, size_t results,
                 const uint8_t *mask = nullptr, size_t mask_bytes = 0, Align align = kStage16)
    {
        VG_HIP(hipSetDevice(ctx->device));
        st = pick_stream(ctx, stream);
        VG_TRY(q.init(queries, query_floats, st, align));
        VG_TRY(oid.init(ids, results, st, align));
        VG_TRY(osc.init(scores, results, st, align));
        return mk.init(mask, mask_bytes, st, align);
    }
    int32_t finish()
    {
        VG_TRY(oid.finish());
        return osc.finish();
    }
};

struct WalkIO : SearchIO {
    DevOut<vg_search_stats> ost;
    int32_t init(vg_ctx *ctx, void *stream, const float *queries, size_t query_floats, uint32_t *ids, float *scores, size_t results,
                 vg_search_stats *stats, int64_t nq, const uint8_t *mask = nullptr, size_t mask_bytes = 0)
    {
        VG_TRY(SearchIO::init(ctx, stream, queries, query_floats, ids, scores, results, mask, mask_bytes));
        return ost.init(stats, stats ? static_cast<size_t>(nq) : 0, st);
    }
    vg_search_stats *stats_at(int64_t q0) const { return ost.ptr ? ost.ptr + q0 : nullptr; }
    int32_t finish()
    {
        VG_TRY(SearchIO::finish());
        return ost.finish();
    }
};

inline size_t mask_span(const uint8_t *mask, int64_t mask_stride, int64_t nq, int64_t n)
// ... 116 lines not shown
```

Before: 425,200 queries/s.

## Run flat threshold sampling through the split big-tile MFMA kernel

Adds a SAMPLE variant of the big-tile flat GEMM body that scores sampled base-row tiles (two strided half-tiles per big tile) with split query images and writes dense score rows. In the split nomination path, queries are now split before sampling, and the sample GEMM uses this persistent big-tile kernel instead of the generic tile kernel. It also adds an appended-candidate counter to the flat stats with a new API for reading it. The intent is to speed up the threshold sampling GEMM. This adds template complexity and a debug hook to fall back.

```diff
diff --git a/go/segment/resident.go b/go/segment/resident.go
--- a/go/segment/resident.go
+++ b/go/segment/resident.go
@@ -452,6 +452,12 @@
 func (r *Resident) FlatRetried() (int64, error) {
 	var n C.int64_t
 	st := C.vg_index_flat_retried(r.h, &n, nil)
+	return int64(n), hipctx.Err(int32(st))
+}
+
+func (r *Resident) FlatAppended() (int64, error) {
+	var n C.int64_t
+	st := C.vg_index_flat_appended(r.h, &n, nil)
 	return int64(n), hipctx.Err(int32(st))
 }
 
diff --git a/include/vecgo_hip.h b/include/vecgo_hip.h
--- a/include/vecgo_hip.h
+++ b/include/vecgo_hip.h
@@ -195,6 +195,8 @@
 
 int32_t vg_index_flat_retried(vg_index *idx, int64_t *retried, void *stream);
 
+int32_t vg_index_flat_appended(vg_index *idx, int64_t *appended, void *stream);
+
 int32_t vg_search_rabitq(vg_index *idx, const float *queries, int64_t nq, int32_t k, uint32_t *ids,
                          float *scores, void *stream);
 
diff --git a/include/vecgo_hip.hpp b/include/vecgo_hip.hpp
--- a/include/vecgo_hip.hpp
+++ b/include/vecgo_hip.hpp
@@ -589,6 +589,12 @@
         check(vg_search_flat_probed_threshold(h_, queries, nq, thresholds, max_results, nprobes, scan, rerank ? 1 : 0, mask, mask_stride,
                                               r.ids.data(), r.scores.data(), r.counts.data(), nullptr));
         return r;
+    }
+    int64_t FlatAppended()
+    {
+        int64_t n = 0;
+        check(vg_index_flat_appended(h_, &n, nullptr));
+        return n;
     }
     void EnableBF16Filter(bool on = true) { check(vg_index_enable_bf16_filter(h_, on ? 1 : 0, nullptr)); }
     Result SearchPQ(const float *queries, int64_t nq, int k) { return run(nq, k, [&](Result &r) { return vg_search_pq_adc(h_, queries, nq, k, r.ids.data(), r.scores.data(), nullptr); }); }
diff --git a/vecgo_amd/api.py b/vecgo_amd/api.py
--- a/vecgo_amd/api.py
+++ b/vecgo_amd/api.py
@@ -1408,6 +1408,11 @@
         check(self._lib.vg_index_flat_retried(self._h, C.byref(r), _stream_ptr(stream)))
         return r.value
 
+    def flat_appended(self, stream=None):
+        r = C.c_int64(0)
+        check(self._lib.vg_index_flat_appended(self._h, C.byref(r), _stream_ptr(stream)))
+        return r.value
+
     def search_pq_adc(self, queries, k, out=None, stream=None):
         return self._search(self._lib.vg_search_pq_adc, queries, k, out=out, stream=stream)
 
diff --git a/vecgo_amd/csrc/k_exact.hip b/vecgo_amd/csrc/k_exact.hip
--- a/vecgo_amd/csrc/k_exact.hip
+++ b/vecgo_amd/csrc/k_exact.hip
@@ -192,12 +192,12 @@
         VG_HIP(hipMalloc(reinterpret_cast<void **>(&idx->d_norms), static_cast<size_t>(idx->n) * sizeof(float)));
         VG_HIP(hipMalloc(reinterpret_cast<void **>(&idx->d_norm_max), 2 * sizeof(float)));
         VG_HIP(hipMemsetAsync(idx->d_norm_max, 0, 2 * sizeof(float), st));
-        VG_HIP(hipMalloc(reinterpret_cast<void **>(&idx->d_flat_stats), 3 * sizeof(unsigned long long)));
+        VG_HIP(hipMalloc(reinterpret_cast<void **>(&idx->d_flat_stats), 4 * sizeof(unsigned long long)));
         VG_HIP(hipMemcpyAsync(idx->d_vectors, base, count * sizeof(float), hipMemcpyDefault, st));
         VG_LAUNCH(vg::row_norms_kernel, dim3(static_cast<unsigned>((idx->n + 3) / 4)), dim3(256),
                            0, st, idx->d_vectors, idx->n, idx->dim, idx->d_norms, reinterpret_cast<int *>(idx->d_norm_max + 1));
         VG_LAUNCH(vg::norm_max_kernel, dim3(1), dim3(1024), 0, st, idx->d_norms, idx->n, idx->d_norm_max);
-        VG_HIP(hipMemsetAsync(idx->d_flat_stats, 0, 3 * sizeof(unsigned long long), st));
+        VG_HIP(hipMemsetAsync(idx->d_flat_stats, 0, 4 * sizeof(unsigned long long), st));
         VG_HIP(hipStreamSynchronize(st));
         return VG_OK;
     }();
diff --git a/vecgo_amd/csrc/k_flat.hip b/vecgo_amd/csrc/k_flat.hip
--- a/vecgo_amd/csrc/k_flat.hip
+++ b/vecgo_amd/csrc/k_flat.hip
@@ -119,11 +119,14 @@
     const int64_t mt = (c.cnt + kGemmBM - 1) / kGemmBM, nt = (c.ops.n + kGemmBN - 1) / kGemmBN;
     const int64_t tiles = skip ? nt - gemm_skip_sampled_tiles(nt, skip) : (nt + a.tile_stride - 1) / a.tile_stride;
     const dim3 grid(static_cast<unsigned>(mt * ((tiles + 7) / 8) * 8)), threads(kGemmThreads);
+    auto big_grid = [&](int64_t bnt ) {
+        const int64_t bmt = (c.cnt + kBigBM - 1) / kBigBM;
+        const int64_t slots = bmt * ((bnt + 7) / 8) * 8, per_cu = std::max(a.cus / 8, 1) * 8;
+        return dim3(static_cast<unsigned>(std::min(slots, per_cu)));
+    };
     auto launch_big = [&](auto kern, size_t lds, auto... extra) -> int32_t {
-        const int64_t bmt = (c.cnt + kBigBM - 1) / kBigBM, bnt = (c.ops.n + kBigBN - 1) / kBigBN;
-        const int64_t slots = bmt * ((bnt + 7) / 8) * 8, per_cu = std::max(a.cus / 8, 1) * 8;
         if (a.counts_wide && !a.tile_active) VG_HIP(hipMemsetAsync(a.counts_wide, 0, sizeof(int) * static_cast<size_t>(c.cnt) * kCountLine, st));
-        VG_TRY(launch_lds(kern, dim3(static_cast<unsigned>(std::min(slots, per_cu))), dim3(kBigThreads), lds, st, a.queries, c.cnt, c.ops.b, c.ops.n,
+        VG_TRY(launch_lds(kern, big_grid((c.ops.n + kBigBN - 1) / kBigBN), dim3(kBigThreads), lds, st, a.queries, c.cnt, c.ops.b, c.ops.n,
                           c.ops.dim_words, c.ops.norms, a.thr, a.thr_stride, a.thr_off, a.counts_wide ? a.counts_wide : a.counts, a.cand, a.cap, c.mask,
                           c.mask_stride, a.counts_wide ? kCountLine : 1, extra...));
         if (a.counts_wide)
@@ -138,6 +141,13 @@
     auto launch_g32 = [&](auto kern, size_t lds) { return launch_tile(kern, dim3(static_cast<unsigned>(tiles)), lds); };
     constexpr int M = MODE == 0 ? 1 : MODE;
     const int rb = static_cast<int>((c.cnt + kG32BM - 1) / kG32BM);
+    if constexpr (MODE == 1) {
+        if (a.split) {
+            VG_CHECK(!bf16 && gemm_runs_split(true, false, dma, c.cnt, c.ops.dim_words, 0, 0), VG_ERR_INVALID_ARG, "launch_gemm: sample tile on a call without it");
+            return launch_lds(flat_gemm_sample_big_kernel<DOT, 3>, big_grid((tiles + 1) / 2), dim3(kBigThreads), big_lds_bytes<3>(), st, a.queries, c.cnt,
+                              c.ops.b, c.ops.n, c.ops.dim_words, c.ops.norms, a.scores, a.tile_stride, a.out_cols, c.mask, c.mask_stride);
+        }
+    }
     if (MODE == 2 && a.split) {
         VG_CHECK(!bf16 && gemm_runs_split(true, false, dma, c.cnt, c.ops.dim_words, a.cap, a.thr_stride), VG_ERR_INVALID_ARG, "launch_gemm: split tile on a call without it");
         if (a.screen) return launch_big(flat_gemm_screen_big_kernel<DOT, 3>, big_lds_bytes<3>());
@@ -198,9 +208,10 @@
 
 __global__ __launch_bounds__(256) void flat_todo_kernel(const int *__restrict__ flags, const int *__restrict__ always,
                                                         int cnt, int *__restrict__ todo,
-                                                        unsigned long long *__restrict__ stats)
+                                                        unsigned long long *__restrict__ stats, const int *__restrict__ counts)
 {
     __shared__ int part[256];
+    __shared__ unsigned long long appended[256];
     const int tid = threadIdx.x;
     const int per = (cnt + 255) / 256;
     const int lo = tid * per < cnt ? tid * per : cnt, hi = lo + per < cnt ? lo + per : cnt;
@@ -210,17 +221,25 @@
     }
     const bool all = *always != 0;
     int mine = 0;
-    for (int i = lo; i < hi; i++) mine += (all || flags[i] != 0);
+    unsigned long long app = 0;
+    for (int i = lo; i < hi; i++) {
+        mine += (all || flags[i] != 0);
+        if (counts) app += static_cast<unsigned long long>(counts[i]);
+    }
     part[tid] = mine;
+    appended[tid] = app;
     __syncthreads();
     if (tid == 0) {
         int run = 0;
+        app = 0;
         for (int t = 0; t < 256; t++) {
             const int c = part[t];
             part[t] = run;
             run += c;
+            app += appended[t];
         }
         todo[0] = run;
+        if (counts) atomicAdd(&stats[3], app);
         atomicAdd(&stats[0], static_cast<unsigned long long>(cnt));
         atomicAdd(&stats[1], static_cast<unsigned long long>(run));
     }
@@ -642,6 +661,10 @@
 static bool gemm_runs_screen(bool split, int k)
 {
     return split && !hook(kHookFlatNoScreen) && k <= (hook(kHookFlatScreenFail) ? kGemmMaxK : kScreenMaxK);
+}
+static bool sample_runs_big(bool split, bool use_sample)
+{
+    return split && use_sample && !hook(kHookFlatF32Sample);
 }
 constexpr int kScanMaxBatch = 4;
 template <bool DOT>
@@ -784,13 +807,16 @@
     VG_TRY(launch_flat_select(s, cnt, sel_k, st));
     return launch_topk_merge(s.partial, cnt, s.slices, sel_k, false, ids, thr, st);
 }
-static int32_t sample_thresholds(const NomCall &c, const NomScratch &s, int stride, int sel_k, float *thr, bool sampled)
+static int32_t sample_thresholds(const NomCall &c, const NomScratch &s, int stride, int sel_k, float *thr, bool sampled, const uint32_t *image = nullptr,
+                                 int cus = 0)
 {
     if (!sampled) {
         VG_LAUNCH(fill_f32_kernel, dim3(static_cast<unsigned>((c.cnt * sel_k + 255) / 256)), dim3(256), 0, c.st, thr, c.cnt * sel_k, INFINITY);
         return VG_OK;
     }
-    VG_TRY(launch_gemm<1>(GemmArgs::sample(c, s.sc, stride, s.cols)));
+    GemmArgs a = GemmArgs::sample(c, s.sc, stride, s.cols);
+    if (image) a.split_tile(image).wide(nullptr, cus);
+    VG_TRY(launch_gemm<1>(a));
     return select_thresholds(s, c.cnt, sel_k, s.sid, thr, c.st);
 }
 static int32_t launch_flat_pick(const ProbeNominated &nom, int64_t cnt, const int *only, hipStream_t st)
@@ -973,11 +999,13 @@
     const bool screen = gemm_runs_screen(split, c.k);
     const float eps_extra = screen ? screen_gemm_eps(c.dot, c.dim) : split ? split_gemm_eps(c.dot, c.dim) : s.bf16 ? bf16_filter_eps(c.dot) : 0.0f;
     if (s.bf16) VG_TRY(gemm_operands(c.q, c.nq, c.dim, c.n, idx->d_norms, idx->d_vectors_bf16, idx->vectors_bf16_dim, s.qbf, c.st, &nc.ops));
-    VG_TRY(sample_thresholds(nc, s, kFlatSampleStride, nom.sel_k, nom.thr, s.use_sample));
-    if (s.bf16 || split) VG_LAUNCH(flat_thr_cap_kernel, dim3(nc.ucnt()), dim3(64), 0, c.st, nom.thr, nom.sel_k, c.q, c.dim, idx->d_norm_max);
+    const uint32_t *image = reinterpret_cast<const uint32_t *>(s.qbf);
     if (split)
         VG_LAUNCH(flat_split_queries_kernel, dim3(static_cast<unsigned>((c.nq * (c.dim / 2) + 255) / 256)), dim3(256), 0, c.st, c.q, c.nq, c.dim,
                   reinterpret_cast<uint32_t *>(s.qbf));
+    VG_TRY(sample_thresholds(nc, s, kFlatSampleStride, nom.sel_k, nom.thr, s.use_sample, sample_runs_big(split, s.use_sample) ? image : nullptr,
+                             idx->ctx->compute_units));
+    if (s.bf16 || split) VG_LAUNCH(flat_thr_cap_kernel, dim3(nc.ucnt()), dim3(64), 0, c.st, nom.thr, nom.sel_k, c.q, c.dim, idx->d_norm_max);
     const bool once = s.use_sample && gemm_skips_sample(nc.ops.dma, c.nq, s.bf16, split);
     if (!once) VG_HIP(hipMemsetAsync(nom.counts, 0, sizeof(int) * static_cast<size_t>(c.nq), c.st));
     {
@@ -1037,7 +1065,7 @@
     for (int64_t q0 = 0; q0 < call.nq; q0 += s.qc) {
         const FlatCall c = call.range(q0, std::min(s.qc, call.nq - q0));
         VG_TRY(s.fused ? flat_fused_chunk(c, s) : flat_unfused_chunk(c, s));
-        VG_TRY(launch_flat_todo(s.flags, always, static_cast<int>(c.nq), s.todo, c.idx->d_flat_stats, c.st));
+        VG_TRY(launch_flat_todo(s.flags, always, static_cast<int>(c.nq), s.todo, c.idx->d_flat_stats, c.st, s.fused ? s.nom.counts : nullptr));
         if (hook(kHookFlatDebug)) flat_debug_counts(c, q0, s);
         VG_TRY(flat_fallback_pages(c, s));
     }
@@ -1237,9 +1265,9 @@
     return launch_gemm<2>(GemmArgs::append(nc, out.gthr, 1, out.counts, out.cand, p.cap).wide(p.bf16 ? s.counts_wide : nullptr, idx->ctx->compute_units));
 }
 
-int32_t launch_flat_todo(const int *flags, const int *always, int cnt, int *todo, unsigned long long *stats, hipStream_t st)
-{
-    VG_LAUNCH(flat_todo_kernel, dim3(1), dim3(256), 0, st, flags, always, cnt, todo, stats);
+int32_t launch_flat_todo(const int *flags, const int *always, int cnt, int *todo, unsigned long long *stats, hipStream_t st, const int *counts)
+{
+    VG_LAUNCH(flat_todo_kernel, dim3(1), dim3(256), 0, st, flags, always, cnt, todo, stats, counts);
     return VG_OK;
 }
 }
@@ -1260,6 +1288,19 @@
               idx->d_vectors_bf16 + from * idx->vectors_bf16_dim);
     return VG_OK;
 }
+}
+
+VG_API int32_t vg_index_flat_appended(vg_index *idx, int64_t *appended, void *stream)
+{
+    VG_CHECK(idx && appended, VG_ERR_INVALID_ARG, "vg_index_flat_appended: NULL index or pointer");
+    VG_CHECK(idx->d_flat_stats, VG_ERR_INVALID_ARG, "vg_index_flat_appended: no fp32 vectors attached");
+    VG_HIP(hipSetDevice(idx->ctx->device));
+    hipStream_t st = vg::pick_stream(idx->ctx, stream);
+    unsigned long long h = 0;
+    VG_HIP(hipMemcpyAsync(&h, idx->d_flat_stats + 3, sizeof h, hipMemcpyDeviceToHost, st));
+    VG_HIP(hipStreamSynchronize(st));
+    *appended = static_cast<int64_t>(h);
+    return VG_OK;
 }
 
 VG_API int32_t vg_index_enable_bf16_filter(vg_index *idx, int32_t on, void *stream)
diff --git a/vecgo_amd/csrc/vg_api.hip b/vecgo_amd/csrc/vg_api.hip
--- a/vecgo_amd/csrc/vg_api.hip
+++ b/vecgo_amd/csrc/vg_api.hip
@@ -321,7 +321,8 @@
                                                    "VG_PQ_LIST_ALL", "VG_PQ_FP32_MFMA", "VG_PROBE_NO_GEMM", "VG_FLAT_NO_BIG_TILE",
                                                    "VG_FLAT_BIG_TILE_2", "VG_FLAT_BIG_EARLY_B", "VG_PQ_NOM_ALWAYS", "VG_KM_NO_RANGES", "VG_NO_CAND_REPLAY",
                                                    "VG_VAMANA_SMALL_SCRATCH", "VG_FLAT_RESCORE_SAMPLE", "VG_PTHR_FORCE_HIST",
-                                                   "VG_WALK_SMALL_SCRATCH", "VG_FLAT_NO_SPLIT", "VG_FLAT_NO_SCREEN", "VG_FLAT_SCREEN_FAIL"};
+                                                   "VG_WALK_SMALL_SCRATCH", "VG_FLAT_NO_SPLIT", "VG_FLAT_NO_SCREEN", "VG_FLAT_SCREEN_FAIL",
+                                                   "VG_FLAT_F32_SAMPLE"};
 static void hooks_from_env()
 {
     for (int h = 0; h < kHookCount; h++) {
diff --git a/vecgo_amd/csrc/vg_flat_gemm.hpp b/vecgo_amd/csrc/vg_flat_gemm.hpp
--- a/vecgo_amd/csrc/vg_flat_gemm.hpp
+++ b/vecgo_amd/csrc/vg_flat_gemm.hpp
@@ -526,20 +526,22 @@
 }
 
 enum { kBigImages = 0, kBigSplit = 1, kBigScreen = 2 };
-template <bool DOT, int NB, int PROBE, int OPS>
+template <bool DOT, int NB, int PROBE, int OPS, bool SAMPLE = false>
 __device__ __forceinline__ void flat_gemm_big_body(
     const float *__restrict__ queries, int64_t nq, const float *__restrict__ base, int64_t n, int dim ,
     const float *__restrict__ norms, const float *__restrict__ thr, int thr_stride, int thr_off, int *__restrict__ counts,
     uint64_t *__restrict__ cand, int cap, const uint8_t *__restrict__ mask, int64_t mask_stride,
     int count_stride ,
-    const uint32_t *__restrict__ tile_active = nullptr)
+    const uint32_t *__restrict__ tile_active = nullptr, float *__restrict__ scores = nullptr ,
+    int tile_stride = 1, int64_t out_cols = 0)
 {
     static_assert(NB == 2 || NB == 3, "two or three row-tile buffers");
     constexpr bool SPLIT = OPS != kBigImages;
     constexpr bool SCREEN = OPS == kBigScreen;
     extern __shared__ float gemm_lds[];
     const int mtiles = static_cast<int>((nq + kBigBM - 1) / kBigBM);
-    const int ntiles = static_cast<int>((n + kBigBN - 1) / kBigBN);
+    const int ntiles = SAMPLE ? static_cast<int>((((n + kGemmBN - 1) / kGemmBN + tile_stride - 1) / tile_stride + 1) / 2)
+                              : static_cast<int>((n + kBigBN - 1) / kBigBN);
     const int total = mtiles * ((ntiles + 7) / 8) * 8, G = static_cast<int>(gridDim.x), xcd = static_cast<int>(blockIdx.x & 7);
     const int dq = (G >> 3) / mtiles, dr = (G >> 3) % mtiles;
     struct Pos {
@@ -586,8 +588,8 @@
     };
     Pos a_pos = pos0, b_pos = pos0;
     int a_k = 0, b_k = 0, ia = 0, ib = 0;
-    const float *abase, *bbase;
-    int a_last, b_last;
+    const float *abase, *bbase, *bbase1 = nullptr;
+    int a_last, b_last, b_last1 = 0;
     const uint32_t off0 = static_cast<uint32_t>((drow * dim + dgl * 4) * 4);
     auto set_a = [&](const Pos &ps) {
         const int64_t q0 = static_cast<int64_t>(tm_of(ps)) * kBigBM;
@@ -599,6 +601,14 @@
         bbase = base + n0 * dim;
         b_last = static_cast<int>(n - n0 < kBigBN ? n - n0 : kBigBN) - 1;
     };
+    auto half_row0 = [&](const Pos &ps, int hf) { return (static_cast<int64_t>(tn_of(ps)) * 2 + hf) * tile_stride * kGemmBN; };
+    auto set_b_halves = [&](const Pos &ps) {
+        const int64_t r0 = half_row0(ps, 0), r1 = half_row0(ps, 1);
+        bbase = base + r0 * dim;
+        b_last = static_cast<int>(n - r0 < kGemmBN ? n - r0 : kGemmBN) - 1;
+        bbase1 = r1 < n ? base + r1 * dim : bbase;
+        b_last1 = r1 < n ? static_cast<int>(n - r1 < kGemmBN ? n - r1 : kGemmBN) - 1 : b_last;
+    };
     auto fill = [&](const float *src , int last, int buf) {
         if (last == kBigBM - 1) {
 #pragma unroll
@@ -610,6 +620,27 @@
                 glds16(src, static_cast<uint32_t>((row * dim + dgl * 4) * 4), piece(buf, p));
             }
         }
+    };
+    auto fill_b = [&](int k0, int buf) {
+        if constexpr (!SAMPLE) {
+            fill(bbase + k0, b_last, buf);
+        } else if (b_last == kGemmBN - 1 && b_last1 == kGemmBN - 1) {
+#pragma unroll
+            for (int p = 0; p < 4; p++) glds16((p < 2 ? bbase : bbase1) + k0 + static_cast<int64_t>(p & 1) * 64 * dim, off0, piece(buf, p));
+        } else {
+#pragma unroll
+            for (int p = 0; p < 4; p++) {
+                const int last = p < 2 ? b_last : b_last1;
+                const int row = (p & 1) * 64 + drow < last ? (p & 1) * 64 + drow : last;
+                glds16((p < 2 ? bbase : bbase1) + k0, static_cast<uint32_t>((row * dim + dgl * 4) * 4), piece(buf, p));
+            }
+        }
+    };
+    auto next_b = [&](const Pos &ps) {
+        if constexpr (SAMPLE)
+            set_b_halves(ps);
+        else
+            set_b(ps);
     };
     auto stage_a = [&]() {
         fill(abase + a_k * kGemmBK, a_last, ia);
@@ -621,16 +652,16 @@
         }
     };
     auto stage_b = [&]() {
-        if (!(PROBE & 64)) fill(bbase + b_k * kGemmBK, b_last, 2 + ib);
+        if (!(PROBE & 64)) fill_b(b_k * kGemmBK, 2 + ib);
         ib = ib + 1 == NB ? 0 : ib + 1;
         if (++b_k == ksteps) {
             b_k = 0;
             step(b_pos);
-            if (b_pos.bt < total) set_b(b_pos);
+            if (b_pos.bt < total) next_b(b_pos);
         }
     };
     set_a(pos0);
-    set_b(pos0);
+    next_b(pos0);
 
     f32x16 acc[4][2];
     const int h = lane >> 5, f = (lane >> 1) & 7;
@@ -645,7 +676,13 @@
     constexpr float kThrClamp = 1e30f;
     Pos c_pos = pos0;
     float tq2[2], xq1;
+    float xn[2] = {0.0f, 0.0f};
     auto tile_loads = [&](const Pos &ps) {
+        if constexpr (SAMPLE) {
+            const int64_t nn = half_row0(ps, wc >> 1) + (wc & 1) * 64 + lane;
+            xq1 = norms[nn < n ? nn : n - 1];
+            return;
+        }
         const int64_t q0 = static_cast<int64_t>(tm_of(ps)) * kBigBM, n0 = static_cast<int64_t>(tn_of(ps)) * kBigBN;
 #pragma unroll
         for (int i = 0; i < 2; i++) {
@@ -656,6 +693,15 @@
         xq1 = norms[nn < n ? nn : n - 1];
     };
     auto tile_init = [&]() {
+        if constexpr (SAMPLE) {
+#pragma unroll
+            for (int i = 0; i < 4; i++)
+#pragma unroll
+                for (int j = 0; j < 2; j++)
+#pragma unroll
+                    for (int r = 0; r < 16; r++) acc[i][j][r] = 0.0f;
+            return;
+        }
         const uint32_t one = 0x3F80u;
         uint4 ta[4], xb[2];
         const int64_t iq0 = static_cast<int64_t>(tm_of(c_pos)) * kBigBM;
@@ -784,6 +830,66 @@
         if (++tiles_done % kFlushEvery == 0) flush_parked();
     };
 
+    auto pull_norms = [&](float (&dst)[2]) {
+#pragma unroll
+        for (int j = 0; j < 2; j++) dst[j] = __shfl(xq1, j * 32 + (lane & 31));
+    };
+    auto tile_scores = [&](const Pos &ps) {
+        float xnext[2];
+        pull_norms(xnext);
+        __builtin_amdgcn_sched_barrier(0);
+        const int64_t q0 = static_cast<int64_t>(tm_of(ps)) * kBigBM;
+        int hv = 4 * h, lv = lane & 31;
+        asm volatile("" : "+v"(hv), "+v"(lv));
+        const int nq_in = static_cast<int>(nq - q0 < kBigBM ? nq - q0 : kBigBM);
+        float *const out = scores + q0 * out_cols + static_cast<int64_t>(tn_of(ps)) * kBigBN;
+        auto put = [&](auto guarded, auto masked) {
+            constexpr bool GUARDED = decltype(guarded)::value, MASKED = decltype(masked)::value;
+#pragma unroll
+            for (int j = 0; j < 2; j++) {
+                const int col = wc * 64 + j * 32 + lv;
+                const int64_t nn = half_row0(ps, wc >> 1) + (col & (kGemmBN - 1));
+                const bool col_ok = static_cast<int64_t>(tn_of(ps)) * kBigBN + col < out_cols, row_ok = nn < n;
+#pragma unroll
+                for (int i = 0; i < 4; i++) {
+                    asm volatile("" : "+v"(hv));
+                    int ql = wr * 128 + i * 32 + hv;
+                    int64_t off = ql * out_cols + col;
+#pragma unroll
+                    for (int g = 0; g < 4; g++) {
+                        bool keep[4];
+#pragma unroll
+                        for (int e = 0; e < 4; e++)
+                            keep[e] = row_ok && (!MASKED || ((!GUARDED || ql + e < nq_in) && mask_bit(mask + (q0 + ql + e) * mask_stride, nn)));
+#pragma unroll
+                        for (int e = 0; e < 4; e++) {
+                            const float sc = DOT ? -acc[i][j][4 * g + e] : __builtin_fmaf(-2.0f, acc[i][j][4 * g + e], xn[j]);
+                            if (!GUARDED || (ql + e < nq_in && col_ok)) out[off] = keep[e] ? sc : INFINITY;
+                            off += out_cols;
+                        }
+                        ql += 8;
+                        off += 4 * out_cols;
+                        asm volatile("" : "+v"(off));
+                        if (MASKED) __builtin_amdgcn_sched_barrier(0);
+                    }
+                }
+            }
+        };
+        const bool whole = nq_in == kBigBM && (static_cast<int64_t>(tn_of(ps)) + 1) * kBigBN <= out_cols;
+        if (mask == nullptr) {
+            if (whole)
+                put(std::false_type{}, std::false_type{});
+            else
+                put(std::true_type{}, std::false_type{});
+        } else {
+            if (whole)
+                put(std::false_type{}, std::true_type{});
+            else
+                put(std::true_type{}, std::true_type{});
+        }
+        xn[0] = xnext[0], xn[1] = xnext[1];
+    };
+
     float4 fa[2][4], fb[2][2];
     uint4 bc[2][2];
     auto read_part = [&](const float *As, const float *Bs, auto P) {
@@ -864,6 +970,7 @@
     stage_a();
     stage_b();
     if (NB == 3 && S > 1) stage_b();
+    if constexpr (SAMPLE) pull_norms(xn);
     tile_init();
     if (NB == 3 && S > 1)
         asm volatile("s_waitcnt vmcnt(4)" ::: "memory");
@@ -913,7 +1020,9 @@
         mfma_part(P3{});
         __builtin_amdgcn_sched_barrier(0);
         if (last) {
-            if (!(PROBE & 1)) {
+            if constexpr (SAMPLE) {
+                tile_scores(c_pos);
+            } else if (!(PROBE & 1)) {
                 tile_append(c_pos);
             } else {
                 float sum = 0.0f;
@@ -938,7 +1047,7 @@
             t++;
         }
     }
-    flush_parked();
+    if constexpr (!SAMPLE) flush_parked();
     if ((PROBE & 32768) && lane == 0) atomicAdd(&counts[nq * count_stride], flushes);
 }
 
@@ -968,6 +1077,15 @@
 {
     flat_gemm_big_body<DOT, NB, PROBE, kBigScreen>(queries, nq, base, n, dim, norms, thr, thr_stride, thr_off, counts, cand, cap, mask,
                                                    mask_stride, count_stride);
+}
+
+template <bool DOT, int NB, int PROBE = 0>
+__global__ __launch_bounds__(kBigThreads) void flat_gemm_sample_big_kernel(
+    const float *__restrict__ queries, int64_t nq, const float *__restrict__ base, int64_t n, int dim, const float *__restrict__ norms,
+    float *__restrict__ scores, int tile_stride, int64_t out_cols, const uint8_t *__restrict__ mask, int64_t mask_stride)
+{
+    flat_gemm_big_body<DOT, NB, PROBE, kBigScreen, true>(queries, nq, base, n, dim, norms, nullptr, 0, 0, nullptr, nullptr, 0, mask, mask_stride, 1,
+                                                         nullptr, scores, tile_stride, out_cols);
 }
 
 constexpr int kG32BM = 32;
diff --git a/vecgo_amd/csrc/vg_grow_rows.hpp b/vecgo_amd/csrc/vg_grow_rows.hpp
--- a/vecgo_amd/csrc/vg_grow_rows.hpp
+++ b/vecgo_amd/csrc/vg_grow_rows.hpp
@@ -29,8 +29,8 @@
         VG_HIP(hipMemsetAsync(idx->d_norm_max, 0, 2 * sizeof(float), st));
     }
     if (!idx->d_flat_stats) {
-        VG_HIP(hipMalloc(reinterpret_cast<void **>(&idx->d_flat_stats), 3 * sizeof(unsigned long long)));
-        VG_HIP(hipMemsetAsync(idx->d_flat_stats, 0, 3 * sizeof(unsigned long long), st));
+        VG_HIP(hipMalloc(reinterpret_cast<void **>(&idx->d_flat_stats), 4 * sizeof(unsigned long long)));
+        VG_HIP(hipMemsetAsync(idx->d_flat_stats, 0, 4 * sizeof(unsigned long long), st));
     }
     {
         int64_t cap = idx->rows_cap;
diff --git a/vecgo_amd/csrc/vg_internal.hpp b/vecgo_amd/csrc/vg_internal.hpp
--- a/vecgo_amd/csrc/vg_internal.hpp
+++ b/vecgo_amd/csrc/vg_internal.hpp
@@ -94,6 +94,7 @@
     kHookFlatNoSplit,
     kHookFlatNoScreen,
     kHookFlatScreenFail,
+    kHookFlatF32Sample,
     kHookCount
 };
 bool hook(Hook h);
diff --git a/vecgo_amd/csrc/vg_search.hpp b/vecgo_amd/csrc/vg_search.hpp
--- a/vecgo_amd/csrc/vg_search.hpp
+++ b/vecgo_amd/csrc/vg_search.hpp
@@ -44,7 +44,8 @@
 size_t flat_thr_nominate_scratch(const vg_index *idx, const ThrNomPlan &plan, int64_t qc);
 int32_t flat_thr_nominate(vg_index *idx, const ThrNomPlan &plan, const float *qp, const float *uthr, int64_t cnt, const uint8_t *m0,
                           int64_t mask_stride, char *scratch, ThrNominated *out, hipStream_t st);
-int32_t launch_flat_todo(const int *flags, const int *always, int cnt, int *todo, unsigned long long *stats, hipStream_t st);
+int32_t launch_flat_todo(const int *flags, const int *always, int cnt, int *todo, unsigned long long *stats, hipStream_t st,
+                         const int *counts = nullptr);
 
 constexpr int kThrMaxResults = 16384;
 constexpr int kThrQB = 8;
```

After: 461,000 queries/s (median of 6 runs). 8.4% higher.
